# TrevorS/qwen3-tts-rs

Hardware: AMD Instinct MI355X
Metric: acoustic_frames_per_sec (higher is better)
Workload: dtype bf16

## Files before the change

include/q3tts.h:

```cpp
#ifndef Q3TTS_H
#define Q3TTS_H

#include <stddef.h>
#include <stdint.h>

#ifdef __cplusplus
extern "C" {
#endif

#define Q3_ABI_VERSION 1
#define Q3_MAX_BATCH 64

typedef enum q3_status {
    Q3_OK = 0,
    Q3_INVALID_ARG = 1,
    Q3_IO = 2,
    Q3_MISSING_WEIGHT = 3,
    Q3_KV_OVERFLOW = 4,
    Q3_HIP_ERROR = 5,
    Q3_RCCL_ERROR = 6,
    Q3_UNSUPPORTED = 7,
    Q3_OOM = 8
} q3_status;

// ... 141 lines not shown
q3_status q3_session_open_text(q3_session* s, int b);
q3_status q3_session_append_text(q3_session* s, int b, const uint32_t* ids, int n, int last);
q3_status q3_session_text_state(q3_session* s, int b, int* n_text, int* frames_committed, int* frames_runnable, int* closed,
                                int* frames_replayed);

enum {
    Q3_GET_PREFILL_EMBEDS = 0,
    Q3_GET_LAST_HIDDEN = 1,
    Q3_GET_LOGITS = 2,
    Q3_GET_TRAILING = 3,
    Q3_GET_PAD_EMBED = 4,
    Q3_GET_LOGITS_HIST = 5,
    Q3_GET_CP_LOGITS = 6,
    Q3_GET_TOKEN = 7,
    Q3_GET_CP_LOGITS_HIST = 8
};
q3_status q3_session_set_kv_dtype(q3_session* s, int dtype);
q3_status q3_session_set_debug(q3_session* s, int capture_logits);
q3_status q3_session_prefill_len(q3_session* s, int b, int* prefill_len, int* trailing_len);
q3_status q3_session_get(q3_session* s, int what, int b, void* out_host, size_t bytes);
q3_status q3_talker_step(q3_session* s, const float* embeds_host, float* hidden_host, float* logits_host);
q3_status q3_cp_generate(q3_session* s, const float* last_hidden_host, const float* sem_embed_host,
                         uint32_t* codes15_host, float* cp_logits_host );
q3_status q3_frame_embed(q3_model* m, uint32_t sem_token, const uint32_t* codes15, const float* text_add_host,
                         float* out_host);
q3_status q3_sample(int device, const float* logits_host, const uint8_t* seen_host, const float* u_host,
                    int rows, int vocab, const q3_options* opts, int token_count, uint32_t* tokens_host);
void      q3_rng_seed(uint64_t seed, uint64_t* state);
float     q3_rng_next(uint64_t* state);
q3_status q3_fused_residual_rmsnorm(int device, int dtype, const void* x_host, const void* res_host,
                                    const void* w_host, int rows, int cols, float eps,
                                    void* normed_host, void* sum_host);
q3_status q3_linear(int device, const float* x_host, const uint16_t* w_bf16_host, const float* bias_host,
                    int M, int N, int K, float* y_host);
typedef struct q3_linear_ex_args {
    int M, N, K, ldx, ldy, ldr, M_alloc;
    int epi, tiled, ksplit, use_ws, zero_n, zero_guard;
    float eps;
    const float* x; const uint16_t* w; const uint16_t* w2;
    const float* bias; const float* norm_w; const float* resid;
    float* y; float* zero_buf;
} q3_linear_ex_args;
q3_status q3_linear_ex(int device, const q3_linear_ex_args* args);
typedef struct q3_attn_step_args {
    int variant, B, nh, nkv, n_splits, max_seq;
    float eps; int reserved;
    const int* pos; const float* qkv; const float* q_norm_w; const float* k_norm_w;
    const float* rope_cos; const float* rope_sin;
    float* kcache; float* vcache; float* out;
} q3_attn_step_args;
q3_status q3_attn_step(int device, const q3_attn_step_args* args);
typedef struct q3_attn_step_ex_args {
    int variant, layout, B, nh, nkv, n_splits, max_seq, rows_per_seq;
    int n_layers, layer, n_slabs, kv_row_pages;
    int qkv_S, qkv_K, g_vocab, g_proj_dim, g_ldx, g_max_frames, g_code_slot, zero_n, zero_guard;
    float eps, qkv_eps; int reserved;
    const int* pos; const float* qkv; const float* q_norm_w; const float* k_norm_w;
    const float* rope_cos; const float* rope_sin;
    float* kcache; float* vcache; float* out;
    const int* page_slots; int* rot_used; long long* stray;
    const float* qkv_part; const float* qkv_ssq;
    const float* g_logits; const uint32_t* g_tok; const float* g_qkv_tab; const float* g_proj_tab;
    float* g_x; uint32_t* g_codes; const int* g_frame_idx;
    float* zero_buf;
} q3_attn_step_ex_args;
q3_status q3_attn_step_ex(int device, const q3_attn_step_ex_args* args);
q3_status q3_kv_pages_to_bf16_ex(int device, int n_layers, int nkv, int n_pages, const int* src_slots, const int* dst_slots,
                                 const float* src, uint16_t* dst, int* rot_used, long long* stray);
int         q3_conv_path(int cout, int cin, int L, int k, int dil, int phases, int packed, int has_resid, int planes, int aligned16);
int         q3_resunit_path(int C, int L, int dil, int packed, int ya_is_xa, int planes);
const char* q3_conv_path_name(int code);
typedef struct q3_conv_ex_args {
    int kind, cin, cout, L, k, dil, stride;
    int act, planes, packed, resid_in_place, snake_raw, y2_is_x;
    int y_front, y_elems;
    int* path;
    const float* x; const float* w; const float* b;
    const float* snake_a; const float* snake_b; const float* resid; const float* scale;
    const float* post_a; const float* post_ib;
    const float* w2; const float* b2; const float* mid_a; const float* mid_ib;
    float* y; float* y2;
} q3_conv_ex_args;
q3_status q3_conv_ex(int device, const q3_conv_ex_args* args);
int q3_gemm_path(int M, int N, int K, int epi, int norm, int w2, int planes, int* path);
typedef struct q3_gemm_ex_args {
    int M, N, K, ldx, ldy, ldr, M_alloc;
    int epi, geometry, k_split, sup_m, sup_n;
    float eps;
    int* path;
    const float* x; const uint16_t* w; const uint16_t* w2;
    const float* bias; const float* norm_w; const float* resid;
    float* y;
} q3_gemm_ex_args;
q3_status q3_gemm_ex(int device, const q3_gemm_ex_args* args);
int q3_attn_prefill_path(int nh, int nkv, int use_planes, int halves, int* path);
typedef struct q3_attn_prefill_ex_args {
    int n_seq, rps, base_pos, nh, nkv, max_seq, ld_qkv, ld_out;
    int kernel, halves, use_planes;
    float eps;
    int* path;
    const float* qkv; const float* q_norm_w; const float* k_norm_w;
    const float* rope_cos; const float* rope_sin;
    float* kcache; float* vcache; float* out;
    int layout, n_layers, layer, n_slabs;
    const int* page_slots; int* rot_used; long long* stray;
} q3_attn_prefill_ex_args;
q3_status q3_attn_prefill_ex(int device, const q3_attn_prefill_ex_args* args);
typedef struct q3_prompt_rows_ex_args {
    int mode, n, cols, n_table, n_rows, n_ref, cp_vocab, lds, ldd, reserved;
    const uint16_t* table; const uint32_t* ids; const float* src;
    const int* text_row; const int* codec_id; const float* xvec;
    const uint32_t* ref_codes; const uint16_t* cp_embs;
    const int* dst_row; const int* ent;
    float* out; int* trail_len; int* text_ready; int* limit;
} q3_prompt_rows_ex_args;
q3_status q3_prompt_rows_ex(int device, const q3_prompt_rows_ex_args* args);
int q3_attn_c_path(int hd, int kernel);
typedef struct q3_attn_c_ex_args {
    int mode, nh, hd, L, kernel, window;
    int N, n_rows, layers, layer, cap, n_blocks, n_tabs;
    float scale;
    const float* q; const float* k; const float* v;
    const int* rows; const float* caches;
    const int* tabs; const int* tab0; const int* tab_n;
    float* o;
} q3_attn_c_ex_args;
q3_status q3_attn_c_ex(int device, const q3_attn_c_ex_args* args);
q3_status q3_rope_c_ex(int device, float* q, float* k, const float* cs, const float* sn, const int* pos, int nh, int hd, int L, int n_pos);
q3_status q3_copy_cols_ex(int device, const float* src, size_t src_elems, float* dst, size_t dst_elems, int n, int C, const long long* s_off,
                          const long long* d_off, const int* sp, const int* dp, size_t src_off, size_t dst_off);
q3_status q3_copy_segs_ex(int device, const float* src, size_t src_elems, float* dst, size_t dst_elems, int n_segs, const unsigned long long* segs);
q3_status q3_gather_frames_ex(int device, const uint32_t* src, size_t src_elems, const long long* s_off, int n, uint32_t* dst, size_t dst_elems);
q3_status q3_rvq_embed_ex(int device, const uint32_t* frames, int n_frames, const float* first_cb, const float* rest_cbs, int cb_dim, int cb_size,
                          float* first_out, float* rest_out, int out_front, int out_elems);
q3_status q3_silu_mul_ex(int device, const float* g, const float* u, float* y, long long n, long long y_elems);
typedef struct q3_spk_op_ex_args {
    int op, C, T, pl, Tp, ld, off, reserved;
    long long a_elems, b_elems, out_front, out_elems;
    const float* a; const float* b; float* out;
} q3_spk_op_ex_args;
q3_status q3_spk_op_ex(int device, const q3_spk_op_ex_args* args);
typedef struct q3_mimi_op_ex_args {
    int op, C, L, r, Lf, elu, replicate, reserved;
    long long a_elems, b_elems, out_front, out_elems;
    const float* a; const float* b; float* out;
} q3_mimi_op_ex_args;
q3_status q3_mimi_op_ex(int device, const q3_mimi_op_ex_args* args);
q3_status q3_mimi_rvq_ex(int device, const float* proj, int T, const float* books, int n_layers, int CB, int CD, uint32_t* codes, int n_q,
                         int q0);
typedef struct q3_sample_rec {
    float inv_temp; int apply_temp, greedy;
    int top_k; float top_p; int use_top_p;
    float rep_pen, rep_inv; int use_rep;
    int eos_id, min_new_tokens, pad;
} q3_sample_rec;
q3_status q3_sample_row(const q3_options* opts, q3_sample_rec* out);
typedef struct q3_prompt_shape_rec {
    int32_t icl, n_ins, n_ref_text, n_icl, overlay;
    int32_t prefill_len, n_rows;
    int32_t trailing_len, n_trail;
    int32_t limit, open_need, prefix_pages;
    int32_t r_role, r_pad, r_bos, r_text, r_eos, trail_base;
} q3_prompt_shape_rec;
q3_status q3_prompt_shape(const q3_request* req, int n_text, q3_prompt_shape_rec* out, int* text_row, int* codec_id, int cap_positions);
typedef struct q3_sample_ex_args {
    int B, vocab, ld, u_stride, u_elems, advance, token_count_static, hist_stride_b, hist_cap, codec_eos, use_suppress, guard;
// ... 228 lines not shown
```

qwen3_tts_rs_amd/_lib.py:

```python
import ctypes
import os

from .config import CConfig

_HERE = os.path.dirname(os.path.abspath(__file__))
LIB_PATH = os.environ.get("Q3TTS_LIB") or os.path.join(_HERE, "libq3tts.so")

if not os.path.exists(LIB_PATH):
    raise ImportError(
        f"{LIB_PATH} not found: the gfx950 HIP library is not built. Run "
        "`python -c 'import __graft_entry__ as g; g.build()'` (or qwen3_tts_rs_amd/csrc/build.sh).")

lib = ctypes.CDLL(LIB_PATH)


class COptions(ctypes.Structure):
    _fields_ = [
        ("temperature", ctypes.c_double), ("top_p", ctypes.c_double), ("repetition_penalty", ctypes.c_double),
        ("seed", ctypes.c_uint64), ("max_length", ctypes.c_int32), ("top_k", ctypes.c_int32),
        ("eos_token_id", ctypes.c_int32), ("chunk_frames", ctypes.c_int32), ("min_new_tokens", ctypes.c_int32),
        ("has_seed", ctypes.c_int32),
    ]


# ... 199 lines not shown
    "q3_pcm_stage_tempo_lags": (c_int, [c_void_p, c_int, P(ctypes.c_int64), c_void_p, ctypes.c_size_t, P(ctypes.c_size_t)]),
    "q3_session_set_tempo": (c_int, [c_void_p, c_int, c_int]),
    "q3_batcher_ticket_tempo": (c_int, [c_void_p, ctypes.c_int64, c_int]),
    "q3_pcm_stage_set_pitch": (c_int, [c_void_p, c_int, c_int]),
    "q3_pcm_stage_pitch_plan": (c_int, [c_int, c_int, P(c_int), P(ctypes.c_double)]),
    "q3_pcm_stage_pitch_tables": (c_int, [c_void_p, ctypes.c_size_t, c_void_p, ctypes.c_size_t, P(c_int), P(c_int)]),
    "q3_pcm_stage_pitch_count": (c_int, [c_int, c_int, ctypes.c_size_t, c_int, P(ctypes.c_size_t)]),
    "q3_pcm_stage_bound_pitch": (c_int, [ctypes.c_uint32, c_int, c_int, c_int, ctypes.c_size_t, P(ctypes.c_size_t)]),
    "q3_session_set_pitch": (c_int, [c_void_p, c_int, c_int]),
    "q3_batcher_ticket_pitch": (c_int, [c_void_p, ctypes.c_int64, c_int]),
    "q3_pcm_stage_set_silence": (c_int, [c_void_p, c_int, c_int, c_int, c_int]),
    "q3_pcm_stage_silence": (c_int, [c_void_p, c_int] + [P(ctypes.c_int64)] * 5),
    "q3_pcm_stage_silence_hold": (c_int, [c_int, c_int, P(ctypes.c_size_t)]),
    "q3_pcm_stage_bound_silence": (c_int, [ctypes.c_uint32, c_int, c_int, c_int, c_int, c_int, ctypes.c_size_t, P(ctypes.c_size_t)]),
    "q3_silence_trim": (c_int, [c_void_p, ctypes.c_size_t, c_int, c_int, c_int, c_void_p, ctypes.c_size_t, P(ctypes.c_size_t), P(ctypes.c_int64)]),
    "q3_session_set_silence": (c_int, [c_void_p, c_int, c_int, c_int, c_int]),
    "q3_session_silence": (c_int, [c_void_p, c_int] + [P(ctypes.c_int64)] * 5),
    "q3_batcher_ticket_silence": (c_int, [c_void_p, ctypes.c_int64, c_int, c_int, c_int]),
    "q3_batcher_ticket_silence_read": (c_int, [c_void_p, ctypes.c_int64] + [P(ctypes.c_int64)] * 5),
    "q3_pcm_stage_set_level": (c_int, [c_void_p, c_int, c_int, c_int]),
    "q3_pcm_stage_level_coeffs": (c_int, [c_int, c_int, P(ctypes.c_float), P(ctypes.c_float)]),
    "q3_pcm_stage_level_count": (c_int, [ctypes.c_size_t, c_int, P(ctypes.c_size_t)]),
    "q3_pcm_stage_bound_level": (c_int, [ctypes.c_uint32, c_int, ctypes.c_size_t, P(ctypes.c_size_t)]),
    "q3_session_set_level": (c_int, [c_void_p, c_int, c_int, c_int]),
    "q3_batcher_ticket_level": (c_int, [c_void_p, ctypes.c_int64, c_int, c_int]),
    "q3_loudness_kweight": (c_int, [ctypes.c_uint32, P(ctypes.c_double), P(ctypes.c_double)]),
    "q3_pcm_stage_loudness_consts": (c_int, [c_int, c_int, P(ctypes.c_float), P(ctypes.c_float), P(ctypes.c_float), P(ctypes.c_float), P(ctypes.c_float)]),
    "q3_pcm_stage_set_loudness": (c_int, [c_void_p, c_int, c_int, c_int, c_int]),
    "q3_pcm_stage_loudness": (c_int, [c_void_p, c_int, P(ctypes.c_float), P(ctypes.c_float), P(c_int), P(c_int)]),
    "q3_pcm_stage_loudness_blocks": (c_int, [c_void_p, c_int, c_void_p, ctypes.c_size_t, P(ctypes.c_size_t)]),
    "q3_session_set_loudness": (c_int, [c_void_p, c_int, c_int, c_int, c_int]),
    "q3_session_loudness": (c_int, [c_void_p, c_int, P(ctypes.c_float), P(ctypes.c_float), P(c_int), P(c_int)]),
    "q3_batcher_ticket_loudness": (c_int, [c_void_p, ctypes.c_int64, c_int, c_int, c_int]),
    "q3_batcher_ticket_loudness_read": (c_int, [c_void_p, ctypes.c_int64, P(ctypes.c_float), P(ctypes.c_float), P(c_int), P(c_int)]),
    "q3_codec_stream_push_out": (c_int, [c_void_p, c_int, P(c_int), P(c_void_p), P(c_int), c_void_p, P(c_int), P(c_int), P(c_void_p),
                                         P(ctypes.c_size_t), P(ctypes.c_size_t)]),
    "q3_session_set_output": (c_int, [c_void_p, ctypes.c_uint32, c_int]),
    "q3_session_next_chunks_out": (c_int, [c_void_p, P(c_void_p), P(ctypes.c_size_t), P(ctypes.c_size_t), P(c_int)]),
    "q3_batcher_ticket_output": (c_int, [c_void_p, ctypes.c_int64, ctypes.c_uint32, c_int]),
    "q3_batcher_read_out": (c_int, [c_void_p, ctypes.c_int64, c_void_p, ctypes.c_size_t, P(ctypes.c_size_t), P(c_int)]),
    "q3_session_replace": (c_int, [c_void_p, c_int, c_void_p]),
    "q3_session_park_row": (c_int, [c_void_p, c_int, P(c_void_p)]),
    "q3_session_resume_row": (c_int, [c_void_p, c_int, c_void_p]),
    "q3_parked_free": (None, [c_void_p]),
    "q3_parked_info": (c_int, [c_void_p, P(c_int), P(c_int), P(c_int), P(c_int), P(ctypes.c_size_t)]),
    "q3_row_move": (c_int, [c_int, c_void_p, ctypes.c_size_t, c_void_p, ctypes.c_size_t, c_int, P(ctypes.c_size_t), P(ctypes.c_size_t),
                            P(ctypes.c_size_t), P(c_int)]),
    "q3_batcher_create": (c_int, [c_void_p, c_int, c_int, c_int, P(c_void_p)]),
    "q3_batcher_free": (None, [c_void_p]),
    "q3_batcher_submit": (c_int, [c_void_p, c_void_p, c_int, P(ctypes.c_int64)]),
    "q3_batcher_submit_streamed": (c_int, [c_void_p, c_void_p, P(ctypes.c_int64)]),
    "q3_batcher_read": (c_int, [c_void_p, ctypes.c_int64, c_void_p, ctypes.c_size_t, P(ctypes.c_size_t), P(c_int)]),
    "q3_batcher_stream_info": (c_int, [c_void_p, P(c_int), P(ctypes.c_size_t), P(c_int), P(c_int), P(c_int)]),
    "q3_batcher_submit_open": (c_int, [c_void_p, c_void_p, c_int, P(ctypes.c_int64)]),
    "q3_batcher_append_text": (c_int, [c_void_p, ctypes.c_int64, c_void_p, c_int, c_int]),
    "q3_batcher_text_state": (c_int, [c_void_p, ctypes.c_int64, P(c_int), P(c_int), P(c_int), P(c_int)]),
    "q3_batcher_cancel": (c_int, [c_void_p, ctypes.c_int64]),
    "q3_batcher_set_parking": (c_int, [c_void_p, c_int, c_int, c_int]),
    "q3_batcher_park": (c_int, [c_void_p, ctypes.c_int64]),
    "q3_batcher_unpark": (c_int, [c_void_p, ctypes.c_int64]),
    "q3_batcher_park_info": (c_int, [c_void_p, P(c_int), P(c_int), P(ctypes.c_longlong), P(ctypes.c_longlong), P(ctypes.c_longlong), P(c_int)]),
    "q3_batcher_step": (c_int, [c_void_p, c_int, c_int, P(c_int), P(c_int), P(c_int)]),
    "q3_batcher_poll": (c_int, [c_void_p, ctypes.c_int64, P(c_int), P(c_int), P(ctypes.c_size_t)]),
    "q3_batcher_fetch": (c_int, [c_void_p, ctypes.c_int64, c_void_p, c_int, c_void_p, ctypes.c_size_t]),
    "q3_session_set_debug": (c_int, [c_void_p, c_int]),
    "q3_session_prefill_len": (c_int, [c_void_p, c_int, P(c_int), P(c_int)]),
    "q3_session_get": (c_int, [c_void_p, c_int, c_int, c_void_p, ctypes.c_size_t]),
    "q3_talker_step": (c_int, [c_void_p, c_void_p, c_void_p, c_void_p]),
    "q3_cp_generate": (c_int, [c_void_p, c_void_p, c_void_p, c_void_p, c_void_p]),
    "q3_frame_embed": (c_int, [c_void_p, ctypes.c_uint32, c_void_p, c_void_p, c_void_p]),
    "q3_sample": (c_int, [c_int, c_void_p, c_void_p, c_void_p, c_int, c_int, P(COptions), c_int, c_void_p]),
    "q3_rng_seed": (None, [ctypes.c_uint64, P(ctypes.c_uint64)]),
    "q3_rng_next": (ctypes.c_float, [P(ctypes.c_uint64)]),
    "q3_fused_residual_rmsnorm": (c_int, [c_int, c_int, c_void_p, c_void_p, c_void_p, c_int, c_int, ctypes.c_float, c_void_p, c_void_p]),
    "q3_linear": (c_int, [c_int, c_void_p, c_void_p, c_void_p, c_int, c_int, c_int, c_void_p]),
    "q3_linear_ex": (c_int, [c_int, P(CLinearEx)]),
    "q3_attn_step": (c_int, [c_int, P(CAttnStep)]),
    "q3_attn_step_ex": (c_int, [c_int, P(CAttnStepEx)]),
    "q3_kv_pages_to_bf16_ex": (c_int, [c_int] * 4 + [c_void_p] * 6),
    "q3_conv_path": (c_int, [c_int] * 10),
    "q3_resunit_path": (c_int, [c_int] * 6),
    "q3_conv_path_name": (c_char_p, [c_int]),
    "q3_conv_ex": (c_int, [c_int, P(CConvEx)]),
    "q3_gemm_path": (c_int, [c_int] * 7 + [P(ctypes.c_int32)]),
    "q3_gemm_ex": (c_int, [c_int, P(CGemmEx)]),
    "q3_attn_prefill_path": (c_int, [c_int] * 4 + [P(ctypes.c_int32)]),
    "q3_attn_prefill_ex": (c_int, [c_int, P(CAttnPrefillEx)]),
    "q3_prompt_rows_ex": (c_int, [c_int, P(CPromptRowsEx)]),
    "q3_attn_c_path": (c_int, [c_int, c_int]),
    "q3_attn_c_ex": (c_int, [c_int, P(CAttnCEx)]),
    "q3_rope_c_ex": (c_int, [c_int, c_void_p, c_void_p, c_void_p, c_void_p, c_void_p, c_int, c_int, c_int, c_int]),
    "q3_copy_cols_ex": (c_int, [c_int, c_void_p, ctypes.c_size_t, c_void_p, ctypes.c_size_t, c_int, c_int, c_void_p, c_void_p, c_void_p, c_void_p,
                                ctypes.c_size_t, ctypes.c_size_t]),
    "q3_copy_segs_ex": (c_int, [c_int, c_void_p, ctypes.c_size_t, c_void_p, ctypes.c_size_t, c_int, c_void_p]),
    "q3_gather_frames_ex": (c_int, [c_int, c_void_p, ctypes.c_size_t, c_void_p, c_int, c_void_p, ctypes.c_size_t]),
    "q3_rvq_embed_ex": (c_int, [c_int, c_void_p, c_int, c_void_p, c_void_p, c_int, c_int, c_void_p, c_void_p, c_int, c_int]),
    "q3_silu_mul_ex": (c_int, [c_int, c_void_p, c_void_p, c_void_p, ctypes.c_longlong, ctypes.c_longlong]),
    "q3_spk_op_ex": (c_int, [c_int, P(CSpkOpEx)]),
    "q3_mimi_op_ex": (c_int, [c_int, P(CMimiOpEx)]),
    "q3_mimi_rvq_ex": (c_int, [c_int, c_void_p, c_int, c_void_p, c_int, c_int, c_int, c_void_p, c_int, c_int]),
    "q3_spk_tables": (c_int, [c_void_p, c_void_p, c_void_p]),
    "q3_sample_row": (c_int, [P(COptions), P(CSampleRow)]),
    "q3_prompt_shape": (c_int, [P(CRequest), c_int, P(CPromptShape), c_void_p, c_void_p, c_int]),
    "q3_sample_ex": (c_int, [c_int, P(CSampleEx)]),
    "q3_frame_embed_ex": (c_int, [c_int, P(CFrameEmbedEx)]),
    "q3_cp_gather_ex": (c_int, [c_int, P(CCpGatherEx)]),
    "q3_rmsnorm_ex": (c_int, [c_int, c_void_p, ctypes.c_longlong, ctypes.c_longlong, c_int, c_void_p, c_void_p, ctypes.c_longlong,
                              ctypes.c_longlong, c_int, c_int, c_int, ctypes.c_float, c_void_p, c_void_p]),
    "q3_norm_c": (c_int, [c_int, c_int, c_void_p, c_void_p, c_void_p, c_int, c_int, ctypes.c_float, c_void_p, c_int, c_int]),
    "q3_dwconv7": (c_int, [c_int, c_void_p, c_void_p, c_void_p, c_int, c_int, c_void_p, c_int, c_int]),
    "q3_decode_codes": (c_int, [c_void_p, c_void_p, c_int, c_void_p, P(c_void_p)]),
    "q3_codes_to_tensor": (None, [c_void_p, c_int, c_void_p]),
    "q3_session_set_profile": (c_int, [c_void_p, c_int]),
    "q3_session_profile_read": (c_int, [c_void_p, P(ctypes.c_double), P(ctypes.c_double), P(ctypes.c_long), c_int]),
    "q3_session_profile_shapes": (c_int, [c_void_p, P(c_int), c_int, P(c_int), c_int]),
    "q3_bench_linear": (c_int, [c_int] * 9 + [P(ctypes.c_double)]),
    "q3_session_stream": (c_int, [c_void_p, P(c_void_p)]),
    "q3_session_frame_bytes": (c_int, [c_void_p, c_int, P(ctypes.c_double), P(ctypes.c_double)]),
    "q3_session_submit_info": (c_int, [c_void_p, P(c_int), P(c_int)]),
    "q3_session_submit_fences": (c_int, [c_void_p, P(c_int), P(c_int)]),
    "q3_session_set_stream_mode": (c_int, [c_void_p, c_int]),
    "q3_session_open_text": (c_int, [c_void_p, c_int]),
    "q3_session_append_text": (c_int, [c_void_p, c_int, c_void_p, c_int, c_int]),
    "q3_session_text_state": (c_int, [c_void_p, c_int, P(c_int), P(c_int), P(c_int), P(c_int), P(c_int)]),
    "q3_model_config": (c_int, [c_void_p, P(CConfig)]),
    "q3_config_default": (c_int, [c_int, P(CConfig)]),
    "q3_config_from_json": (c_int, [c_char_p, P(CConfig), P(c_int)]),
    "q3_model_load": (c_int, [c_char_p, c_int, P(c_void_p), P(c_int)]),
    "q3_model_load_safetensors": (c_int, [c_void_p, c_char_p, P(c_int)]),
    "q3_safetensors_info": (c_int, [c_char_p, c_char_p, P(c_int), P(ctypes.c_int64), c_int, P(c_int)]),
    "q3_pcm16_from_f32": (c_int, [c_void_p, ctypes.c_int64, c_void_p]),
    "q3_wav_write_pcm16": (c_int, [c_char_p, c_void_p, ctypes.c_int64, ctypes.c_uint32]),
    "q3_g711_from_pcm16": (c_int, [c_void_p, ctypes.c_int64, c_int, c_void_p]),
    "q3_wav_write_g711": (c_int, [c_char_p, c_void_p, ctypes.c_int64, ctypes.c_uint32, c_int]),
    "q3_wav_read": (c_int, [c_char_p, c_void_p, ctypes.c_int64, P(ctypes.c_int64), P(ctypes.c_uint32)]),
    "q3_codes_write_bin": (c_int, [c_char_p, c_void_p, c_int, c_int]),
    "q3_codes_read_bin": (c_int, [c_char_p, c_void_p, c_int, c_int, P(c_int)]),
    "q3_audio_write_bin": (c_int, [c_char_p, c_void_p, ctypes.c_int64]),
    "q3_audio_read_bin": (c_int, [c_char_p, c_void_p, ctypes.c_int64, P(ctypes.c_int64)]),
    "q3_resample": (c_int, [c_void_p, ctypes.c_int64, ctypes.c_uint32, ctypes.c_uint32, c_void_p, ctypes.c_int64, P(ctypes.c_int64)]),
    "q3_dp_unique_id": (c_int, [c_void_p]),
    "q3_dp_init": (c_int, [c_int, c_int, c_void_p, c_int, P(c_void_p)]),
    "q3_dp_free": (None, [c_void_p]),
    "q3_dp_info": (c_int, [c_void_p, P(c_int), P(c_int)]),
    "q3_dp_broadcast_weights": (c_int, [c_void_p, c_void_p, c_int]),
    "q3_dp_allgather_f64": (c_int, [c_void_p, c_void_p, c_int, c_void_p]),
    "q3_spk_config_default": (c_int, [P(CSpkConfig)]),
    "q3_spk_config_from_json": (c_int, [c_char_p, P(CSpkConfig), P(c_int)]),
    "q3_spk_create": (c_int, [P(CSpkConfig), c_int, P(c_void_p)]),
    "q3_spk_free": (None, [c_void_p]),
    "q3_spk_get_config": (c_int, [c_void_p, P(CSpkConfig)]),
    "q3_spk_n_tensors": (c_int, [c_void_p]),
    "q3_spk_tensor_info": (c_int, [c_void_p, c_int, P(c_char_p), P(ctypes.c_int64)]),
    "q3_spk_set_tensor": (c_int, [c_void_p, c_char_p, c_void_p, c_int, ctypes.c_int64]),
    "q3_spk_finalize": (c_int, [c_void_p]),
    "q3_spk_load_safetensors": (c_int, [c_void_p, c_char_p]),
    "q3_spk_mel_frames": (c_int, [ctypes.c_int64]),
    "q3_spk_mel": (c_int, [c_void_p, c_void_p, ctypes.c_int64, c_void_p, ctypes.c_int64, P(c_int)]),
    "q3_spk_forward": (c_int, [c_void_p, c_void_p, c_int, c_void_p, P(c_void_p)]),
    "q3_spk_encode": (c_int, [c_void_p, c_void_p, ctypes.c_int64, ctypes.c_uint32, c_void_p]),
    "q3_mimi_config_default": (c_int, [P(CMimiConfig)]),
    "q3_mimi_create": (c_int, [P(CMimiConfig), c_int, P(c_void_p)]),
    "q3_mimi_free": (None, [c_void_p]),
    "q3_mimi_get_config": (c_int, [c_void_p, P(CMimiConfig)]),
    "q3_mimi_n_tensors": (c_int, [c_void_p]),
    "q3_mimi_tensor_info": (c_int, [c_void_p, c_int, P(c_char_p), P(ctypes.c_int64)]),
# ... 38 lines not shown
```

qwen3_tts_rs_amd/api.py:

```python
import ctypes
import enum
from dataclasses import dataclass
from typing import List, NamedTuple, Optional, Sequence, Tuple

import numpy as np

from . import _lib
from ._lib import lib, check, COptions, CRequest, CTiming
from .config import Q3Config
from . import synth

MAX_BATCH = 64
CODEC_EOS_TOKEN_ID = 2150
SAMPLES_PER_FRAME = 1920


class Language(enum.Enum):
    Chinese = 2055
    English = 2050
    Japanese = 2058
    Korean = 2064
    German = 2053
    French = 2061
    Russian = 2069
# ... 1997 lines not shown
def copy_segs_ex(src: np.ndarray, dst: np.ndarray, segs, device: int = 0) -> np.ndarray:
    src = np.ascontiguousarray(src, dtype=np.float32)
    assert dst.dtype == np.float32 and dst.flags.c_contiguous and dst.ndim == 1 and src.ndim == 1
    sg = np.ascontiguousarray(segs, dtype=np.uint64); assert sg.ndim == 2 and sg.shape[1] == 3
    check(lib.q3_copy_segs_ex(device, _vp(src), src.size, _vp(dst), dst.size, sg.shape[0], _vp(sg)))
    return dst


def gather_frames_ex(src: np.ndarray, s_off, dst: np.ndarray, device: int = 0) -> np.ndarray:
    src = np.ascontiguousarray(src, dtype=np.uint32)
    assert dst.dtype == np.uint32 and dst.flags.c_contiguous and dst.ndim == 1 and src.ndim == 1
    so = np.ascontiguousarray(s_off, dtype=np.int64); assert so.ndim == 1
    check(lib.q3_gather_frames_ex(device, _vp(src), src.size, _vp(so), so.size, _vp(dst), dst.size))
    return dst


def rvq_embed_ex(frames: np.ndarray, first_cb: np.ndarray, rest_cbs: np.ndarray, first_out: np.ndarray, rest_out: np.ndarray, out_front: int = 0,
                 device: int = 0):
    fr = np.ascontiguousarray(frames, dtype=np.uint32); assert fr.ndim == 2 and fr.shape[1] == 16
    fc = np.ascontiguousarray(first_cb, dtype=np.float32); rc = np.ascontiguousarray(rest_cbs, dtype=np.float32)
    assert fc.ndim == 2 and rc.shape == (15,) + fc.shape
    for buf in (first_out, rest_out):
        assert buf.dtype == np.float32 and buf.flags.c_contiguous and buf.ndim == 1 and buf.size == first_out.size
    check(lib.q3_rvq_embed_ex(device, _vp(fr), fr.shape[0], _vp(fc), _vp(rc), fc.shape[1], fc.shape[0], _vp(first_out), _vp(rest_out), out_front,
                              first_out.size))
    return first_out, rest_out


def silu_mul_ex(g: np.ndarray, u: np.ndarray, y: np.ndarray, device: int = 0) -> np.ndarray:
    g = np.ascontiguousarray(g, dtype=np.float32); u = np.ascontiguousarray(u, dtype=np.float32)
    assert g.ndim == 1 and u.shape == g.shape and y.dtype == np.float32 and y.flags.c_contiguous and y.ndim == 1
    check(lib.q3_silu_mul_ex(device, _vp(g), _vp(u), _vp(y), g.size, y.size))
    return y


SPK_PAD, SPK_COLS, SPK_MEAN, SPK_SE_APPLY, SPK_ASP_IN, SPK_ASP_POOL = range(6)
MIMI_ELU, MIMI_FOLD, MIMI_CODEBOOK = range(3)


def _clone_op(args, call, a, b, out, out_front, device):
    aa = np.ascontiguousarray(a, dtype=np.float32)
    bb = None if b is None else np.ascontiguousarray(b, dtype=np.float32)
    assert out.dtype == np.float32 and out.flags.c_contiguous and out.ndim == 1
    args.a_elems, args.b_elems, args.out_front, args.out_elems = aa.size, 0 if bb is None else bb.size, out_front, out.size
    args.a, args.b, args.out = _vp(aa), _vp(bb), _vp(out)
    check(call(device, ctypes.byref(args)))
    return out


def spk_op_ex(op: int, a: np.ndarray, out: np.ndarray, *, C: int, T: int, b: Optional[np.ndarray] = None, pl: int = 0, Tp: int = 0, ld: int = 0,
              off: int = 0, out_front: int = 0, device: int = 0) -> np.ndarray:
    args = _lib.CSpkOpEx()
    args.op, args.C, args.T, args.pl, args.Tp, args.ld, args.off = op, C, T, pl, Tp, ld, off
    return _clone_op(args, lib.q3_spk_op_ex, a, b, out, out_front, device)


def mimi_op_ex(op: int, a: np.ndarray, out: np.ndarray, *, L: int, C: int = 1, r: int = 1, Lf: int = 0, elu: bool = False, replicate: bool = False,
               b: Optional[np.ndarray] = None, out_front: int = 0, device: int = 0) -> np.ndarray:
    args = _lib.CMimiOpEx()
    args.op, args.C, args.L, args.r, args.Lf, args.elu, args.replicate = op, C, L, r, Lf, int(elu), int(replicate)
    return _clone_op(args, lib.q3_mimi_op_ex, a, b, out, out_front, device)


def mimi_rvq_ex(proj: np.ndarray, books: np.ndarray, codes: np.ndarray, q0: int = 0, device: int = 0) -> np.ndarray:
    pp = np.ascontiguousarray(proj, dtype=np.float32); bk = np.ascontiguousarray(books, dtype=np.float32)
    assert pp.ndim == 2 and bk.ndim == 3 and bk.shape[2] == pp.shape[0]
    assert codes.dtype == np.uint32 and codes.flags.c_contiguous and codes.ndim == 2 and codes.shape[0] == pp.shape[1]
    check(lib.q3_mimi_rvq_ex(device, _vp(pp), pp.shape[1], _vp(bk), bk.shape[0], bk.shape[1], bk.shape[2], _vp(codes), codes.shape[1], q0))
    return codes


def resunit_path(C: int, L: int, dil: int, packed: bool = True, ya_is_xa: bool = False, planes: int = 3) -> int:
    return lib.q3_resunit_path(C, L, dil, int(packed), int(ya_is_xa), planes)


def conv_path_name(code: int) -> str:
    return lib.q3_conv_path_name(code).decode()


def conv_ex(kind: int, x: np.ndarray, w: np.ndarray, *, dil: int = 1, stride: int = 1, b: Optional[np.ndarray] = None, snake=None,
            post=None, mid=None, resid: Optional[np.ndarray] = None, resid_in_place: bool = False, scale: Optional[np.ndarray] = None,
            act: int = 0, planes: int = 3, packed: bool = True, snake_raw: bool = False, w2: Optional[np.ndarray] = None,
            b2: Optional[np.ndarray] = None, y: Optional[np.ndarray] = None, y2: Optional[np.ndarray] = None, y_front: int = 0,
            y2_is_x: bool = False, device: int = 0):
    f = lambda a: np.ascontiguousarray(a, dtype=np.float32)
    x = f(x); w = f(w)
    assert x.ndim == 2 and w.ndim == 3
    cin, L = x.shape
    cout = w.shape[1] if kind == 1 else w.shape[0]
    assert (w.shape[0] if kind == 1 else w.shape[1]) == cin
    a = _lib.CConvEx()
    a.kind, a.cin, a.cout, a.L, a.k, a.dil, a.stride = kind, cin, cout, L, w.shape[2], dil, stride
    a.act, a.planes, a.packed, a.resid_in_place, a.snake_raw, a.y2_is_x = act, planes, int(packed), int(resid_in_place), int(snake_raw), int(y2_is_x)
    n_out = cout * L * (stride if kind == 1 else 1)
    if y is None:
        y = np.zeros(n_out, dtype=np.float32); y_front = 0
    for buf in (y, y2):
        assert buf is None or (buf.dtype == np.float32 and buf.flags.c_contiguous and buf.ndim == 1 and buf.size == y.size)
    a.y_front, a.y_elems = y_front, y.size
    path = ctypes.c_int32(0)
    a.path = ctypes.pointer(path)
    keep = [x, w]
    ptr = lambda arr: arr.ctypes.data_as(ctypes.c_void_p)
    a.x, a.w, a.y = ptr(x), ptr(w), ptr(y)
    if y2 is not None:
        a.y2 = ptr(y2)

    def opt(name, arr, n):
        if arr is not None:
            arr = f(arr); assert arr.size == n, (name, arr.size, n)
            keep.append(arr); setattr(a, name, ptr(arr))
    opt("b", b, cout); opt("b2", b2, cout); opt("scale", scale, cout); opt("resid", resid, n_out)
    if w2 is not None:
        opt("w2", w2, cout * cin)
    for (na, nb, pr, n) in (("snake_a", "snake_b", snake, cin), ("post_a", "post_ib", post, cout), ("mid_a", "mid_ib", mid, cout)):
        if pr is not None:
            opt(na, pr[0], n); opt(nb, pr[1], n)
    try:
        check(lib.q3_conv_ex(device, ctypes.byref(a)))
    except _lib.Q3Error as e:
        e.path = path.value
        raise
    return y, y2, path.value


def norm_c(x: np.ndarray, w: np.ndarray, b: Optional[np.ndarray] = None, eps: float = 1e-6, y: Optional[np.ndarray] = None,
           y_front: int = 0, device: int = 0) -> np.ndarray:
    x = np.ascontiguousarray(x, dtype=np.float32); C, L = x.shape
    w = np.ascontiguousarray(w, dtype=np.float32); assert w.shape == (C,)
    bb = None if b is None else np.ascontiguousarray(b, dtype=np.float32)
    if y is None:
        y = np.zeros(C * L, dtype=np.float32); y_front = 0
    assert y.dtype == np.float32 and y.flags.c_contiguous and y.ndim == 1
    ptr = lambda arr: arr.ctypes.data_as(ctypes.c_void_p)
    check(lib.q3_norm_c(device, 0 if bb is None else 1, ptr(x), ptr(w), None if bb is None else ptr(bb), C, L, eps, ptr(y), y_front, y.size))
    return y


def dwconv7(x: np.ndarray, w: np.ndarray, b: np.ndarray, y: Optional[np.ndarray] = None, y_front: int = 0, device: int = 0) -> np.ndarray:
    x = np.ascontiguousarray(x, dtype=np.float32); C, L = x.shape
    w = np.ascontiguousarray(w, dtype=np.float32); b = np.ascontiguousarray(b, dtype=np.float32)
    assert w.shape == (C, 7) and b.shape == (C,)
    if y is None:
        y = np.zeros(C * L, dtype=np.float32); y_front = 0
    assert y.dtype == np.float32 and y.flags.c_contiguous and y.ndim == 1
    ptr = lambda arr: arr.ctypes.data_as(ctypes.c_void_p)
    check(lib.q3_dwconv7(device, ptr(x), ptr(w), ptr(b), C, L, ptr(y), y_front, y.size))
    return y


def _io(arr, dtype, n, name):
    assert isinstance(arr, np.ndarray) and arr.dtype == dtype and arr.flags.c_contiguous and arr.ndim == 1 and arr.size == n, (name, n)
    return _vp(arr)


def prompt_shape(u: Utterance, options: SynthesisOptions, n_text: Optional[int] = None, tables: bool = False):
    r = CRequest(); keep = []; rec = _lib.CPromptShape()
    fill_request(r, u, options, keep)
    n = r.n_text if n_text is None else int(n_text)
    check(lib.q3_prompt_shape(ctypes.byref(r), n, ctypes.byref(rec), None, None, 0))
    if not tables:
        return rec
    tr = np.zeros(rec.prefill_len, np.int32); ci = np.zeros(rec.prefill_len, np.int32)
    check(lib.q3_prompt_shape(ctypes.byref(r), n, ctypes.byref(rec), tr.ctypes.data_as(ctypes.c_void_p), ci.ctypes.data_as(ctypes.c_void_p), rec.prefill_len))
    return rec, tr, ci


def sample_row(options: SynthesisOptions) -> "_lib.CSampleRow":
    r = _lib.CSampleRow(); o = options.to_c()
    check(lib.q3_sample_row(ctypes.byref(o), ctypes.byref(r)))
    return r


def sample_ex(logits: np.ndarray, u: np.ndarray, vocab: int, tok: np.ndarray, scalar, *, rows=None, seen: Optional[np.ndarray] = None,
              u_stride: int = 1, draw_idx=None, token_count: Optional[np.ndarray] = None, token_count_static: int = 0, advance: bool = False,
              frame_idx: Optional[np.ndarray] = None, pos: Optional[np.ndarray] = None, limit=None, text_ready=None,
              logits_hist: Optional[np.ndarray] = None, hist_stride_b: int = 0, hist_cap: int = 0, codec_eos: int = 2150,
              use_suppress: bool = True, guard: int = 0, device: int = 0) -> np.ndarray:
    lg = np.ascontiguousarray(logits, dtype=np.float32); assert lg.ndim == 2
    B, ld = lg.shape
    uu = np.ascontiguousarray(u, dtype=np.float32).reshape(-1)
    a = _lib.CSampleEx()
    a.B, a.vocab, a.ld, a.u_stride, a.u_elems, a.advance, a.token_count_static = B, vocab, ld, u_stride, uu.size, int(advance), token_count_static
    a.hist_stride_b, a.hist_cap, a.codec_eos, a.use_suppress, a.guard = hist_stride_b, hist_cap, codec_eos, int(use_suppress), guard
    a.scalar = scalar
    keep = [lg, uu]
    a.logits, a.u = _vp(lg), _vp(uu)
    a.tok = _io(tok, np.uint32, B + 2 * guard, "tok")
    if seen is not None:
        a.seen = _io(seen, np.uint8, B * vocab + 2 * guard, "seen")
    for name, arr in (("token_count", token_count), ("frame_idx", frame_idx), ("pos", pos)):
        if arr is not None:
            setattr(a, name, _io(arr, np.int32, B + 2 * guard, name))
    if logits_hist is not None:
        a.logits_hist = _io(logits_hist, np.float32, B * hist_stride_b + 2 * guard, "logits_hist")
    for name, arr in (("draw_idx", draw_idx), ("limit", limit), ("text_ready", text_ready)):
        if arr is not None:
            v = np.ascontiguousarray(arr, dtype=np.int32); assert v.shape == (B,), name
            keep.append(v); setattr(a, name, _vp(v))
    if rows is not None:
        assert len(rows) == B
        rr = (_lib.CSampleRow * B)(*rows); keep.append(rr)
        a.rows = ctypes.cast(rr, ctypes.c_void_p)
    check(lib.q3_sample_ex(device, ctypes.byref(a)))
    return tok

# ... 106 lines not shown
```

qwen3_tts_rs_amd/csrc/q3_codec_run.hip:

```cpp
#include "q3_engine.h"

namespace {
struct DevCache {
    std::mutex mu;
    std::unordered_multimap<uint64_t, void*> free_blocks;
    std::unordered_map<void*, uint64_t> live;
    size_t cached = 0, cap = 0;
    DevCache() { const char* e = getenv("Q3_DEV_CACHE_MB"); cap = (size_t)(e ? atol(e) : 32768) << 20; }
    static uint64_t key(int dev, size_t bytes) { return ((uint64_t)dev << 48) | (uint64_t)bytes; }
    static size_t size_class(size_t bytes) {
        if (bytes <= 4096) return (bytes + 255) & ~(size_t)255;
        size_t p2 = 1; while ((p2 << 1) <= bytes) p2 <<= 1;
        const size_t step = p2 >> 4;
        return (bytes + step - 1) / step * step;
    }
    hipError_t get(void** p, size_t bytes) {
        bytes = size_class(bytes);
        int dev = 0; (void)hipGetDevice(&dev);
        const uint64_t k = key(dev, bytes);
        {
            std::lock_guard<std::mutex> g(mu);
            auto it = free_blocks.find(k);
            if (it != free_blocks.end()) { *p = it->second; free_blocks.erase(it); cached -= bytes; live[*p] = k; return hipSuccess; }
        }
// ... 6 lines not shown
        std::lock_guard<std::mutex> g(mu);
        live[*p] = k;
        return hipSuccess;
    }
    void put(void* p) {
        if (!p) return;
        uint64_t k = 0; bool known = false;
        {
            std::lock_guard<std::mutex> g(mu);
            auto it = live.find(p);
            if (it != live.end()) { k = it->second; known = true; live.erase(it); }
            const size_t bytes = (size_t)(k & 0xffffffffffffull);
            if (known && cap && cached + bytes <= cap) { free_blocks.emplace(k, p); cached += bytes; return; }
        }
        (void)hipFree(p);
    }
    void trim(size_t keep) {
        std::vector<void*> drop;
        {
            std::lock_guard<std::mutex> g(mu);
            for (auto it = free_blocks.begin(); it != free_blocks.end() && cached > keep;) {
                cached -= (size_t)(it->first & 0xffffffffffffull); drop.push_back(it->second); it = free_blocks.erase(it);
            }
        }
        for (void* p : drop) (void)hipFree(p);
    }
};
DevCache& dev_cache() { static DevCache* c = new DevCache(); return *c; }
}
hipError_t dev_malloc(void** p, size_t bytes) { return dev_cache().get(p, bytes ? bytes : 4); }
void dev_free(void* p) { dev_cache().put(p); }

q3_status codec_reserve(const q3_model* m, CodecWS& ws, int T, int Tf) {
    if (Tf < T) Tf = T;
    if (T <= ws.cap_frames && Tf <= ws.cap_front) return Q3_OK;
    if (T < ws.cap_frames) T = ws.cap_frames;
    if (Tf < ws.cap_front) Tf = ws.cap_front;
    if (ws.bufA) HIPC(q3_hipDeviceSynchronize());
    ws.release();
    const q3_config& c = m->cfg;
    int up = 1; for (int i = 0; i < 2; ++i) up *= c.dec_up_ratios[i];
    size_t per = (size_t)4 * c.dec_latent * up;
    { size_t L = up; int C = c.dec_dim; per = per > (size_t)C * L ? per : (size_t)C * L;
      for (int b = 0; b < 4; ++b) { L *= c.dec_up_rates[b]; C /= 2; if ((size_t)C * L > per) per = (size_t)C * L; } }
    const int QDm = c.dec_heads * c.dec_head_dim;
    size_t per_front = (size_t)4 * QDm;
    if ((size_t)2 * c.dec_inter > per_front) per_front = (size_t)2 * c.dec_inter;
    if ((size_t)2 * c.dec_cb_dim > per_front) per_front = (size_t)2 * c.dec_cb_dim;
    if ((size_t)c.dec_latent > per_front) per_front = (size_t)c.dec_latent;
    if ((size_t)c.dec_q_dim > per_front) per_front = (size_t)c.dec_q_dim;
    size_t n = per * (size_t)T;
    if (per_front * (size_t)Tf > n) n = per_front * (size_t)Tf;
    HIPC(dev_malloc((void**)&ws.bufA, n * 4)); HIPC(dev_malloc((void**)&ws.bufB, n * 4)); HIPC(dev_malloc((void**)&ws.bufC, n * 4));
    HIPC(dev_malloc((void**)&ws.bufF, n * 4));
    const size_t small = (size_t)Tf * (size_t)(QDm > c.dec_latent ? QDm : c.dec_latent);
    HIPC(dev_malloc((void**)&ws.bufD, small * 4)); HIPC(dev_malloc((void**)&ws.bufE, small * 4));
    HIPC(dev_malloc((void**)&ws.cs, (size_t)Tf * 32 * 4)); HIPC(dev_malloc((void**)&ws.sn, (size_t)Tf * 32 * 4));
    HIPC(dev_malloc((void**)&ws.frames, (size_t)Tf * 16 * 4));
    size_t total_up = up; for (int b = 0; b < 4; ++b) total_up *= c.dec_up_rates[b];
    HIPC(dev_malloc((void**)&ws.pcm, (size_t)T * total_up * 4));
    Q3C(codec_rope_table(c, Tf, ws.cs, ws.sn));
    ws.cap_frames = T; ws.cap_front = Tf;
    return Q3_OK;
}
q3_status codec_rope_table(const q3_config& c, int n, float* cs_dev, float* sn_dev) {
    std::vector<float> cs((size_t)n * 32), sn((size_t)n * 32);
    for (int i = 0; i < 32; ++i) {
        const float inv = 1.0f / powf(c.dec_theta, (float)(2 * i) / (float)c.dec_head_dim);
        for (int t = 0; t < n; ++t) { const float f = (float)t * inv; cs[(size_t)t * 32 + i] = cosf(f); sn[(size_t)t * 32 + i] = sinf(f); }
    }
    HIPC(q3_hipMemcpy(cs_dev, cs.data(), cs.size() * 4, hipMemcpyHostToDevice));
    HIPC(q3_hipMemcpy(sn_dev, sn.data(), sn.size() * 4, hipMemcpyHostToDevice));
    return Q3_OK;
}

int samples_per_frame(const q3_config& c) {
    int u = 1; for (int i = 0; i < 2; ++i) u *= c.dec_up_ratios[i]; for (int i = 0; i < 4; ++i) u *= c.dec_up_rates[i];
    return u;
}

static thread_local const q3_model* tl_codec_model = nullptr;
static const void* packed_of(const float* w) { return tl_codec_model ? tl_codec_model->pk(w) : nullptr; }
static thread_local int tl_codec_planes = 3;
CodecScope::CodecScope(const q3_model* m) {
    static const int env_planes = [] { const char* e = getenv("Q3_CODEC_PLANES"); const int v = e ? atoi(e) : 0; return (v == 2 || v == 3) ? v : 0; }();
    planes = env_planes ? env_planes : m->codec_planes;
    tl_codec_model = m; tl_codec_planes = planes;
}
CodecScope::~CodecScope() { tl_codec_planes = 3; }
static hipError_t conv1(const float* x, const float* w, const float* b, float* y, int cin, int cout, int L, hipStream_t st,
                        const float* resid = nullptr, const float* scale = nullptr, int act = 0,
                        const float* sa = nullptr, const float* sib = nullptr) {
    ConvArgs a; a.x = x; a.w = w; a.b = b; a.y = y; a.cin = cin; a.cout = cout; a.L = L; a.k = 1; a.dil = 1;
    a.resid = resid; a.scale = scale; a.act = act; a.snake_a = sa; a.snake_b = sib; a.wpk = packed_of(w); a.planes = tl_codec_planes;
    return launch_conv1d(a, st);
}
static hipError_t convk(const float* x, const float* w, const float* b, float* y, int cin, int cout, int L, int k, int dil,
                        hipStream_t st, const float* sa = nullptr, const float* sib = nullptr, int act = 0) {
    ConvArgs a; a.x = x; a.w = w; a.b = b; a.y = y; a.cin = cin; a.cout = cout; a.L = L; a.k = k; a.dil = dil;
    a.snake_a = sa; a.snake_b = sib; a.act = act; a.wpk = packed_of(w); a.planes = tl_codec_planes;
    return launch_conv1d(a, st);
}

static q3_status tap_out(float** taps, int id, const float* dev, size_t n, hipStream_t st) {
    if (taps && taps[id]) { HIPC(hipStreamSynchronize(st)); HIPC(q3_hipMemcpy(taps[id], dev, n * 4, hipMemcpyDeviceToHost)); }
    return Q3_OK;
}
q3_status codec_front_quant(const q3_model* m, CodecWS& ws, int T, hipStream_t st) {
    const q3_config& c = m->cfg;
    const int CD = c.dec_cb_dim, Q = c.dec_q_dim;
    float *A = ws.bufA, *B = ws.bufB;
    float* e1 = A; float* e2 = A + (size_t)CD * T;
    HIPC(launch_rvq_embed(ws.frames, T, m->first_cb, m->rest_cbs_dev, e1, e2, CD, c.dec_cb_size, st));
    HIPC(conv1(e1, m->first_proj, nullptr, B, CD, Q, T, st));
    HIPC(conv1(e2, m->rest_proj, nullptr, B, CD, Q, T, st, B));
    return Q3_OK;
}
q3_status codec_front_preconv(const q3_model* m, const float* x, float* y, int L, hipStream_t st) {
    HIPC(convk(x, m->pre_w, m->pre_b, y, m->cfg.dec_q_dim, m->cfg.dec_latent, L, 3, 1, st));
    return Q3_OK;
}
q3_status codec_front_transformer(const q3_model* m, CodecWS& ws, int T, hipStream_t st, const CodecAttnFn& rope_attn) {
    const q3_config& c = m->cfg;
    const int LAT = c.dec_latent, DH = c.dec_hidden, QD = c.dec_heads * c.dec_head_dim, DI = c.dec_inter;
    float *A = ws.bufA, *B = ws.bufB, *C = ws.bufC, *D = ws.bufD, *E = ws.bufE;
    float* Hd = D;
    HIPC(conv1(C, m->inp_w, m->inp_b, Hd, LAT, DH, T, st));
    float* Nn = E;
    float* q = A; float* k = A + (size_t)QD * T; float* v = A + (size_t)2 * QD * T; float* ao = A + (size_t)3 * QD * T;
    float* g = B; float* u = B + (size_t)DI * T;
    for (int l = 0; l < c.dec_layers; ++l) {
        const DecLayerW& L = m->dl[l];
        HIPC(launch_rmsnorm_c(Hd, L.in_ln, Nn, DH, T, c.dec_eps, st));
        auto adjacent = [&](const float* w0, const float* w1, int cout, int cin) {
            const char* p0 = (const char*)m->pk(w0); const char* p1 = (const char*)m->pk(w1);
            return p0 && p1 && p1 == p0 + packed_conv_w_bytes(cout, cin, 1) && w1 == w0 + (size_t)cout * cin &&
                   cout % 32 == 0 && cin % 16 == 0;
        };
        static const bool no_fuse_qkv = getenv("Q3_CODEC_NO_QKV_FUSE") != nullptr || getenv("Q3_CONV_F32") != nullptr ||
                                        getenv("Q3_CONV_VALU") != nullptr;
        if (!no_fuse_qkv && adjacent(L.q, L.k, QD, DH) && adjacent(L.k, L.v, QD, DH)) {
            HIPC(conv1(Nn, L.q, nullptr, q, DH, 3 * QD, T, st));
        } else {
            HIPC(conv1(Nn, L.q, nullptr, q, DH, QD, T, st));
            HIPC(conv1(Nn, L.k, nullptr, k, DH, QD, T, st));
            HIPC(conv1(Nn, L.v, nullptr, v, DH, QD, T, st));
        }
        Q3C(rope_attn(l, q, k, v, ao));
        HIPC(conv1(ao, L.o, nullptr, Hd, QD, DH, T, st, Hd, L.attn_scale));
        HIPC(launch_rmsnorm_c(Hd, L.post_ln, Nn, DH, T, c.dec_eps, st));
        if (!no_fuse_qkv && adjacent(L.gate, L.up, DI, DH)) {
            HIPC(conv1(Nn, L.gate, nullptr, g, DH, 2 * DI, T, st));
        } else {
            HIPC(conv1(Nn, L.gate, nullptr, g, DH, DI, T, st));
            HIPC(conv1(Nn, L.up, nullptr, u, DH, DI, T, st));
        }
        HIPC(launch_silu_mul(g, u, g, (int64_t)DI * T, st));
        HIPC(conv1(g, L.down, nullptr, Hd, DI, DH, T, st, Hd, L.mlp_scale));
    }
    HIPC(launch_rmsnorm_c(Hd, m->dec_norm, Nn, DH, T, c.dec_eps, st));
    HIPC(conv1(Nn, m->outp_w, m->outp_b, C, DH, LAT, T, st));
    return Q3_OK;
}
q3_status codec_stack_dev(const q3_model* m, CodecWS& ws, float* cur, int L, hipStream_t st, float** taps, const CodecScope& scope) {
    const int NPL = scope.planes;
    const q3_config& c = m->cfg;
    const int LAT = c.dec_latent;
    auto TAP = [&](int id, const float* dev, size_t n) -> q3_status { return tap_out(taps, id, dev, n, st); };
    float *A = ws.bufA, *B = ws.bufB, *C = ws.bufC;
    for (int i = 0; i < 2; ++i) {
        const UpW& U = m->up[i];
        float* upo = (cur == C) ? A : C;
        HIPC(launch_transconv1d_taps(cur, U.tw, U.tb, upo, LAT, LAT, L, U.ratio, 1, nullptr, nullptr, st, nullptr, nullptr, nullptr, m->pk(U.tw), NPL));
        L *= U.ratio;
        float* dw = (upo == A) ? C : A;
        HIPC(launch_dwconv7(upo, U.dww, U.dwb, dw, LAT, L, st));
        float* ln = dw + (size_t)LAT * L;
        HIPC(launch_layernorm_c(dw, U.nw, U.nb, ln, LAT, L, 1e-6f, st));
        HIPC(conv1(ln, U.p1w, U.p1b, B, LAT, 4 * LAT, L, st, nullptr, nullptr, 1));
        HIPC(conv1(B, U.p2w, U.p2b, upo, 4 * LAT, LAT, L, st, upo, U.gamma));
        cur = upo;
        Q3C(TAP(Q3_DEC_UP0 + i, cur, (size_t)LAT * L));
    }
    int Cc = c.dec_dim;
    float* pool4[4] = {A, B, C, ws.bufF};
    auto other = [&](std::initializer_list<const float*> used) -> float* {
        for (float* p : pool4) { bool u = false; for (const float* q : used) if (q == p) u = true; if (!u) return p; }
        return nullptr;
    };
    float* xact = other({cur});
    {
        ConvArgs a; a.x = cur; a.w = m->init_w; a.wpk = m->pk(m->init_w); a.b = m->init_b; a.cin = LAT; a.cout = Cc; a.L = L; a.k = 7; a.dil = 1; a.planes = NPL;
        a.post_a = m->blk[0].a; a.post_ib = m->blk[0].ib;
        if (taps && taps[Q3_DEC_INIT]) { float* raw = other({cur, xact}); a.y = raw; a.y2 = xact; HIPC(launch_conv1d(a, st)); Q3C(TAP(Q3_DEC_INIT, raw, (size_t)Cc * L)); }
        else { a.y = xact; HIPC(launch_conv1d(a, st)); }
    }
    static const int dils[3] = {1, 3, 9};
    for (int b = 0; b < 4; ++b) {
        const DecBlockW& Bk = m->blk[b];
        float* Y = other({xact});
        float* YA = other({xact, Y});
        HIPC(launch_transconv1d_taps(xact, Bk.tw, Bk.tb, Y, Bk.cin, Bk.cout, L, Bk.rate, 2, nullptr, nullptr, st, Bk.res[0].a1, Bk.res[0].ib1, YA, m->pk(Bk.tw), NPL));
        L *= Bk.rate; Cc = Bk.cout;
        float* T2 = other({Y, YA});
        for (int uu = 0; uu < 3; ++uu) {
            const ResUnitW& R = Bk.res[uu];
            const float* nxt_a = uu < 2 ? Bk.res[uu + 1].a1 : (b < 3 ? m->blk[b + 1].a : m->fin_a);
            const float* nxt_ib = uu < 2 ? Bk.res[uu + 1].ib1 : (b < 3 ? m->blk[b + 1].ib : m->fin_ib);
            {
                ResUnitArgs r{};
                r.xa = YA; r.y = Y; r.ya = T2; r.w1pk = m->pk(R.c1w); r.w2pk = m->pk(R.c2w); r.b1 = R.c1b; r.b2 = R.c2b;
                r.mid_a = R.a2; r.mid_ib = R.ib2; r.post_a = nxt_a; r.post_ib = nxt_ib; r.C = Cc; r.L = L; r.dil = dils[uu]; r.planes = NPL;
                const hipError_t e = launch_resunit(r, st);
                if (e == hipSuccess) { float* t = YA; YA = T2; T2 = t; continue; }
                if (e != hipErrorNotSupported) HIPC(e);
            }
            {
                ConvArgs a; a.x = YA; a.w = R.c1w; a.wpk = m->pk(R.c1w); a.b = R.c1b; a.y = T2; a.cin = Cc; a.cout = Cc; a.L = L; a.k = 7; a.dil = dils[uu]; a.planes = NPL;
                a.post_a = R.a2; a.post_ib = R.ib2;
                HIPC(launch_conv1d(a, st));
            }
            {
                ConvArgs a; a.x = T2; a.w = R.c2w; a.wpk = m->pk(R.c2w); a.b = R.c2b; a.y = Y; a.y2 = YA; a.cin = Cc; a.cout = Cc; a.L = L; a.k = 1; a.dil = 1; a.resid = Y; a.planes = NPL;
                if (uu < 2) { a.post_a = Bk.res[uu + 1].a1; a.post_ib = Bk.res[uu + 1].ib1; }
                else if (b < 3) { a.post_a = m->blk[b + 1].a; a.post_ib = m->blk[b + 1].ib; }
                else { a.post_a = m->fin_a; a.post_ib = m->fin_ib; }
                HIPC(launch_conv1d(a, st));
            }
        }
        Q3C(TAP(Q3_DEC_BLK0 + b, Y, (size_t)Cc * L));
        xact = YA;
    }
    HIPC(convk(xact, m->fin_w, m->fin_b, ws.pcm, Cc, 1, L, 7, 1, st, nullptr, nullptr, 2));
    return Q3_OK;
}

q3_status codec_decode_dev(const q3_model* m, CodecWS& ws, int T, hipStream_t st, float** taps, int c0) {
    const q3_config& c = m->cfg;
    const CodecScope scope(m);
    const int Q = c.dec_q_dim, LAT = c.dec_latent;
    float *B = ws.bufB, *C = ws.bufC;
    Q3C(codec_front_quant(m, ws, T, st));
    Q3C(tap_out(taps, Q3_DEC_QUANT, B, (size_t)Q * T, st));
    Q3C(codec_front_preconv(m, B, C, T, st));
    Q3C(tap_out(taps, Q3_DEC_PRECONV, C, (size_t)LAT * T, st));
    const float scale = (float)pow((double)c.dec_head_dim, -0.5);
    Q3C(codec_front_transformer(m, ws, T, st, [&](int, float* q, float* k, float* v, float* ao) -> q3_status {
        HIPC(launch_rope_c(q, k, ws.cs, ws.sn, c.dec_heads, c.dec_head_dim, T, st));
        HIPC(launch_attn_c(q, k, v, ao, c.dec_heads, c.dec_head_dim, T, scale, st));
        return Q3_OK;
    }));
    Q3C(tap_out(taps, Q3_DEC_PRETRANS, C, (size_t)LAT * T, st));
    float* cur = C;
    int L = T;
    if (c0 > 0) {
        HIPC(launch_copy_rows(C + c0, T, ws.bufF, T - c0, LAT, T - c0, st));
        cur = ws.bufF; L = T - c0;
    }
    return codec_stack_dev(m, ws, cur, L, st, taps, scope);
}

extern "C" q3_status q3_decode_codes(q3_model* m, const uint32_t* frames_host, int n_frames, float* pcm_host, float** taps_host) {
    if (!m || !m->finalized) return set_err(Q3_INVALID_ARG, "model not finalized");
    if (n_frames < 0 || (n_frames > 0 && (!frames_host || !pcm_host))) return set_err(Q3_INVALID_ARG, "q3_decode_codes: bad argument");
    if (n_frames == 0) return Q3_OK;
    for (int f = 0; f < n_frames; ++f)
        for (int g = 1; g < 16; ++g)
            if (frames_host[(size_t)f * 16 + g] >= (uint32_t)m->cfg.dec_cb_size)
                return set_err(Q3_INVALID_ARG, "code %u out of range for codebook %d (frame %d)", frames_host[(size_t)f * 16 + g], g, f);
    HIPC(hipSetDevice(m->device));
    CodecWS ws;
    q3_status st = codec_reserve(m, ws, n_frames);
    if (st == Q3_OK) {
        hipError_t e = q3_hipMemcpy(ws.frames, frames_host, (size_t)n_frames * 16 * 4, hipMemcpyHostToDevice);
        if (e != hipSuccess) st = set_err(Q3_HIP_ERROR, "hipMemcpy frames: %s", hipGetErrorString(e));
    }
    if (st == Q3_OK) st = codec_decode_dev(m, ws, n_frames, 0, taps_host);
    if (st == Q3_OK) {
        hipError_t e = q3_hipDeviceSynchronize();
        if (e == hipSuccess) e = q3_hipMemcpy(pcm_host, ws.pcm, (size_t)n_frames * samples_per_frame(m->cfg) * 4, hipMemcpyDeviceToHost);
        if (e != hipSuccess) st = set_err(Q3_HIP_ERROR, "decode: %s", hipGetErrorString(e));
    }
    ws.release();
    return st;
}
```

qwen3_tts_rs_amd/csrc/q3_engine.h:

```cpp
#pragma once
#include "../../include/q3tts.h"
#include "q3_kernels.h"

#include <math.h>
#include <stdarg.h>
#include <stdio.h>
#include <string.h>

#include <algorithm>
#include <atomic>
#include <chrono>
#include <functional>
#include <memory>
#include <string>
#include <thread>
#include <mutex>
#include <unordered_map>
#include <vector>

#include "q3_internal.h"
#include "q3_aql.h"

using namespace q3;
#define Q3_HIDDEN __attribute__((visibility("hidden")))
// ... 285 lines not shown
    int gain_mB = 0, ceil_mB = 0;
    int loud = Q3_LOUD_OFF, target_mB = -1900, prior_mB = 0;
    int sil_mB = 0, edge_ms = 0, pause_ms = 20;
    bool plain() const {
        return rate == 24000 && fmt == Q3_PCM_F32 && tempo == 1000 && cents == 0 && gain_mB == 0 && ceil_mB == 0 && loud == Q3_LOUD_OFF && sil_mB == 0;
    }
    size_t sample_bytes() const { return fmt == Q3_PCM_F32 ? 4 : fmt == Q3_PCM_S16 ? 2 : 1; }
};

struct q3_session {
    q3_model* m = nullptr; int B = 0;
    hipStream_t stream = nullptr; bool owns_stream = true;
    DevPool pool;
    std::vector<SeqInfo> seq;
    q3_options opts{};
    int max_frames = 0, max_seq = 0, prefill_len = 0, n_splits = 1;
    int* limit = nullptr;
    SampleRow* sample_rows = nullptr;
    int row_cap = 0, repl_base = 0;
    LmBuf tb{}, cb{};
    float *LASTH = nullptr, *LOGITS = nullptr, *CP_IN = nullptr, *CP_LOGITS = nullptr;
    float* wide_ws = nullptr; size_t wide_ws_bytes = 0;
    float *kcache = nullptr, *vcache = nullptr, *ckcache = nullptr, *cvcache = nullptr;
    size_t kv_layer_stride = 0, ckv_layer_stride = 0;
    bool paged = false; unsigned long long* kv_table = nullptr; std::vector<std::vector<float*>> kv_rows;
    std::vector<BatReq> ragged;
    bool regrouped = false;
    bool prefix_common = false;
    int kv_overflow_row = -1;
    bool kv_bf16 = false, kv_in_bf16 = false; unsigned long long* kv_conv = nullptr;
    float *rows = nullptr, *embeds = nullptr, *xvec = nullptr; int n_rows_total = 0;
    uint32_t* ids_dev = nullptr; int *tr_dev = nullptr, *ci_dev = nullptr; float *proj_e = nullptr, *proj_h = nullptr;
    uint32_t* ref_codes_dev = nullptr;
    int *trail_base = nullptr, *trail_len = nullptr, *pad_row = nullptr;
    int* text_ready = nullptr;
    uint32_t* app_ids = nullptr; float *app_e = nullptr, *app_h = nullptr, *app_out = nullptr;
    int* flush_buf = nullptr; size_t flush_cap = 0;
    uint32_t* tok = nullptr; uint8_t* seen = nullptr; int *frame_idx = nullptr, *pos = nullptr, *token_count = nullptr;
    float* U = nullptr; uint32_t* codes = nullptr;
    float* logits_hist = nullptr; float* cp_logits_hist = nullptr; bool debug = false;
    bool prefilled = false; int frames_run = 0;
    uint64_t uid = 0; char* park_desc = nullptr; std::shared_ptr<ParkShelf> shelf;
    hipGraphExec_t graph_exec = nullptr; hipGraph_t graph = nullptr;
    q3::AqlProgram* aql = nullptr; int aql_mode = 0; bool aql_tried = false, aql_failed = false;
    bool precapture = false;
    CodecWS cws;
    q3_codec_stream* cstream = nullptr;
    q3_pcm_stage* ostage = nullptr; bool out_started = false;
    std::vector<OutSettings> out;
    hipStream_t dec_stream = nullptr; hipEvent_t dec_ev = nullptr;
    std::vector<CodecWS> par_ws; std::vector<hipStream_t> par_streams;
    CodecWS seg_ws;
    std::vector<uint32_t> codes_host; bool codes_host_valid = false;
    int stream_pos = 0;
    int stream_mode = 0;
    bool profile = false; ProfAcc prof_linear;
    bool legacy_attn = getenv("Q3_LEGACY_ATTN") != nullptr;
    bool proj_tables = getenv("Q3_NO_PROJ_TABLES") == nullptr;
    bool qkv_tables = getenv("Q3_NO_QKV_TABLES") == nullptr;
    bool ksplit = getenv("Q3_NO_KSPLIT") == nullptr;
    bool cp_attn = getenv("Q3_NO_CP_ATTN") == nullptr;
    bool no_chunk = getenv("Q3_NO_CHUNK") != nullptr;
    std::vector<std::pair<hipEvent_t, hipEvent_t>> prof_events; std::vector<double> prof_event_bytes;
    std::vector<hipEvent_t> prof_pool; size_t prof_pool_next = 0;
    std::vector<ProfShape> prof_shapes;
#ifdef Q3_TRACE
    unsigned long long* trace_buf = nullptr; int trace_node = 0, trace_cap = 0;
    struct TraceMeta { int kind, a, b, c, d, e, f; };
    std::vector<TraceMeta> trace_meta;
    unsigned long long* trace_next(int kind, int a, int b, int c, int d = 0, int e = 0, int f = 0) {
        if (!trace_buf || trace_node >= trace_cap) return nullptr;
        trace_meta.push_back({kind, a, b, c, d, e, f});
        return trace_buf + (size_t)(trace_node++) * TRACE_NODE;
    }
#endif
    ~q3_session();
};


Q3_HIDDEN void model_destroy(q3_model* m);
Q3_HIDDEN void retile_bf16(const uint16_t* src, int N, int K, uint16_t* dst, int mode);
Q3_HIDDEN q3_status codec_reserve(const q3_model* m, CodecWS& ws, int T, int Tf = 0);
Q3_HIDDEN int samples_per_frame(const q3_config& c);
Q3_HIDDEN q3_status codec_decode_dev(const q3_model* m, CodecWS& ws, int T, hipStream_t st, float** taps, int c0 = 0);
struct Q3_HIDDEN CodecScope { int planes; explicit CodecScope(const q3_model* m); ~CodecScope(); CodecScope(const CodecScope&) = delete; };
using CodecAttnFn = std::function<q3_status(int layer, float* q, float* k, float* v, float* ao)>;
Q3_HIDDEN q3_status codec_rope_table(const q3_config& c, int n, float* cs_dev, float* sn_dev);
Q3_HIDDEN q3_status codec_front_quant(const q3_model* m, CodecWS& ws, int T, hipStream_t st);
Q3_HIDDEN q3_status codec_front_preconv(const q3_model* m, const float* x, float* y, int L, hipStream_t st);
Q3_HIDDEN q3_status codec_front_transformer(const q3_model* m, CodecWS& ws, int T, hipStream_t st, const CodecAttnFn& rope_attn);
Q3_HIDDEN q3_status codec_stack_dev(const q3_model* m, CodecWS& ws, float* cur, int L, hipStream_t st, float** taps, const CodecScope& scope);
struct CsPush {
    int row; int n; int skip; const uint32_t* host; const uint32_t* dev; float* pcm_host;
    q3_pcm_stage* ps = nullptr; int ps_row = -1; int last = 0; void* out_host = nullptr; size_t* n_out = nullptr;
};
Q3_HIDDEN q3_status codec_stream_create(q3_model* m, int rows, int max_frames, hipStream_t st, q3_codec_stream** out, int block_frames = 0,
                                        int max_blocks = 0);
Q3_HIDDEN q3_status codec_stream_push(q3_codec_stream* cs, const std::vector<CsPush>& pushes);
Q3_HIDDEN int codec_stream_pos(const q3_codec_stream* cs, int row);
Q3_HIDDEN void codec_stream_blocks(const q3_codec_stream* cs, int row, int upto, int* held, int* need);
Q3_HIDDEN void codec_stream_reset(q3_codec_stream* cs, int row);
struct PsSeg { int row; const float* dev; size_t n; int last; };
struct PsDesc {
    const float* src; const float* tail_in; float* tail_out; const float* taps; void* out;
    long long base, i0;
    int n_new, n_out, L, M, fmt, pad;
};
struct PsPlan { std::vector<PsDesc> desc; std::vector<size_t> off, count; size_t bytes = 0; bool late = false; };
Q3_HIDDEN void resampler_taps(int L, int M, std::vector<float>& out);
Q3_HIDDEN int pcm_stage_rows(const q3_pcm_stage* ps);
Q3_HIDDEN void pcm_stage_reset(q3_pcm_stage* ps, int row);
Q3_HIDDEN q3_status pcm_stage_check_rows(const q3_pcm_stage* ps, const char* who, int n_rows, const int* rows);
Q3_HIDDEN size_t pcm_stage_count(const q3_pcm_stage* ps, int row, size_t n, int last);
Q3_HIDDEN q3_status out_set_output(const char* who, OutSettings& o, uint32_t sample_rate, int format);
Q3_HIDDEN q3_status out_set_tempo(const char* who, OutSettings& o, int tempo_permille);
Q3_HIDDEN q3_status out_set_pitch(const char* who, OutSettings& o, int cents);
Q3_HIDDEN q3_status out_set_level(const char* who, OutSettings& o, int gain_mB, int ceiling_mB);
Q3_HIDDEN q3_status out_set_loudness(const char* who, OutSettings& o, int mode, int target_mB, int prior_mB);
Q3_HIDDEN q3_status out_set_silence(const char* who, OutSettings& o, int threshold_mB, int edge_ms, int pause_ms);
Q3_HIDDEN q3_status pcm_stage_apply(q3_pcm_stage* ps, int row, const char* who, const OutSettings& o);
Q3_HIDDEN const OutSettings& pcm_stage_settings(const q3_pcm_stage* ps, int row);
Q3_HIDDEN void out_loudness_at_rest(const OutSettings& o, float* mean_square, float* gain, int* blocks, int* gated);
Q3_HIDDEN void out_silence_at_rest(int64_t* n_in, int64_t* n_out, int64_t* lead_cut, int64_t* pause_cut, int64_t* trail_cut);
Q3_HIDDEN q3_status pcm_stage_begin(q3_pcm_stage* ps, const std::vector<PsSeg>& segs, PsPlan& plan);
Q3_HIDDEN q3_status pcm_stage_run(q3_pcm_stage* ps, const std::vector<PsSeg>& segs, PsPlan& plan, const PsDesc* desc_dev, hipStream_t st);
Q3_HIDDEN void pcm_stage_finish(q3_pcm_stage* ps, const std::vector<PsSeg>& segs, const PsPlan& plan, void* const* out_host, size_t* n_samples);
Q3_HIDDEN q3_status pcm_stage_push_dev(q3_pcm_stage* ps, const std::vector<PsSeg>& segs, hipStream_t st, void* const* out_host, size_t* n_samples);
Q3_HIDDEN hipError_t sync_frames(q3_session* s);
Q3_HIDDEN q3_status kv_reserve_row(q3_session* s, int b, int n_pos);
Q3_HIDDEN q3_status kv_reserve_frames(q3_session* s, int frames);
Q3_HIDDEN void kv_release_row(q3_session* s, int b);
Q3_HIDDEN LmDims talker_dims(const q3_config& c);
Q3_HIDDEN LmDims cp_dims(const q3_config& c);
Q3_HIDDEN q3_status talker_step(q3_session* s, const int* pos_dev, int pos_static, bool with_head, int rows_per_seq = 1,
                                const int* text_ready = nullptr);
Q3_HIDDEN SampleRow sample_row(const q3_options& o);
using PromptShape = q3_prompt_shape_rec;
Q3_HIDDEN int icl_frame_cap(int n_text);
Q3_HIDDEN PromptShape prompt_shape(const q3_request& r, int n_text);
static inline PromptShape prompt_shape(const q3_request& r) { return prompt_shape(r, r.n_text); }
Q3_HIDDEN void prompt_positions(const PromptShape& sh, const q3_request& r, int row_base, int* text_row, int* codec_id);
Q3_HIDDEN long row_worst_units(int prefill_len, int limit, bool bf16);
Q3_HIDDEN q3_request idle_request(int chunk_frames);
Q3_HIDDEN q3_status session_create(q3_model* m, const q3_request* reqs, int batch, int frame_budget, int prompt_budget, q3_session** out,
                                   hipStream_t borrow = nullptr);
Q3_HIDDEN q3_status lm_layer(q3_session* s, const LmDims& d, const LayerW& w, LmBuf& b, float* kc, float* vc, int max_seq,
                             const int* pos_dev, int pos_static, int n_splits, int rows_per_seq = 1, bool skip_qkv = false,
                             const CpGatherArgs* fold = nullptr, int paged_layer = -1);
struct TextPiece { int b; const uint32_t* ids; int n; bool last; };
Q3_HIDDEN q3_status session_text_enable(q3_session* s);
Q3_HIDDEN q3_status session_append_many(q3_session* s, const std::vector<TextPiece>& pieces);
Q3_HIDDEN int session_row_remaining(const q3_session* s, int b);
Q3_HIDDEN int session_row_committed(const q3_session* s, int b);
Q3_HIDDEN q3_status session_refresh_codes(q3_session* s);
enum { ROW_MOVE_COPY = 0, ROW_MOVE_EXCHANGE = 1 };
struct RowSeg { void* src; void* dst; unsigned long long bytes; int mode; int pad; };
Q3_HIDDEN hipError_t launch_row_move(const RowSeg* segs_dev, int n_segs, size_t max_bytes, hipStream_t st);
Q3_HIDDEN int parked_frames(const q3_parked* p, const uint32_t** codes);
Q3_HIDDEN int parked_committed(const q3_parked* p);
Q3_HIDDEN int parked_pages(const q3_parked* p);
Q3_HIDDEN bool parked_done(const q3_parked* p);
Q3_HIDDEN const SeqInfo& parked_seq(const q3_parked* p);
Q3_HIDDEN q3_status transplant_row(q3_session* s, int b, q3_session* side, int j, int limit);
Q3_HIDDEN q3_status side_prefill(q3_session* host, const q3_request* reqs, const int* limit_req, int n, bool open_text, bool closed,
                                 bool prefix_common, hipStream_t borrow, std::unique_ptr<q3_session>* side_out, int* limit_out,
                                 const std::function<void()>& created = nullptr);
```

qwen3_tts_rs_amd/csrc/q3_kernels.h:

```cpp
#pragma once
#include <hip/hip_runtime.h>
#include <stdint.h>

namespace q3 {

constexpr int HEAD_DIM = 128;
constexpr int MAX_SPLITS = 64;
constexpr int PART_STRIDE = HEAD_DIM + 2;
constexpr int KV_PAGE_POS = 128, KV_PAGE_SHIFT = 7, KV_MAX_PAGES = 64;

#ifdef Q3_TRACE
constexpr int TRACE_SLOTS = 8, TRACE_WGS = 512, TRACE_DWGS = 16, TRACE_WAVES = 16;
constexpr int TRACE_NODE = TRACE_SLOTS * (TRACE_WGS + TRACE_DWGS * TRACE_WAVES);
#define Q3_TRACE_FIELD unsigned long long* trace = nullptr;
#if defined(__HIPCC__)
#define Q3T_DECL unsigned long long q3t_[q3::TRACE_SLOTS] = {0, 0, 0, 0, 0, 0, 0, 0};
#define Q3T(i) do { q3t_[i] = (unsigned long long)wall_clock64(); } while (0)
#define Q3T_W(i) do { asm volatile("s_waitcnt vmcnt(0)" ::: "memory"); q3t_[i] = (unsigned long long)wall_clock64(); } while (0)
#define Q3T_K(i, val) do { asm volatile("s_waitcnt lgkmcnt(0)" :: "s"(val) : "memory"); q3t_[i] = (unsigned long long)wall_clock64(); } while (0)
#define Q3T_FLUSH(a, wg) do { if ((a).trace && threadIdx.x == 0 && (int)(wg) < q3::TRACE_WGS) { \
        _Pragma("unroll") for (int q3i_ = 0; q3i_ < q3::TRACE_SLOTS; ++q3i_) (a).trace[(size_t)(wg) * q3::TRACE_SLOTS + q3i_] = q3t_[q3i_]; } \
    if ((a).trace && (threadIdx.x & 63) == 0 && (int)(wg) < q3::TRACE_DWGS && (int)(threadIdx.x >> 6) < q3::TRACE_WAVES) { \
        _Pragma("unroll") for (int q3i_ = 0; q3i_ < q3::TRACE_SLOTS; ++q3i_) \
            (a).trace[(size_t)q3::TRACE_SLOTS * (q3::TRACE_WGS + (wg) * q3::TRACE_WAVES + (threadIdx.x >> 6)) + q3i_] = q3t_[q3i_]; } } while (0)
// ... 134 lines not shown
int attn_prefill_rows_wg(int kernel, int nrep);
hipError_t launch_attn_prefill(const AttnArgs& a, hipStream_t st);
hipError_t launch_attn_prefill(const AttnArgs& a, const AttnPrefillPick& p, hipStream_t st);
hipError_t launch_attn_fused(const AttnArgs& a, hipStream_t st);
bool attn_cp_ok(const AttnArgs& a);
hipError_t launch_attn_cp(const AttnArgs& a, hipStream_t st);

hipError_t launch_gather_rows_bf16(const uint16_t* table, const uint32_t* ids, float* out, int n_rows, int dim,
                                   hipStream_t st);
hipError_t launch_assemble_rows(const float* rows, const int* text_row, const uint16_t* codec_emb, const int* codec_id,
                                const float* xvec, float* out, int n, int H, hipStream_t st,
                                const uint32_t* ref_codes = nullptr, const uint16_t* const* cp_embs = nullptr);
hipError_t launch_copy_rows(const float* src, int lds, float* dst, int ldd, int rows, int cols, hipStream_t st);
hipError_t launch_scatter_rows(const float* src, const int* dst_row, float* rows, int n_src, int cols, hipStream_t st);
hipError_t launch_publish_text(const int* ent, int n, int* trail_len, int* text_ready, int* limit, hipStream_t st);

struct CpGatherArgs {
    int pass;
    const float* last_hidden; int H;
    const uint16_t* codec_emb;
    const uint32_t* tok;
    const uint16_t* cp_emb;
    const float* cp_logits;
    int cp_vocab;
    uint32_t* codes;
    const int* frame_idx;
    int max_frames;
    float* out; int ld_out;
    const float* proj_tab = nullptr; int proj_dim = 0;
    const float* qkv_tab = nullptr; int qkv_dim = 0; float* qkv_out = nullptr; int ld_qkv_out = 0;
    int B;
};
hipError_t launch_cp_gather(const CpGatherArgs& a, hipStream_t st);

struct FrameEmbedArgs {
    const uint16_t* codec_emb; const uint16_t* cp_embs[15];
    const uint32_t* tok; const float* cp_logits_last; int cp_vocab;
    uint32_t* codes; const int* frame_idx; int max_frames;
    const float* text_rows; const int* trail_base; const int* trail_len; const int* pad_row;
    float* out; int H; int B; int n_acoustic;
    const int* text_ready = nullptr;
};
hipError_t launch_frame_embed(const FrameEmbedArgs& a, hipStream_t st);

struct SampleRow {
    float inv_temp; int apply_temp; int greedy;
    int top_k; float top_p; int use_top_p;
    float rep_pen, rep_inv; int use_rep;
    int eos_id; int min_new_tokens; int pad;
};
struct SampleArgs {
    const float* logits; int ld;
    uint8_t* seen;
    const float* u; int u_stride;
    const int* draw_idx;
    uint32_t* tok;
    int* token_count;
    int token_count_static;
    int* frame_idx; int* pos;
    int advance;
    const SampleRow* rows;
    const int* limit;
    float* logits_hist; int hist_stride_b; int hist_cap;
    int vocab, B;
    float inv_temp; int apply_temp; int greedy;
    int top_k; float top_p; int use_top_p;
    float rep_pen, rep_inv; int use_rep;
    int eos_id; int min_new_tokens; int codec_eos; int use_suppress;
    const int* text_ready;
};
hipError_t launch_sample(const SampleArgs& a, hipStream_t st);

struct ConvArgs {
    const float* x; const float* w; const float* b; float* y;
    int cin, cout, L, k, dil;
    const float* snake_a = nullptr; const float* snake_b = nullptr;
    const float* resid = nullptr;
    const float* scale = nullptr;
    int act = 0;
    const float* post_a = nullptr; const float* post_ib = nullptr;
    float* y2 = nullptr;
    const void* wpk = nullptr;
    int planes = 3;
};
hipError_t launch_pack_conv_w(const float* w, void* out, int cout, int cin, int K, hipStream_t st);
size_t packed_conv_w_bytes(int cout, int cin, int K);
enum ConvKernel {
    CK_NONE = 0,
    CK_OUT1 = 1, CK_OUT1_V4 = 2,
    CK_LIN_SMALL_4W = 3, CK_LIN_SMALL_8W = 4,
    CK_BF16X3_96x128_TM4 = 5,
    CK_BF16X3_4Wx32x128 = 6,
    CK_BF16X3_4Wx32x256 = 7,
    CK_BF16X3_64x128 = 8,
    CK_BF16X3_64x64 = 9,
    CK_BF16X3_128x128 = 10,
    CK_BF16X3_96x128_6W = 11,
    CK_MFMA_F32_64 = 12, CK_MFMA_F32_32 = 13,
    CK_VALU = 14,
    CK_RESUNIT_3W = 15, CK_RESUNIT_6W = 16,
    CK_COUNT = 17
};
enum { CP_KERNEL_MASK = 31, CP_PRE = 32, CP_SEG = 64, CP_CIS128 = 128, CP_NP2 = 256 };
struct ConvPath {
    int kernel = CK_NONE;
    int co_m = 0, t_m = 0, wco = 0, wt = 0;
    bool pre = false, seg = false;
    int cis = 0, np = 0;
    hipError_t refusal = hipSuccess;
};
ConvPath conv_pick(int cout, int cin, int L, int k, int dil, int phases, bool packed, bool has_resid, int planes, bool aligned16,
                   bool transposed = false);
ConvPath resunit_pick(int C, int L, int dil, bool complete, bool ya_is_xa, int planes);
int conv_path_code(const ConvPath& p);
const char* conv_path_name(int code);
hipError_t launch_conv1d(const ConvArgs& a, hipStream_t st, int* path = nullptr);
struct ResUnitArgs {
    const float* xa; float* y; float* ya;
    const void* w1pk; const void* w2pk; const float* b1; const float* b2;
    const float* mid_a; const float* mid_ib; const float* post_a; const float* post_ib;
    int C, L, dil;
    int planes = 3;
};
hipError_t launch_resunit(const ResUnitArgs& r, hipStream_t st, int* path = nullptr);
hipError_t launch_transconv1d_taps(const float* x, const float* wp, const float* b, float* y, int cin, int cout, int L,
                                   int stride, int taps, const float* snake_a, const float* snake_ib, hipStream_t st,
                                   const float* post_a = nullptr, const float* post_ib = nullptr, float* y2 = nullptr,
                                   const void* wpk = nullptr,
                                   int planes = 3, int* path = nullptr);
void transconv_phase_weights(const float* w, int cin, int cout, int k, int stride, float* out);
hipError_t launch_snake_tables(const float* alpha, const float* beta, float* a, float* ib, int C, hipStream_t st);
hipError_t launch_dwconv7(const float* x, const float* w, const float* b, float* y, int C, int L, hipStream_t st);
hipError_t launch_layernorm_c(const float* x, const float* w, const float* b, float* y, int C, int L, float eps,
                              hipStream_t st);
hipError_t launch_rmsnorm_c(const float* x, const float* w, float* y, int C, int L, float eps, hipStream_t st);
hipError_t launch_rope_c(float* q, float* k, const float* cs, const float* sn, int nh, int hd, int L, hipStream_t st);
enum { ATTN_C_VALU = 0, ATTN_C_MFMA = 1 };
int attn_c_pick();
hipError_t launch_attn_c(const float* q, const float* k, const float* v, float* o, int nh, int hd, int L, float scale,
                         hipStream_t st);
hipError_t launch_attn_c(const float* q, const float* k, const float* v, float* o, int nh, int hd, int L, float scale, int kernel,
                         hipStream_t st);
hipError_t launch_mimi_attn(const float* q, const float* k, const float* v, float* o, int nh, int hd, int T, int window, float scale,
                            hipStream_t st);
hipError_t launch_mimi_elu(const float* x, float* y, size_t n, hipStream_t st);
hipError_t launch_mimi_fold(const float* x, float* y, int C, int L, int r, int Lf, int elu, int replicate, hipStream_t st);
hipError_t launch_mimi_codebook(const float* esum, const float* usage, float* out, int CB, int dim, hipStream_t st);
hipError_t launch_mimi_rvq(const float* proj, int T, const float* books, int n_layers, int CB, int CD, uint32_t* codes, int n_q, int q0,
                           hipStream_t st);
hipError_t launch_spk_stft_mel(const float* x, long n, int T, const float* win, const double* cs, const double* sn, const float* fb, float* mel,
                               int n_mels, hipStream_t st);
hipError_t launch_spk_pad(const float* a, const float* b, float* out, int C, int T, int pl, int Tp, hipStream_t st);
hipError_t launch_spk_cols(const float* src, int ld, int off, float* dst, int C, int T, hipStream_t st);
hipError_t launch_spk_mean(const float* x, float* mean, int C, int T, hipStream_t st);
hipError_t launch_spk_se_apply(const float* o, const float* g, float* h, int C, int T, hipStream_t st);
hipError_t launch_spk_asp_in(const float* m, float* ain, int C, int T, hipStream_t st);
hipError_t launch_spk_asp_pool(const float* aw, const float* m, float* pooled, int C, int T, hipStream_t st);
struct AttnCsRow { const float* kv; int a0, e, qcol; };
struct AttnCbRow { int tab0, a0, e, qcol; };
struct ColCopy { const float* src; float* dst; int sp, dp; };
struct SegCopy { unsigned long long src, dst, n; };
hipError_t launch_rope_c_pos(float* q, float* k, const float* cs, const float* sn, const int* pos, int nh, int hd, int L, hipStream_t st);
hipError_t launch_attn_cs(const float* q, float* o, const AttnCsRow* rows, int n_rows, int max_tiles, size_t layer_off, int nh, int hd,
                          int N, int cap, float scale, hipStream_t st);
hipError_t launch_attn_cb(const float* q, float* o, const AttnCbRow* rows, const float* const* tabs, int n_rows, int max_tiles, size_t layer_off,
                          int nh, int hd, int N, int bf, float scale, hipStream_t st);
hipError_t launch_copy_cols(const ColCopy* d, int n, int C, size_t src_off, size_t dst_off, hipStream_t st);
hipError_t launch_copy_segs(const float* src, float* dst, const SegCopy* segs, int n_segs, size_t max_n, hipStream_t st);
hipError_t launch_gather_frames(const uint32_t* const* src, uint32_t* dst, int n, hipStream_t st);
hipError_t launch_silu_mul(const float* g, const float* u, float* y, int64_t n, hipStream_t st);
hipError_t launch_rvq_embed(const uint32_t* frames, int n_frames, const float* first_cb, const float* const* rest_cbs,
                            float* first_out, float* rest_out, int cb_dim, int cb_size, hipStream_t st);
hipError_t launch_norm_codebook(const float* esum, const float* usage, float* out, int rows, int dim, hipStream_t st);

#if defined(__HIPCC__)
__device__ __forceinline__ float mul_rn(float a, float b) {
#pragma clang fp contract(off)
    return a * b;
}
__device__ __forceinline__ float add_rn(float a, float b) {
#pragma clang fp contract(off)
    return a + b;
}
__device__ __forceinline__ float sub_rn(float a, float b) {
#pragma clang fp contract(off)
    return a - b;
}
typedef __attribute__((ext_vector_type(4))) float act_f4_t;
typedef __attribute__((ext_vector_type(2))) float act_f2_t;
constexpr int ACT_SC1 = 16;
__device__ __forceinline__ __amdgpu_buffer_rsrc_t act_rsrc(const void* p) {
    return __builtin_amdgcn_make_buffer_rsrc(const_cast<void*>(p), 0, 0x7fffffff, 0x00020000);
}
__device__ __forceinline__ float4 act_ld4(__amdgpu_buffer_rsrc_t r, int byte_off) {
    const act_f4_t v = __builtin_bit_cast(act_f4_t, __builtin_amdgcn_raw_buffer_load_b128(r, byte_off, 0, ACT_SC1));
    return float4{v[0], v[1], v[2], v[3]};
}
__device__ __forceinline__ float2 act_ld2(__amdgpu_buffer_rsrc_t r, int byte_off) {
    const act_f2_t v = __builtin_bit_cast(act_f2_t, __builtin_amdgcn_raw_buffer_load_b64(r, byte_off, 0, ACT_SC1));
    return float2{v[0], v[1]};
}
__device__ __forceinline__ float act_ld1(__amdgpu_buffer_rsrc_t r, int byte_off) {
    return __builtin_bit_cast(float, __builtin_amdgcn_raw_buffer_load_b32(r, byte_off, 0, ACT_SC1));
}
__device__ __forceinline__ void act_st4(__amdgpu_buffer_rsrc_t r, int byte_off, const float4& v) {
    typedef __attribute__((ext_vector_type(4))) unsigned int u4;
    const act_f4_t f = {v.x, v.y, v.z, v.w};
    __builtin_amdgcn_raw_buffer_store_b128(__builtin_bit_cast(u4, f), r, byte_off, 0, ACT_SC1);
}
__device__ __forceinline__ void act_st2(__amdgpu_buffer_rsrc_t r, int byte_off, const float2& v) {
    typedef __attribute__((ext_vector_type(2))) unsigned int u2;
    const act_f2_t f = {v.x, v.y};
// ... 52 lines not shown
```

qwen3_tts_rs_amd/csrc/q3_kernels_codec.hip:

```cpp
#include "q3_kernels.h"

#include <math.h>
#include <stdio.h>
#include <stdlib.h>

namespace q3 {

__device__ __forceinline__ float sin_sq(float x) {
    if (fabsf(x) >= 8192.0f) { const float s = sinf(x); return s * s; }
    const float k = rintf(x * 0.31830988618379067154f);
    float r = fmaf(-k, 3.140625f, x);
    r = fmaf(-k, 9.67502593994140625e-4f, r);
    r = fmaf(-k, 1.509957990978376432e-7f, r);
    const float z = r * r;
    float p = fmaf(z, -2.50521083854417188e-8f, 2.75573192239858907e-6f);
    p = fmaf(z, p, -1.98412698412698413e-4f);
    p = fmaf(z, p, 8.33333333333333333e-3f);
    p = fmaf(z, p, -1.66666666666666667e-1f);
    const float s = fmaf(r * z, p, r);
    return s * s;
}
__device__ __forceinline__ float snake_f(float x, float a, float ib) { return add_rn(x, mul_rn(sin_sq(x * a), ib)); }

constexpr int CV_CO = 32, CV_T = 128, CV_CI = 16, CV_MAXK = 7, CV_MAXHALO = 54;

__device__ __forceinline__ float conv_act(float v, int act) {
    if (act == 1) return 0.5f * v * (1.0f + erff(v * 0.70710678118654752440f));
    if (act == 3) return fmaxf(v, 0.0f);
    if (act == 4) return tanhf(fmaxf(v, 0.0f));
    if (act == 5) return 1.0f / (expf(-v) + 1.0f);
    if (act == 6) return v > 0.0f ? v : expf(v) - 1.0f;
    return v;
}

struct ConvDev {
    const float* x; const float* w; const float* b; float* y;
    int cin, cout, L, k, dil;
    const float* snake_a; const float* snake_ib;
    const float* resid; const float* scale;
    int act;
    int ostride, ooff, oL;
    size_t w_phase_stride;
    int ooff_phase;
    const float* post_a; const float* post_ib;
    float* y2;
    const void* wpk;
    size_t wpk_phase_stride;
    int phases;
    int planes;
};

__global__ __launch_bounds__(256) void k_conv1d(ConvDev a) {
    __shared__ float xs[CV_CI][CV_T + CV_MAXHALO + 2];
    __shared__ __attribute__((aligned(16))) float ws[CV_CI][CV_MAXK][CV_CO];
    const int tid = threadIdx.x, tx = tid & 31, ty = tid >> 5;
    const int t0 = blockIdx.x * CV_T, co0 = blockIdx.y * CV_CO;
    const float* w = a.w + (size_t)blockIdx.z * a.w_phase_stride;
    const int ooff = a.ooff + (int)blockIdx.z * a.ooff_phase;
    const int halo = (a.k - 1) * a.dil;
    const int W = CV_T + halo;
    float acc[4][4];
#pragma unroll
    for (int i = 0; i < 4; ++i)
#pragma unroll
        for (int j = 0; j < 4; ++j) acc[i][j] = 0.0f;

    for (int ci0 = 0; ci0 < a.cin; ci0 += CV_CI) {
        __syncthreads();
        for (int e = tid; e < CV_CI * W; e += 256) {
            const int ci = e / W, tt = e - ci * W;
            const int c = ci0 + ci, t = t0 - halo + tt;
            float v = 0.0f;
            if (c < a.cin && t >= 0 && t < a.L) {
                v = a.x[(size_t)c * a.L + t];
                if (a.snake_a) v = snake_f(v, a.snake_a[c], a.snake_ib[c]);
            }
            xs[ci][tt] = v;
        }
        for (int e = tid; e < CV_CI * a.k * CV_CO; e += 256) {
            const int co = e % CV_CO, r = e / CV_CO, kk = r % a.k, ci = r / a.k;
            const int c = ci0 + ci, o = co0 + co;
            ws[ci][kk][co] = (c < a.cin && o < a.cout) ? w[((size_t)o * a.cin + c) * a.k + kk] : 0.0f;
        }
        __syncthreads();
// ... 532 lines not shown
        for (int st = 0; st < n_steps; st += 2) {
            fetch(A[1], st + 1); do_step(A[0], st);
            fetch(A[0], st + 2); do_step(A[1], st + 1);
        }
    }
    auto load_A2 = [&](cu32x4_t (&A)[NP], int s) {
        const int tile = wave * nc16 + s;
#pragma unroll
        for (int pl = 0; pl < NP; ++pl)
            A[pl] = __builtin_bit_cast(cu32x4_t, __builtin_amdgcn_raw_buffer_load_b128(w2rs, lane * 16, (tile * 3 + pl) * 1024, 0));
    };
    constexpr unsigned plane2 = 32u * XP2;
    const unsigned bfrag2 = (unsigned)(li * XP2 + lk * 16);
#pragma unroll
    for (int tq = 0; tq < T_M; ++tq) {
        cu32x4_t A2[3][NP];
        load_A2(A2[0], 0); load_A2(A2[1], 1);
        float rs[16];
#pragma unroll
        for (int reg = 0; reg < 16; ++reg) {
            const int o = wave * 32 + (reg & 3) + 8 * (reg >> 2) + 4 * lk;
            const int t = t0 + tq * 32 + li;
            rs[reg] = t < a.L ? a.y[(size_t)o * a.L + t] : 0.0f;
        }
        __syncthreads();
        {
            const f32x16_t& ac = acc[tq];
            unsigned char* row = smem + (unsigned)li * XP2 + wave * 64 + lk * 8;
#pragma unroll
            for (int g = 0; g < 4; ++g) {
                float v[4];
#pragma unroll
                for (int j = 0; j < 4; ++j) {
                    const int pi = wave * 32 + 8 * g + 4 * lk + j;
                    v[j] = snake_f(ac[4 * g + j] + s_prm[0][pi], s_prm[1][pi], s_prm[2][pi]);
                }
                uint32_t h0, m0, l0, h1, m1, l1;
                split3_pair(v[0], v[1], h0, m0, l0); split3_pair(v[2], v[3], h1, m1, l1);
                *reinterpret_cast<uint2*>(row + g * 16) = make_uint2(h0, h1);
                *reinterpret_cast<uint2*>(row + g * 16 + plane2) = make_uint2(m0, m1);
                if constexpr (NP == 3) *reinterpret_cast<uint2*>(row + g * 16 + 2 * plane2) = make_uint2(l0, l1);
            }
        }
        __syncthreads();
        f32x16_t acc2;
#pragma unroll
        for (int r = 0; r < 16; ++r) acc2[r] = 0.0f;
        auto step2 = [&](const cu32x4_t (&Af)[NP], int s) {
            cu32x4_t B[NP];
            const unsigned char* bp = smem + (bfrag2 + (unsigned)s * 32);
            B[0] = *reinterpret_cast<const cu32x4_t*>(bp);
            B[1] = *reinterpret_cast<const cu32x4_t*>(bp + plane2);
            if constexpr (NP == 3) B[2] = *reinterpret_cast<const cu32x4_t*>(bp + 2 * plane2);
            acc2 = mfmaP<NP>(Af, B, acc2);
        };
        auto fetch2 = [&](cu32x4_t (&Ad)[NP], int sp) {
            sp = sp < nc16 - 1 ? sp : nc16 - 1;
            __builtin_amdgcn_sched_barrier(0); load_A2(Ad, sp); __builtin_amdgcn_sched_barrier(0);
        };
        static_assert(nc16 % 3 == 0, "ring of three");
        for (int s = 0; s < nc16; s += 3) {
            fetch2(A2[2], s + 2); step2(A2[0], s);
            fetch2(A2[0], s + 3); step2(A2[1], s + 1);
            fetch2(A2[1], s + 4); step2(A2[2], s + 2);
        }
#pragma unroll
        for (int reg = 0; reg < 16; ++reg) {
            const int pi = wave * 32 + (reg & 3) + 8 * (reg >> 2) + 4 * lk;
            const float bias = s_prm[3][pi], pa = s_prm[4][pi], pib = s_prm[5][pi];
            const int t = t0 + tq * 32 + li;
            if (t < a.L) {
                float v = acc2[reg] + bias;
                v = rs[reg] + v;
                const size_t oi = (size_t)pi * a.L + t;
                a.y[oi] = v;
                if (a.ya) a.ya[oi] = a.post_a ? snake_f(v, pa, pib) : v;
            }
        }
    }
}

static int conv_planes(int asked) { return asked == 2 ? 2 : 3; }

ConvPath resunit_pick(int C, int L, int dil, bool complete, bool ya_is_xa, int planes) {
    static const bool off = getenv("Q3_CONV_F32") != nullptr || getenv("Q3_CODEC_NO_UNIT_FUSE") != nullptr;
    static const bool fuse192 = getenv("Q3_CODEC_UNIT_FUSE_192") != nullptr;
    ConvPath p;
    p.refusal = hipErrorNotSupported;
    if (off || !complete || (C != 96 && !(C == 192 && fuse192)) || L < 4096 || (dil != 1 && dil != 3 && dil != 9) || ya_is_xa) return p;
    p.kernel = C == 96 ? CK_RESUNIT_3W : CK_RESUNIT_6W;
    p.co_m = 1; p.t_m = 4; p.wco = C / 32; p.wt = 1; p.cis = 32; p.np = conv_planes(planes);
    p.refusal = hipSuccess;
    return p;
}

hipError_t launch_resunit(const ResUnitArgs& r, hipStream_t st, int* path) {
    const ConvPath p = resunit_pick(r.C, r.L, r.dil, r.w1pk && r.w2pk && r.mid_a && r.xa && r.y, r.ya == r.xa, r.planes);
    if (path) *path = conv_path_code(p);
    if (p.kernel == CK_NONE) return p.refusal;
    ResUnitDev a{};
    a.xa = r.xa; a.y = r.y; a.ya = r.ya; a.w1pk = r.w1pk; a.w2pk = r.w2pk; a.b1 = r.b1; a.b2 = r.b2;
    a.mid_a = r.mid_a; a.mid_ib = r.mid_ib; a.post_a = r.post_a; a.post_ib = r.post_ib; a.C = r.C; a.L = r.L; a.dil = r.dil;
    const int W = 128 + 6 * r.dil;
    const int np = conv_planes(r.planes);
    const size_t lds_x = (size_t)np * W * 80, lds_mid = (size_t)np * 32 * (r.C * 2 + 16);
    const size_t lds = lds_x > lds_mid ? lds_x : lds_mid;
    const dim3 grid((r.L + 127) / 128);
    if (np == 2) {
        if (r.C == 96) hipLaunchKernelGGL((k_resunit_bf16x3<3, 2>), grid, dim3(192), lds, st, a);
        else hipLaunchKernelGGL((k_resunit_bf16x3<6, 2>), grid, dim3(384), lds, st, a);
    } else {
        if (r.C == 96) hipLaunchKernelGGL((k_resunit_bf16x3<3, 3>), grid, dim3(192), lds, st, a);
        else hipLaunchKernelGGL((k_resunit_bf16x3<6, 3>), grid, dim3(384), lds, st, a);
    }
    return hipGetLastError();
}

template <int W, int NP = 3>
__global__ __launch_bounds__(64 * W) void k_lin_small_bf16x3(ConvDev a) {
    __shared__ float part[W][16][64];
    constexpr int NR = 16 / W;
    const int tid = threadIdx.x, wave = tid >> 6, lane = tid & 63, li = lane & 31, lk = lane >> 5;
    const int co32 = blockIdx.x, co0 = co32 * 32;
    const int tc = (int)blockIdx.y * 32 + li;
    const cu32x4_t* __restrict__ wpk = reinterpret_cast<const cu32x4_t*>(a.wpk);
    const float* __restrict__ x = a.x;
    const int nc16 = a.cin >> 4, nseg = a.cin >> 7;
    const bool tok = tc < a.L;
    float tot[NR];
#pragma unroll
    for (int j = 0; j < NR; ++j) tot[j] = 0.0f;
    for (int s0 = 0; s0 < nseg; s0 += W) {
        const int seg = s0 + wave;
        if (seg < nseg) {
            cu32x4_t A[8][NP];
            float xv[8][8];
#pragma unroll
            for (int i = 0; i < 8; ++i) {
                const size_t tile = (size_t)co32 * nc16 + seg * 8 + i;
#pragma unroll
                for (int pl = 0; pl < NP; ++pl) A[i][pl] = wpk[(tile * 3 + pl) * 64 + lane];
            }
#pragma unroll
            for (int i = 0; i < 8; ++i)
#pragma unroll
                for (int e = 0; e < 8; ++e) {
                    const int ci = seg * 128 + i * 16 + lk * 8 + e;
                    xv[i][e] = tok ? x[(size_t)ci * a.L + tc] : 0.0f;
                }
            if (a.snake_a) {
#pragma unroll
                for (int i = 0; i < 8; ++i)
#pragma unroll
                    for (int e = 0; e < 8; ++e) {
                        const int ci = seg * 128 + i * 16 + lk * 8 + e;
                        if (tok) xv[i][e] = snake_f(xv[i][e], a.snake_a[ci], a.snake_ib[ci]);
                    }
            }
            f32x16_t acc;
#pragma unroll
            for (int r = 0; r < 16; ++r) acc[r] = 0.0f;
#pragma unroll
            for (int i = 0; i < 8; ++i) {
                cu32x4_t B[NP];
#pragma unroll
                for (int e = 0; e < 4; ++e) { uint32_t h, m, l; split3_pair(xv[i][2 * e], xv[i][2 * e + 1], h, m, l); B[0][e] = h; B[1][e] = m; if constexpr (NP == 3) B[2][e] = l; }
                acc = mfmaP<NP>(A[i], B, acc);
            }
#pragma unroll
            for (int r = 0; r < 16; ++r) part[wave][r][lane] = acc[r];
        }
        __syncthreads();
        const int n = (nseg - s0) < W ? (nseg - s0) : W;
#pragma unroll
        for (int j = 0; j < NR; ++j)
            for (int q = 0; q < n; ++q) tot[j] = tot[j] + part[q][wave + j * W][lane];
        __syncthreads();
    }
#pragma unroll
    for (int j = 0; j < NR; ++j) {
        const int reg = wave + j * W;
        const int o = co0 + (reg & 3) + 8 * (reg >> 2) + 4 * lk;
        if (o < a.cout && tok) {
            float v = tot[j] + (a.b ? a.b[o] : 0.0f);
            v = conv_act(v, a.act);
            if (a.scale) v = v * a.scale[o];
            const size_t oi = (size_t)o * a.oL + (size_t)tc * a.ostride + a.ooff;
            if (a.resid) v = a.resid[oi] + v;
            if (a.act == 2) v = fminf(fmaxf(v, -1.0f), 1.0f);
            if (a.post_a) {
                const float va = snake_f(v, a.post_a[o], a.post_ib[o]);
                if (a.y2) { a.y[oi] = v; a.y2[oi] = va; } else a.y[oi] = va;
            } else {
                a.y[oi] = v;
            }
        }
    }
}

template <int K, int CO_M, int T_M, int WCO, int WT, int NP>
static hipError_t launch_bf16x3_vp(const ConvPath& p, const ConvDev& a, int phases, hipStream_t st) {
    constexpr int CO_WG = 32 * CO_M * WCO, T_WG = 32 * T_M * WT;
    constexpr bool K1 = K == 1;
    constexpr int CIS1 = T_WG <= 64 ? 128 : 32;
    if ((p.cis != 32 && !(K1 && p.cis == CIS1)) || (!K1 && (p.pre || p.seg)) || (p.pre && CO_M != 1)) return hipErrorInvalidValue;
    const bool wide = p.cis > 32;
    const size_t lds = (size_t)NP * (T_WG + (K - 1) * a.dil) * (p.cis * 2 + 16);
    dim3 grid(((a.L + T_WG - 1) / T_WG) * (a.cout / CO_WG) * phases);
    ConvDev ap = a; ap.phases = phases;
    const bool segm = p.seg;
    const dim3 blk(64 * WCO * WT);
    if constexpr (K1) {
        const bool pre = p.pre;
#define Q3_CV(P, S, C) hipLaunchKernelGGL((k_conv_bf16x3<K, CO_M, T_M, WCO, WT, P, S, C, NP>), grid, blk, lds, st, ap)
        if (wide) {
            if (segm) { if (pre) Q3_CV(CO_M == 1, true, CIS1); else Q3_CV(false, true, CIS1); }
            else { if (pre) Q3_CV(CO_M == 1, false, CIS1); else Q3_CV(false, false, CIS1); }
        } else {
            if (segm) { if (pre) Q3_CV(CO_M == 1, true, 32); else Q3_CV(false, true, 32); }
            else { if (pre) Q3_CV(CO_M == 1, false, 32); else Q3_CV(false, false, 32); }
        }
#undef Q3_CV
    } else {
        hipLaunchKernelGGL((k_conv_bf16x3<K, CO_M, T_M, WCO, WT, false, false, 32, NP>), grid, blk, lds, st, ap);
    }
    return hipGetLastError();
}
static bool conv_two_plane_taps(int k) { return k == 1 || k == 2 || k == 7; }
template <int K, int CO_M, int T_M, int WCO, int WT>
static hipError_t launch_bf16x3_v(const ConvPath& p, const ConvDev& a, int phases, hipStream_t st) {
    if constexpr (K == 1 || K == 2 || K == 7)
        if (p.np == 2) return launch_bf16x3_vp<K, CO_M, T_M, WCO, WT, 2>(p, a, phases, st);
    if (p.np != 3) return hipErrorInvalidValue;
    return launch_bf16x3_vp<K, CO_M, T_M, WCO, WT, 3>(p, a, phases, st);
}
template <int K>
static hipError_t launch_bf16x3_k(const ConvPath& p, const ConvDev& a, int phases, hipStream_t st) {
    switch (p.kernel) {
        case CK_BF16X3_96x128_TM4: return launch_bf16x3_v<K, 1, 4, 3, 1>(p, a, phases, st);
        case CK_BF16X3_4Wx32x128: return launch_bf16x3_v<K, 1, 4, 4, 1>(p, a, phases, st);
        case CK_BF16X3_4Wx32x256: return launch_bf16x3_v<K, 1, 8, 4, 1>(p, a, phases, st);
        case CK_BF16X3_64x128: return launch_bf16x3_v<K, 1, 2, 2, 2>(p, a, phases, st);
        case CK_BF16X3_64x64: return launch_bf16x3_v<K, 1, 1, 2, 2>(p, a, phases, st);
        case CK_BF16X3_128x128: return launch_bf16x3_v<K, 2, 2, 2, 2>(p, a, phases, st);
        case CK_BF16X3_96x128_6W: return launch_bf16x3_v<K, 1, 2, 3, 2>(p, a, phases, st);
        default: return hipErrorInvalidValue;
    }
}
static int conv_pick_geometry(int K, int cout, int L, int phases, bool has_resid) {
    const long big_tiles = (long)((L + 127) / 128) * (cout / 128) * phases;
    static const int geo = [] { const char* e = getenv("Q3_CONV_TM4"); return e ? atoi(e) : 2; }();
    if (geo && K >= 2 && L >= 4096 && (cout == 192 || cout == 96)) return CK_BF16X3_96x128_TM4;
    if (geo >= 2 && K >= 2 && L >= 4096 && cout % 128 == 0 && big_tiles >= 192) {
        if (geo == 2) return CK_BF16X3_4Wx32x128;
        if (geo == 3) return CK_BF16X3_4Wx32x256;
    }
    if (K == 1 && has_resid && cout % 64 == 0 && cout != 96 && big_tiles >= 192) return CK_BF16X3_64x128;
    {
        static const int pw = [] { const char* e = getenv("Q3_CONV_PW1_GEO"); return e ? atoi(e) : 2; }();
        if (pw && K == 1 && !has_resid && cout % 128 == 0 && big_tiles >= 192 && big_tiles < 1024) {
            if (pw == 1) return CK_BF16X3_64x128;
            return CK_BF16X3_64x64;
        }
    }
    if (cout % 128 == 0 && big_tiles >= 192) return CK_BF16X3_128x128;
    if (cout == 192) return CK_BF16X3_96x128_6W;
    if (cout == 96) return CK_BF16X3_96x128_6W;
    if (cout % 64 == 0) return CK_BF16X3_64x64;
    return CK_NONE;
}
static bool conv_pick_bf16x3(ConvPath& p, int cout, int cin, int L, int k, int phases, bool packed, bool has_resid, int np) {
    static const bool off = getenv("Q3_CONV_F32") != nullptr;
    if (off || !packed || cin % 16 || cout % 32) return false;
    static const bool no_small = getenv("Q3_CONV_NO_SMALL") != nullptr;
    static const bool no_small_tiles = getenv("Q3_CONV_NO_SMALL_TILES") != nullptr;
    const long small_wgs = (long)(cout / 32) * ((L + 31) / 32);
    const bool small_tiles = L > 32 && cin >= 1024 && small_wgs <= 512 && !no_small_tiles;
    if (conv_segmented(k, cin) && (L <= 32 || small_tiles) && phases == 1 && cout % 64 == 0 && !no_small) {
        p.kernel = cin >= 1024 ? CK_LIN_SMALL_8W : CK_LIN_SMALL_4W;
        p.co_m = 1; p.t_m = 1; p.wco = 1; p.wt = 1; p.seg = true; p.np = np;
        return true;
    }
    if (k != 1 && k != 2 && k != 3 && k != 5 && k != 7) return false;
    const int g = conv_pick_geometry(k, cout, L, phases, has_resid);
    if (g == CK_NONE) return false;
    static const int GEO[7][4] = {{1, 4, 3, 1}, {1, 4, 4, 1}, {1, 8, 4, 1}, {1, 2, 2, 2}, {1, 1, 2, 2}, {2, 2, 2, 2}, {1, 2, 3, 2}};
    const int* q = GEO[g - CK_BF16X3_96x128_TM4];
    p.kernel = g; p.co_m = q[0]; p.t_m = q[1]; p.wco = q[2]; p.wt = q[3];
    p.np = conv_two_plane_taps(k) ? np : 3;
    p.cis = 32;
    if (k == 1) {
        static const bool cis32 = getenv("Q3_CONV_CIS32") != nullptr;
        const int cis1 = 32 * p.t_m * p.wt <= 64 ? 128 : 32;
        if (cis1 > 32 && !cis32 && cin >= 2 * cis1) p.cis = cis1;
        p.seg = conv_segmented(k, cin);
        p.pre = p.co_m == 1 && has_resid;
    }
    return true;
}

ConvPath conv_pick(int cout, int cin, int L, int k, int dil, int phases, bool packed, bool has_resid, int planes, bool aligned16, bool transposed) {
    ConvPath p;
    if (k < 1 || k > CV_MAXK || (k - 1) * dil > CV_MAXHALO || L <= 0 || cout < 1 || cin < 1 || phases < 1) { p.refusal = hipErrorInvalidValue; return p; }
    if (cout == 1 && !transposed) {
        p.kernel = (k == 7 && dil == 1 && L % 4 == 0 && aligned16) ? CK_OUT1_V4 : CK_OUT1;
        return p;
    }
    if (conv_pick_bf16x3(p, cout, cin, L, k, phases, packed, has_resid, conv_planes(planes))) return p;
    if (conv_pick_mfma(p, cout, k)) return p;
    p.kernel = CK_VALU;
    return p;
}

int conv_path_code(const ConvPath& p) {
    return p.kernel | (p.pre ? CP_PRE : 0) | (p.seg ? CP_SEG : 0) | (p.cis == 128 ? CP_CIS128 : 0) | (p.np == 2 ? CP_NP2 : 0);
}
const char* conv_path_name(int code) {
    static const char* const KN[CK_COUNT] = {
        "none", "k_conv_out1", "k_conv_out1_v4", "k_lin_small_bf16x3<4>", "k_lin_small_bf16x3<8>",
        "k_conv_bf16x3<96co x 128t, 3 waves, T_M=4>", "k_conv_bf16x3<4 waves x 32co x 128t>", "k_conv_bf16x3<4 waves x 32co x 256t>",
        "k_conv_bf16x3<64co x 128t>", "k_conv_bf16x3<64co x 64t>", "k_conv_bf16x3<128co x 128t>", "k_conv_bf16x3<96co x 128t, 6 waves>",
        "k_conv1d_mfma<CO_W=2>", "k_conv1d_mfma<CO_W=1>", "k_conv1d", "k_resunit_bf16x3<3>", "k_resunit_bf16x3<6>"};
    static thread_local char buf[96];
    const int k = code & CP_KERNEL_MASK;
    if (code < 0 || k >= CK_COUNT || (code & ~(CP_KERNEL_MASK | CP_PRE | CP_SEG | CP_CIS128 | CP_NP2))) return "invalid";
    snprintf(buf, sizeof buf, "%s%s%s%s%s", KN[k], (code & CP_PRE) ? " PRE" : "", (code & CP_SEG) ? " SEG" : "", (code & CP_CIS128) ? " CIS=128" : "",
             (code & CP_NP2) ? " NP=2" : "");
    return buf;
}

__global__ __launch_bounds__(256) void k_conv_out1(ConvDev a) {
    const int t = blockIdx.x * 256 + threadIdx.x;
    if (t >= a.L) return;
    float acc = 0.0f;
    for (int c = 0; c < a.cin; ++c) {
        const float sa = a.snake_a ? a.snake_a[c] : 0.0f, sib = a.snake_a ? a.snake_ib[c] : 0.0f;
        for (int kk = 0; kk < a.k; ++kk) {
            const int ts = t - (a.k - 1 - kk) * a.dil;
            if (ts < 0) continue;
            float v = a.x[(size_t)c * a.L + ts];
            if (a.snake_a) v = snake_f(v, sa, sib);
            acc = fmaf(a.w[(size_t)c * a.k + kk], v, acc);
        }
    }
    float v = acc + (a.b ? a.b[0] : 0.0f);
    if (a.act == 2) v = fminf(fmaxf(v, -1.0f), 1.0f);
    a.y[t] = v;
}

__global__ __launch_bounds__(256) void k_conv_out1_v4(ConvDev a) {
    const int t = (blockIdx.x * 256 + threadIdx.x) * 4;
    if (t >= a.L) return;
    float acc[4] = {0.0f, 0.0f, 0.0f, 0.0f};
    for (int c = 0; c < a.cin; ++c) {
        const float* xr = a.x + (size_t)c * a.L + t;
        const float4 z = make_float4(0.f, 0.f, 0.f, 0.f);
        const float4 p0 = t >= 8 ? *reinterpret_cast<const float4*>(xr - 8) : z;
        const float4 p1 = t >= 4 ? *reinterpret_cast<const float4*>(xr - 4) : z;
        const float4 p2 = *reinterpret_cast<const float4*>(xr);
        float v[12] = {p0.x, p0.y, p0.z, p0.w, p1.x, p1.y, p1.z, p1.w, p2.x, p2.y, p2.z, p2.w};
        if (a.snake_a) {
            const float sa = a.snake_a[c], sib = a.snake_ib[c];
#pragma unroll
            for (int i = 2; i < 12; ++i) v[i] = snake_f(v[i], sa, sib);
        }
        float w[7];
#pragma unroll
        for (int kk = 0; kk < 7; ++kk) w[kk] = a.w[(size_t)c * 7 + kk];
#pragma unroll
        for (int j = 0; j < 4; ++j)
#pragma unroll
            for (int kk = 0; kk < 7; ++kk) acc[j] = fmaf(w[kk], v[j + kk + 2], acc[j]);
    }
    float o[4];
#pragma unroll
    for (int j = 0; j < 4; ++j) {
        float v = acc[j] + (a.b ? a.b[0] : 0.0f);
        if (a.act == 2) v = fminf(fmaxf(v, -1.0f), 1.0f);
        o[j] = v;
    }
    *reinterpret_cast<float4*>(a.y + t) = make_float4(o[0], o[1], o[2], o[3]);
}

static hipError_t launch_conv_path(const ConvPath& p, const ConvDev& a, int phases, hipStream_t st) {
    switch (p.kernel) {
        case CK_NONE: return p.refusal != hipSuccess ? p.refusal : hipErrorInvalidValue;
        case CK_OUT1_V4: hipLaunchKernelGGL(k_conv_out1_v4, dim3((a.L / 4 + 255) / 256), dim3(256), 0, st, a); break;
        case CK_OUT1: hipLaunchKernelGGL(k_conv_out1, dim3((a.L + 255) / 256), dim3(256), 0, st, a); break;
        case CK_LIN_SMALL_4W:
        case CK_LIN_SMALL_8W: {
            const dim3 grid(a.cout / 32, (a.L + 31) / 32);
            if (p.np == 2) {
                if (p.kernel == CK_LIN_SMALL_8W) hipLaunchKernelGGL((k_lin_small_bf16x3<8, 2>), grid, dim3(512), 0, st, a);
                else hipLaunchKernelGGL((k_lin_small_bf16x3<4, 2>), grid, dim3(256), 0, st, a);
            } else {
                if (p.kernel == CK_LIN_SMALL_8W) hipLaunchKernelGGL((k_lin_small_bf16x3<8, 3>), grid, dim3(512), 0, st, a);
                else hipLaunchKernelGGL((k_lin_small_bf16x3<4, 3>), grid, dim3(256), 0, st, a);
            }
            break;
        }
        case CK_MFMA_F32_64:
        case CK_MFMA_F32_32: return launch_conv_mfma(p, a, phases, st);
        case CK_VALU: {
            dim3 grid((a.L + CV_T - 1) / CV_T, (a.cout + CV_CO - 1) / CV_CO, phases);
            hipLaunchKernelGGL(k_conv1d, grid, dim3(256), 0, st, a);
            break;
        }
        default:
            switch (a.k) {
                case 1: return launch_bf16x3_k<1>(p, a, phases, st);
                case 2: return launch_bf16x3_k<2>(p, a, phases, st);
                case 3: return launch_bf16x3_k<3>(p, a, phases, st);
                case 5: return launch_bf16x3_k<5>(p, a, phases, st);
                case 7: return launch_bf16x3_k<7>(p, a, phases, st);
                default: return hipErrorInvalidValue;
            }
    }
    return hipGetLastError();
}

hipError_t launch_conv1d(const ConvArgs& c, hipStream_t st, int* path) {
    const ConvPath p = conv_pick(c.cout, c.cin, c.L, c.k, c.dil, 1, c.wpk != nullptr, c.resid != nullptr, c.planes,
                                 (((uintptr_t)c.x | (uintptr_t)c.y) & 15) == 0, false);
    if (path) *path = conv_path_code(p);
    if (p.kernel == CK_NONE) return p.refusal;
    ConvDev a{};
    a.x = c.x; a.w = c.w; a.b = c.b; a.y = c.y; a.cin = c.cin; a.cout = c.cout; a.L = c.L; a.k = c.k; a.dil = c.dil;
    a.snake_a = c.snake_a; a.snake_ib = c.snake_b; a.resid = c.resid; a.scale = c.scale; a.act = c.act;
    a.ostride = 1; a.ooff = 0; a.oL = c.L; a.w_phase_stride = 0; a.ooff_phase = 0;
    a.post_a = c.post_a; a.post_ib = c.post_ib; a.y2 = c.y2;
    a.wpk = c.wpk; a.wpk_phase_stride = 0; a.planes = conv_planes(c.planes);
    return launch_conv_path(p, a, 1, st);
}

hipError_t launch_transconv1d_taps(const float* x, const float* wp, const float* b, float* y, int cin, int cout, int L,
                                   int stride, int taps, const float* snake_a, const float* snake_ib, hipStream_t st,
                                   const float* post_a, const float* post_ib, float* y2, const void* wpk, int planes, int* path) {
    const ConvPath p = conv_pick(cout, cin, L, taps, 1, stride, wpk != nullptr, false, planes, false, true);
    if (path) *path = conv_path_code(p);
    if (p.kernel == CK_NONE) return p.refusal;
    ConvDev a{};
    a.planes = conv_planes(planes);
    a.wpk = wpk; a.wpk_phase_stride = packed_conv_w_bytes(cout, cin, taps) / 16;
    a.post_a = post_a; a.post_ib = post_ib; a.y2 = y2;
    a.x = x; a.w = wp; a.b = b; a.y = y; a.cin = cin; a.cout = cout; a.L = L; a.k = taps; a.dil = 1;
    a.snake_a = snake_a; a.snake_ib = snake_ib; a.resid = nullptr; a.scale = nullptr; a.act = 0;
    a.ostride = stride; a.ooff = 0; a.oL = L * stride;
    a.w_phase_stride = (size_t)cout * cin * taps; a.ooff_phase = 1;
    return launch_conv_path(p, a, stride, st);
}

void transconv_phase_weights(const float* w, int cin, int cout, int k, int stride, float* out) {
    const int taps = k / stride;
    for (int ph = 0; ph < stride; ++ph)
        for (int co = 0; co < cout; ++co)
            for (int ci = 0; ci < cin; ++ci)
                for (int tp = 0; tp < taps; ++tp) {
                    const int kk = ph + (taps - 1 - tp) * stride;
                    out[(((size_t)ph * cout + co) * cin + ci) * taps + tp] = w[((size_t)ci * cout + co) * k + kk];
                }
}

__global__ __launch_bounds__(256) void k_dwconv7(const float* x, const float* w, const float* b, float* y, int L) {
    const int c = blockIdx.y, t = blockIdx.x * 256 + threadIdx.x;
    if (t >= L) return;
    const float* xr = x + (size_t)c * L;
    float acc = 0.0f;
#pragma unroll
    for (int kk = 0; kk < 7; ++kk) {
        const int ts = t - 6 + kk;
        if (ts >= 0) acc = fmaf(w[c * 7 + kk], xr[ts], acc);
    }
    y[(size_t)c * L + t] = acc + b[c];
}
hipError_t launch_dwconv7(const float* x, const float* w, const float* b, float* y, int C, int L, hipStream_t st) {
    hipLaunchKernelGGL(k_dwconv7, dim3((L + 255) / 256, C), dim3(256), 0, st, x, w, b, y, L);
    return hipGetLastError();
}

template <bool LAYERNORM>
__global__ __launch_bounds__(256) void k_norm_c(const float* __restrict__ x, const float* __restrict__ w, const float* __restrict__ b,
                                                float* __restrict__ y, int C, int L, float eps) {
    __shared__ float s1[8][32], s2[8][32];
    const int tx = threadIdx.x & 31, cg = threadIdx.x >> 5;
    const int t = blockIdx.x * 32 + tx;
    float a = 0.0f, q = 0.0f;
    if (t < L) {
        int c = cg;
        for (; c + 56 < C; c += 64) {
            float v[8];
#pragma unroll
            for (int u = 0; u < 8; ++u) v[u] = x[(size_t)(c + 8 * u) * L + t];
#pragma unroll
            for (int u = 0; u < 8; ++u) { a += v[u]; q += v[u] * v[u]; }
        }
        for (; c < C; c += 8) { const float v = x[(size_t)c * L + t]; a += v; q += v * v; }
    }
    s1[cg][tx] = a; s2[cg][tx] = q;
    __syncthreads();
    float sum = 0.0f, sq = 0.0f;
#pragma unroll
    for (int g = 0; g < 8; ++g) { sum += s1[g][tx]; sq += s2[g][tx]; }
    if (t >= L) return;
    if (LAYERNORM) {
        const float mean = sum / (float)C, var = sq / (float)C - mean * mean;
        const float inv = 1.0f / sqrtf(var + eps);
#pragma unroll 8
        for (int c = cg; c < C; c += 8) y[(size_t)c * L + t] = (x[(size_t)c * L + t] - mean) * inv * w[c] + b[c];
    } else {
        const float den = sqrtf(sq / (float)C + eps);
#pragma unroll 8
        for (int c = cg; c < C; c += 8) y[(size_t)c * L + t] = x[(size_t)c * L + t] / den * w[c];
    }
}
template <bool LAYERNORM, int CPT>
__global__ __launch_bounds__(256) void k_norm_c2(const float* __restrict__ x, const float* __restrict__ w, const float* __restrict__ b,
                                                 float* __restrict__ y, int C, int L, float eps) {
    __shared__ float s1[16][16], s2[16][16];
    const int tx = threadIdx.x & 15, cg = threadIdx.x >> 4;
    const int t = blockIdx.x * 16 + tx;
    const bool in = t < L;
    float v[CPT];
#pragma unroll
    for (int u = 0; u < CPT; ++u) v[u] = in ? x[(size_t)(cg + 16 * u) * L + t] : 0.0f;
    float wv[CPT], bv[LAYERNORM ? CPT : 1];
#pragma unroll
    for (int u = 0; u < CPT; ++u) { wv[u] = w[cg + 16 * u]; if (LAYERNORM) bv[u] = b[cg + 16 * u]; }
    float a = 0.0f, q = 0.0f;
#pragma unroll
    for (int u = 0; u < CPT; ++u) { a += v[u]; q += v[u] * v[u]; }
    s1[cg][tx] = a; s2[cg][tx] = q;
    __syncthreads();
// ... 331 lines not shown
```

qwen3_tts_rs_amd/csrc/q3_session.hip:

```cpp
#include "q3_engine.h"
#include "q3_prefix_cache.h"

hipError_t sync_frames(q3_session* s) {
    if (s->aql) {
        std::string why;
        if (!q3::aql_wait(s->aql, &why)) { s->aql_failed = true; set_err(Q3_HIP_ERROR, "AQL frame submission: %s", why.c_str()); return hipErrorUnknown; }
    }
    return hipStreamSynchronize(s->stream);
}

static hipError_t run_linear(q3_session* s, const LinArgs& a_in) {
    LinArgs a = a_in;
    a.ws = s->wide_ws; a.ws_bytes = s->wide_ws_bytes;
#ifdef Q3_TRACE
    a.trace = s->trace_next(0, a.M, a.N, a.K, a.epi, a.norm_w ? 1 : 0, a.tiled);
#endif
    if (!s->profile) return launch_linear(a, s->stream);
    hipEvent_t e0, e1;
    if (s->prof_pool_next + 2 <= s->prof_pool.size()) { e0 = s->prof_pool[s->prof_pool_next++]; e1 = s->prof_pool[s->prof_pool_next++]; }
    else {
        hipError_t e = hipEventCreate(&e0); if (e != hipSuccess) return e;
        e = hipEventCreate(&e1); if (e != hipSuccess) return e;
        s->prof_pool.push_back(e0); s->prof_pool.push_back(e1); s->prof_pool_next = s->prof_pool.size();
    }
// ... 1624 lines not shown
        }
        if (a <= 0) continue;
        if (s->stream_mode == 1 && !q.icl) {
            if (!s->cstream) Q3C(codec_stream_create(s->m, s->B, s->max_frames, s->stream, &s->cstream));
            if (codec_stream_pos(s->cstream, b) > q.stream_pos) codec_stream_reset(s->cstream, b);
            const int sp = codec_stream_pos(s->cstream, b);
            pushes.push_back({b, q.stream_pos + a - sp, q.stream_pos - sp, nullptr, s->codes + ((size_t)b * s->max_frames + sp) * 16,
                              pcm_host ? pcm_host[b] : nullptr});
        } else {
            Q3C(chunk_decode_row(s, b, a, pcm_host ? pcm_host[b] : nullptr, cap ? cap[b] : 0, nullptr));
        }
    }
    if (!pushes.empty()) Q3C(codec_stream_push(s->cstream, pushes));
    for (int b = 0; b < s->B; ++b) {
        SeqInfo& q = s->seq[b];
        q.stream_pos += avail[(size_t)b];
        done[b] = held[(size_t)b] ? 0 : (avail[(size_t)b] <= 0 || (q.done && q.stream_pos >= q.n_frames)) ? 1 : 0;
    }
    return Q3_OK;
}

extern "C" q3_status q3_session_frames(q3_session* s, int b, int* n_frames, int* done) {
    if (!s || b < 0 || b >= s->B) return set_err(Q3_INVALID_ARG, "bad sequence index");
    HIPC(hipSetDevice(s->m->device));
    Q3C(refresh_codes(s));
    if (n_frames) *n_frames = s->seq[b].n_frames;
    if (done) *done = s->seq[b].done ? 1 : 0;
    return Q3_OK;
}

extern "C" q3_status q3_session_codes(q3_session* s, int b, uint32_t* codes_host, int cap_frames, int* n_frames) {
    if (!s || b < 0 || b >= s->B) return set_err(Q3_INVALID_ARG, "bad sequence index");
    HIPC(hipSetDevice(s->m->device));
    Q3C(refresh_codes(s));
    const int n = s->seq[b].n_frames;
    if (n_frames) *n_frames = n;
    if (codes_host) {
        if (cap_frames < n) return set_err(Q3_INVALID_ARG, "codes buffer too small (%d < %d frames)", cap_frames, n);
        memcpy(codes_host, &s->codes_host[(size_t)b * s->max_frames * 16], (size_t)n * 16 * 4);
    }
    return Q3_OK;
}

static q3_status decode_range_on(q3_session* s, int b, int f0, int f1, hipStream_t st, float* pcm_host, size_t cap, size_t* n_samples) {
    const int T = f1 - f0, spf = samples_per_frame(s->m->cfg);
    if (n_samples) *n_samples = (size_t)T * spf;
    if (T == 0) return Q3_OK;
    Q3C(codec_reserve(s->m, s->cws, T));
    HIPC(hipMemcpyAsync(s->cws.frames, s->codes + ((size_t)b * s->max_frames + f0) * 16, (size_t)T * 16 * 4, hipMemcpyDeviceToDevice, st));
    Q3C(codec_decode_dev(s->m, s->cws, T, st, nullptr));
    HIPC(hipStreamSynchronize(st));
    if (pcm_host) {
        if (cap < (size_t)T * spf) return set_err(Q3_INVALID_ARG, "pcm buffer too small");
        HIPC(q3_hipMemcpy(pcm_host, s->cws.pcm, (size_t)T * spf * 4, hipMemcpyDeviceToHost));
    }
    return Q3_OK;
}

extern "C" q3_status q3_session_decode(q3_session* s, int b, int f0, int f1, float* pcm_host, size_t cap, size_t* n_samples) {
    if (!s || b < 0 || b >= s->B) return set_err(Q3_INVALID_ARG, "bad sequence index");
    HIPC(hipSetDevice(s->m->device));
    Q3C(refresh_codes(s));
    if (f0 < 0 || f1 < f0 || f1 > s->seq[b].n_frames) return set_err(Q3_INVALID_ARG, "bad frame range [%d,%d) of %d", f0, f1, s->seq[b].n_frames);
    const int T = f1 - f0, spf = samples_per_frame(s->m->cfg);
    const SeqInfo& q = s->seq[b];
    if (!q.ref_codes.empty() && s->prefilled && f0 == 0 && f1 == q.n_frames) {
        const int n_ref = (int)(q.ref_codes.size() / 16), total = n_ref + T;
        const size_t all = (size_t)total * spf, cut = (size_t)n_ref * all / (size_t)(total > 0 ? total : 1);
        if (n_samples) *n_samples = all - cut;
        Q3C(codec_reserve(s->m, s->cws, total));
        HIPC(hipMemcpyAsync(s->cws.frames, q.ref_codes.data(), (size_t)n_ref * 16 * 4, hipMemcpyHostToDevice, s->stream));
        if (T > 0) HIPC(hipMemcpyAsync(s->cws.frames + (size_t)n_ref * 16, s->codes + (size_t)b * s->max_frames * 16, (size_t)T * 16 * 4, hipMemcpyDeviceToDevice, s->stream));
        Q3C(codec_decode_dev(s->m, s->cws, total, s->stream, nullptr));
        HIPC(sync_frames(s));
        if (pcm_host) {
            if (cap < all - cut) return set_err(Q3_INVALID_ARG, "pcm buffer too small");
            HIPC(q3_hipMemcpy(pcm_host, s->cws.pcm + cut, (all - cut) * 4, hipMemcpyDeviceToHost));
        }
        return Q3_OK;
    }
    return decode_range_on(s, b, f0, f1, s->stream, pcm_host, cap, n_samples);
}

extern "C" q3_status q3_session_run(q3_session* s, int use_graph, float** pcm_host, const size_t* cap, size_t* n_samples, q3_timing* timing) {
    if (!s) return set_err(Q3_INVALID_ARG, "null session");
    if (any_open_text(s)) return set_err(Q3_UNSUPPORTED, "q3_session_run: a row's text is still open (q3_session_append_text with last != 0 closes it; or drive the session with q3_session_generate)");
    using clk = std::chrono::steady_clock;
    auto ms = [](clk::time_point a, clk::time_point b) { return std::chrono::duration<double, std::milli>(b - a).count(); };
    const auto t0 = clk::now();
    s->precapture = use_graph != 0;
    Q3C(q3_session_prefill(s));
    const auto t1 = clk::now();
    const int overlap_env = [] { const char* e = getenv("Q3_DECODE_OVERLAP"); return e ? atoi(e) : 0; }();
    static const int seg_env = [] { const char* e = getenv("Q3_DECODE_SEG"); const int v = e ? atoi(e) : 128; return v < 16 ? 16 : v; }();
    bool overlap = overlap_env != 0 && !s->debug && !s->profile && s->max_frames > seg_env;
    for (auto& q : s->seq) if (!q.ref_codes.empty()) overlap = false;
    const int spf = samples_per_frame(s->m->cfg);
    if (!overlap) {
        Q3C(q3_session_generate(s, s->max_frames, use_graph));
        Q3C(refresh_codes(s));
        const auto t2 = clk::now();
        int total = 0;
        static const int conc = [] { const char* e = getenv("Q3_DECODE_PAIRS"); const int v = e ? atoi(e) : 2; return v < 1 ? 1 : (v > 8 ? 8 : v); }();
        bool any_icl = false;
        for (auto& q : s->seq) any_icl = any_icl || !q.ref_codes.empty();
        if (conc > 1 && s->B > 1 && !any_icl) {
            while ((int)s->par_ws.size() < conc - 1) {
                s->par_ws.emplace_back();
                hipStream_t st = nullptr;
                HIPC(hipStreamCreateWithFlags(&st, hipStreamNonBlocking));
                s->par_streams.push_back(st);
            }
            auto ws_of = [&](int k) -> CodecWS& { return k == 0 ? s->cws : s->par_ws[(size_t)k - 1]; };
            auto st_of = [&](int k) { return k == 0 ? s->stream : s->par_streams[(size_t)k - 1]; };
            if (pcm_host)
                for (int b = 0; b < s->B; ++b)
                    if (pcm_host[b] && s->seq[b].n_frames && (!cap || cap[b] < (size_t)s->seq[b].n_frames * spf)) return set_err(Q3_INVALID_ARG, "pcm buffer too small");
            for (int b0 = 0; b0 < s->B; b0 += conc) {
                const int nb = (s->B - b0) < conc ? (s->B - b0) : conc;
                for (int k = 0; k < nb; ++k) {
                    const int b = b0 + k, T = s->seq[b].n_frames;
                    if (n_samples) n_samples[b] = (size_t)T * spf;
                    total += T;
                    if (T == 0) continue;
                    Q3C(codec_reserve(s->m, ws_of(k), T));
                    HIPC(hipMemcpyAsync(ws_of(k).frames, s->codes + (size_t)b * s->max_frames * 16, (size_t)T * 16 * 4, hipMemcpyDeviceToDevice, st_of(k)));
                    Q3C(codec_decode_dev(s->m, ws_of(k), T, st_of(k), nullptr));
                    if (pcm_host && pcm_host[b])
                        HIPC(hipMemcpyAsync(pcm_host[b], ws_of(k).pcm, (size_t)T * spf * 4, hipMemcpyDeviceToHost, st_of(k)));
                }
                for (int k = 0; k < nb; ++k) HIPC(hipStreamSynchronize(st_of(k)));
            }
        } else
        for (int b = 0; b < s->B; ++b) {
            size_t n = 0;
            Q3C(q3_session_decode(s, b, 0, s->seq[b].n_frames, pcm_host ? pcm_host[b] : nullptr, cap ? cap[b] : 0, &n));
            if (n_samples) n_samples[b] = n;
            total += s->seq[b].n_frames;
        }
        const auto t3 = clk::now();
        if (timing) { timing->prefill_ms = ms(t0, t1); timing->generation_ms = ms(t1, t2); timing->decode_ms = ms(t2, t3); timing->generation_frames = total; }
        return Q3_OK;
    }
    HIPC(hipSetDevice(s->m->device));
    static const int cus = [] { const char* e = getenv("Q3_DECODE_CUS"); const int v = e ? atoi(e) : 0; return v <= 0 ? 0 : (v < 8 ? 8 : (v > 248 ? 248 : v & ~7)); }();
    if (!s->dec_stream) {
        if (cus) {
            uint32_t mask[8] = {0, 0, 0, 0, 0, 0, 0, 0};
            for (int i = 256 - cus; i < 256; ++i) mask[i >> 5] |= 1u << (i & 31);
            HIPC(hipExtStreamCreateWithCUMask(&s->dec_stream, 8, mask));
        } else {
            int least = 0, greatest = 0;
            HIPC(hipDeviceGetStreamPriorityRange(&least, &greatest));
            HIPC(hipStreamCreateWithPriority(&s->dec_stream, hipStreamNonBlocking, least));
        }
    }
    Q3C(codec_reserve(s->m, s->seg_ws, seg_env + CODEC_CTX_FRAMES, s->max_frames));
    struct Split {
        q3::AqlProgram* p = nullptr;
        void release() { if (p) { std::string why; q3::aql_restrict_cus(p, 0, &why); p = nullptr; } }
        ~Split() { release(); }
    } split;
    if (cus && s->aql && !s->aql_failed) { std::string why; if (q3::aql_restrict_cus(s->aql, 256 - cus, &why)) split.p = s->aql; }
    std::vector<int> dec_pos((size_t)s->B, 0);
    std::thread worker; q3_status wst = Q3_OK; std::string werr;
    auto join = [&]() -> q3_status {
        if (worker.joinable()) worker.join();
        if (wst != Q3_OK) return set_err(wst, "%s", werr.c_str());
        return Q3_OK;
    };
    struct Job { int b, a, e; };
    auto seg_enqueue = [s, spf, pcm_host, cap](const Job& j, CodecWS& ws, hipStream_t st) -> q3_status {
        const int c0 = j.a > CODEC_CTX_FRAMES ? j.a - CODEC_CTX_FRAMES : 0;
        if (pcm_host && pcm_host[j.b] && (!cap || cap[j.b] < (size_t)j.e * spf)) return set_err(Q3_INVALID_ARG, "pcm buffer too small");
        HIPC(hipMemcpyAsync(ws.frames, s->codes + (size_t)j.b * s->max_frames * 16, (size_t)j.e * 16 * 4, hipMemcpyDeviceToDevice, st));
        Q3C(codec_decode_dev(s->m, ws, j.e, st, nullptr, c0));
        if (pcm_host && pcm_host[j.b])
            HIPC(hipMemcpyAsync(pcm_host[j.b] + (size_t)j.a * spf, ws.pcm + (size_t)(j.a - c0) * spf, (size_t)(j.e - j.a) * spf * 4, hipMemcpyDeviceToHost, st));
        return Q3_OK;
    };
    auto collect = [&](bool final_pass) {
        std::vector<Job> jobs;
        for (int b = 0; b < s->B; ++b) {
            const SeqInfo& q = s->seq[b];
            const int e = (q.done || final_pass) ? q.n_frames : (q.n_frames < s->frames_run ? q.n_frames : s->frames_run);
            if (e > dec_pos[(size_t)b] && (final_pass || q.done || e - dec_pos[(size_t)b] >= 16)) {
                for (int a = dec_pos[(size_t)b]; a < e; a += seg_env) jobs.push_back({b, a, a + seg_env < e ? a + seg_env : e});
                dec_pos[(size_t)b] = e;
            }
        }
        return jobs;
    };
    auto dispatch = [&]() -> q3_status {
        std::vector<Job> jobs = collect(false);
        if (jobs.empty()) return Q3_OK;
        Q3C(join());
        worker = std::thread([s, jobs, seg_enqueue, &wst, &werr]() {
            if (hipSetDevice(s->m->device) != hipSuccess) { wst = Q3_HIP_ERROR; werr = "hipSetDevice failed in the decode thread"; return; }
            for (const Job& j : jobs) {
                const q3_status st = seg_enqueue(j, s->seg_ws, s->dec_stream);
                if (st != Q3_OK) { wst = st; werr = q3_last_error(); return; }
            }
        });
        return Q3_OK;
    };
    static const int tail_env = [] { const char* e = getenv("Q3_DECODE_TAIL"); const int v = e ? atoi(e) : 32; return v < 16 ? 16 : v; }();
    q3_status st = Q3_OK;
    while (st == Q3_OK && session_remaining(s) > 0 && !all_done(s)) {
        int n = seg_env;
        const int left = session_remaining(s);
        if (left > tail_env && left - n < tail_env) n = left - tail_env;
        st = q3_session_generate(s, n, use_graph);
        if (st == Q3_OK) st = refresh_codes(s);
        if (st == Q3_OK && session_remaining(s) > 0 && !all_done(s)) st = dispatch();
    }
    const auto t2 = clk::now();
    split.release();
    { const q3_status js = join(); if (st == Q3_OK) st = js; }
    if (st != Q3_OK) { hipStreamSynchronize(s->dec_stream); return st; }
    {
        const int conc = 2;
        auto ws_of = [&](int k) -> CodecWS& { return k == 0 ? s->cws : s->par_ws[(size_t)k - 1]; };
        auto st_of = [&](int k) { return k == 0 ? s->stream : s->par_streams[(size_t)k - 1]; };
        auto tail = [&]() -> q3_status {
            std::vector<Job> jobs = collect(true);
            while ((int)s->par_ws.size() < conc - 1) {
                hipStream_t pst = nullptr;
                HIPC(hipStreamCreateWithFlags(&pst, hipStreamNonBlocking));
                s->par_ws.emplace_back(); s->par_streams.push_back(pst);
            }
            for (int k = 0; k < conc; ++k) Q3C(codec_reserve(s->m, ws_of(k), seg_env + CODEC_CTX_FRAMES, s->max_frames));
            for (size_t i = 0; i < jobs.size(); ++i) Q3C(seg_enqueue(jobs[i], ws_of((int)(i % conc)), st_of((int)(i % conc))));
            return Q3_OK;
        };
        st = tail();
        hipError_t he = hipStreamSynchronize(s->dec_stream);
        for (int k = 0; k < conc && k <= (int)s->par_streams.size(); ++k) { const hipError_t e2 = hipStreamSynchronize(st_of(k)); if (he == hipSuccess) he = e2; }
        if (st != Q3_OK) return st;
        HIPC(he);
    }
    int total = 0;
    for (int b = 0; b < s->B; ++b) {
        if (n_samples) n_samples[b] = (size_t)s->seq[b].n_frames * spf;
        total += s->seq[b].n_frames;
    }
    const auto t3 = clk::now();
    if (timing) { timing->prefill_ms = ms(t0, t1); timing->generation_ms = ms(t1, t2); timing->decode_ms = ms(t2, t3); timing->generation_frames = total; }
    return Q3_OK;
}

extern "C" q3_status q3_session_set_stream_mode(q3_session* s, int mode) {
    if (!s || (mode != 0 && mode != 1)) return set_err(Q3_INVALID_ARG, "q3_session_set_stream_mode: mode must be 0 (context-free) or 1 (continuous)");
    s->stream_mode = mode;
    return Q3_OK;
}

extern "C" q3_status q3_session_next_chunk(q3_session* s, float* pcm_host, size_t cap, size_t* n_samples, int* done) {
    if (!s) return set_err(Q3_INVALID_ARG, "null session");
    if (s->B != 1) return set_err(Q3_UNSUPPORTED, "streaming sessions are batch 1 (StreamingSession, lib.rs:1484)");
    if (!s->prefilled) { s->precapture = true; Q3C(q3_session_prefill(s)); }
    Q3C(refresh_codes(s));
    SeqInfo& q = s->seq[0];
    const int chunk = s->opts.chunk_frames > 0 ? s->opts.chunk_frames : 10;
    while (!q.done && q.n_frames - s->stream_pos < chunk && session_remaining(s) > 0) {
        int need = chunk - (q.n_frames - s->stream_pos);
        Q3C(q3_session_generate(s, need, 1));
        Q3C(refresh_codes(s));
    }
    int avail = q.n_frames - s->stream_pos;
    if (avail > chunk) avail = chunk;
    if (q.opened && !q.done && avail < chunk) { if (n_samples) *n_samples = 0; if (done) *done = 0; return Q3_OK; }
    if (avail <= 0) { if (n_samples) *n_samples = 0; if (done) *done = 1; return Q3_OK; }
    const bool chunk_done = q.done && s->stream_pos + avail >= q.n_frames;
    static const bool no_ahead = getenv("Q3_STREAM_NO_AHEAD") != nullptr;
    int ahead = 0;
    if (!no_ahead && !q.done && (s->aql || s->graph_exec) && !s->aql_failed && !s->debug && !s->profile) {
        ahead = chunk - (q.n_frames - (s->stream_pos + avail));
        if (ahead > session_remaining(s)) ahead = session_remaining(s);
        if (ahead < 0) ahead = 0;
    }
    const bool first = s->stream_pos == 0;
    auto launch_ahead = [&]() -> q3_status {
        Q3C(kv_reserve_frames(s, ahead));
        if (s->aql) HIPC(hipStreamSynchronize(s->stream));
        return frames_enqueue(s, ahead);
    };
    hipStream_t dst = s->stream;
    if (ahead > 0 && !first) {
        if (!s->dec_stream) HIPC(hipStreamCreateWithFlags(&s->dec_stream, hipStreamNonBlocking));
        Q3C(launch_ahead());
        dst = s->dec_stream;
    }
    const int spf = samples_per_frame(s->m->cfg);
    const float* src = nullptr;
    if (s->stream_mode == 1 && !q.icl) {
        const int a0 = s->stream_pos, e = s->stream_pos + avail;
        const int c0 = a0 > CODEC_CTX_FRAMES ? a0 - CODEC_CTX_FRAMES : 0;
        Q3C(codec_reserve(s->m, s->cws, chunk + CODEC_CTX_FRAMES, s->max_frames));
        HIPC(hipMemcpyAsync(s->cws.frames, s->codes, (size_t)e * 16 * 4, hipMemcpyDeviceToDevice, dst));
        Q3C(codec_decode_dev(s->m, s->cws, e, dst, nullptr, c0));
        src = s->cws.pcm + (size_t)(a0 - c0) * spf;
    } else {
        Q3C(codec_reserve(s->m, s->cws, avail));
        HIPC(hipMemcpyAsync(s->cws.frames, s->codes + (size_t)s->stream_pos * 16, (size_t)avail * 16 * 4, hipMemcpyDeviceToDevice, dst));
        Q3C(codec_decode_dev(s->m, s->cws, avail, dst, nullptr));
        src = s->cws.pcm;
    }
    if (ahead > 0 && first) {
        if (!s->dec_ev) HIPC(hipEventCreateWithFlags(&s->dec_ev, hipEventDisableTiming));
        HIPC(hipEventRecord(s->dec_ev, s->stream));
        Q3C(launch_ahead());
        HIPC(hipEventSynchronize(s->dec_ev));
    } else {
        HIPC(hipStreamSynchronize(dst));
    }
    if (n_samples) *n_samples = (size_t)avail * spf;
    if (pcm_host) {
        if (cap < (size_t)avail * spf) return set_err(Q3_INVALID_ARG, "pcm buffer too small");
        HIPC(q3_hipMemcpy(pcm_host, src, (size_t)avail * spf * 4, hipMemcpyDeviceToHost));
    }
    s->stream_pos += avail;
    if (done) *done = chunk_done ? 1 : 0;
    return Q3_OK;
}

extern "C" q3_status q3_session_get(q3_session* s, int what, int b, void* out, size_t bytes) {
    if (!s || !out || b < 0 || b >= s->B) return set_err(Q3_INVALID_ARG, "bad argument");
    const q3_config& c = s->m->cfg;
    HIPC(hipSetDevice(s->m->device));
    HIPC(sync_frames(s));
// ... 36 lines not shown
```

qwen3_tts_rs_amd/csrc/q3_testapi.hip:

```cpp
#include "q3_engine.h"

extern "C" q3_status q3_talker_step(q3_session* s, const float* embeds_host, float* hidden_host, float* logits_host) {
    if (!s || !embeds_host) return set_err(Q3_INVALID_ARG, "null argument");
    if (!s->prefilled) return set_err(Q3_INVALID_ARG, "session not prefilled");
    const q3_config& c = s->m->cfg;
    HIPC(hipSetDevice(s->m->device));
    std::vector<int> posv(s->B);
    HIPC(sync_frames(s));
    HIPC(q3_hipMemcpy(posv.data(), s->pos, s->B * 4, hipMemcpyDeviceToHost));
    for (int p : posv) if (p >= s->max_seq) return set_err(Q3_KV_OVERFLOW, "KV cache full (%d)", s->max_seq);
    for (int b = 0; b < s->B; ++b) Q3C(kv_reserve_row(s, b, posv[(size_t)b] + 1));
    HIPC(hipMemcpyAsync(s->tb.X, embeds_host, (size_t)s->B * c.hidden * 4, hipMemcpyHostToDevice, s->stream));
    Q3C(talker_step(s, s->pos, 0, true));
    HIPC(sync_frames(s));
    for (int& p : posv) p += 1;
    HIPC(q3_hipMemcpy(s->pos, posv.data(), s->B * 4, hipMemcpyHostToDevice));
    if (hidden_host) HIPC(q3_hipMemcpy(hidden_host, s->LASTH, (size_t)s->B * c.hidden * 4, hipMemcpyDeviceToHost));
    if (logits_host) HIPC(q3_hipMemcpy(logits_host, s->LOGITS, (size_t)s->B * c.codec_vocab * 4, hipMemcpyDeviceToHost));
    return Q3_OK;
}

extern "C" q3_status q3_cp_generate(q3_session* s, const float* last_hidden_host, const float* sem_embed_host,
                                    uint32_t* codes15_host, float* cp_logits_host) {
    if (!s || !last_hidden_host || !codes15_host) return set_err(Q3_INVALID_ARG, "null argument");
// ... 483 lines not shown
        if (e == hipSuccess && p->n_splits > 1) e = launch_attn_merge(t, 0);
    } else if (variant == 1) {
        e = launch_qknorm_rope_kv(t, 0);
        if (e == hipSuccess) e = launch_attn_decode(t, 0);
        if (e == hipSuccess) e = launch_attn_merge(t, 0);
    } else if (variant == 2) e = launch_attn_cp(t, 0);
    else e = launch_attn_first2(t, 0);
    if (e == hipErrorInvalidValue || e == hipErrorNotSupported) {
        (void)hipGetLastError();
        (void)q3_hipDeviceSynchronize();
        return set_err(Q3_UNSUPPORTED, "q3_attn_step_ex: the launcher refused variant=%d layout=%d nh=%d nkv=%d splits=%d rows_per_seq=%d (%s)", variant, layout, nh, nkv,
                       p->n_splits, rps, hipGetErrorString(e));
    }
    HIPC(e);
    HIPC(q3_hipDeviceSynchronize());
    HIPC(q3_hipMemcpy(p->out, out, (size_t)B * QD * 4, hipMemcpyDeviceToHost));
    if (layout != 0) {
        std::vector<std::vector<uint32_t>> got;
        HIPC(slabs.download(got));
        each_row([&](int slot, size_t elem, float* row) { slabs.get_row(got, slot, elem, row); slabs.copy_row(slabs.img, got, slot, elem); });
        slabs.strays(got, p->stray);
    } else {
        HIPC(q3_hipMemcpy(p->kcache, kv, cn * 4, hipMemcpyDeviceToHost)); HIPC(q3_hipMemcpy(p->vcache, kv + cn, cn * 4, hipMemcpyDeviceToHost));
        if (p->stray) { p->stray[0] = 0; p->stray[1] = -1; }
    }
    if (t.g_x) HIPC(q3_hipMemcpy(p->g_x, t.g_x, gx_rows * p->g_ldx * 4, hipMemcpyDeviceToHost));
    if (t.g_codes) HIPC(q3_hipMemcpy(p->g_codes, t.g_codes, (size_t)B * p->g_max_frames * 16 * 4, hipMemcpyDeviceToHost));
    if (t.zero) HIPC(q3_hipMemcpy(p->zero_buf, t.zero, zn * 4, hipMemcpyDeviceToHost));
    return Q3_OK;
}

extern "C" q3_status q3_kv_pages_to_bf16_ex(int device, int n_layers, int nkv, int n_pages, const int* src_slots, const int* dst_slots,
                                            const float* src, uint16_t* dst, int* rot_used, long long* stray) {
    if (!src_slots || !dst_slots || !src || !dst || !stray) return set_err(Q3_INVALID_ARG, "q3_kv_pages_to_bf16_ex: null argument");
    if (n_layers < 1 || n_layers > 4 || nkv < 1 || nkv > 8 || n_pages < 1 || n_pages > KvPool::SLAB_SLOTS)
        return set_err(Q3_INVALID_ARG, "q3_kv_pages_to_bf16_ex: bad shape (n_layers 1..4, nkv 1..8, n_pages 1..%d)", KvPool::SLAB_SLOTS);
    if (!slots_ok(src_slots, n_pages, KvPool::SLAB_SLOTS) || !slots_ok(dst_slots, n_pages, KvPool::SLAB_SLOTS))
        return set_err(Q3_INVALID_ARG, "q3_kv_pages_to_bf16_ex: the slots of a list must be distinct slots of 0 .. %d", KvPool::SLAB_SLOTS - 1);
    HIPC(hipSetDevice(device));
    DevPool pool;
    TestSlabs a, b;
    a.shape(n_layers, nkv, 4); b.shape(n_layers, nkv, 2);
    HIPC(a.add_slab(pool)); HIPC(b.add_slab(pool));
    a.fill_pattern(); b.fill_pattern();
    auto each_row = [&](auto&& f) {
        for (int pg = 0; pg < n_pages; ++pg) for (int l = 0; l < n_layers; ++l) for (int v = 0; v < 2; ++v) for (int g = 0; g < nkv; ++g) for (int pp = 0; pp < KV_PAGE_POS; ++pp)
            f(pg, l, v, g, pp, (((((size_t)pg * n_layers + l) * 2 + v) * nkv + g) * KV_PAGE_POS + pp) * HEAD_DIM);
    };
    each_row([&](int pg, int l, int v, int g, int pp, size_t at) { a.put_row(a.img, src_slots[pg], a.row_elem(src_slots[pg], l, v, g, pp), src + at); });
    HIPC(a.upload()); HIPC(b.upload());
    std::vector<unsigned long long> lists((size_t)2 * n_pages);
    for (int pg = 0; pg < n_pages; ++pg) { lists[(size_t)pg] = a.page(src_slots[pg]); lists[(size_t)n_pages + pg] = b.page(dst_slots[pg]); }
    if (rot_used)
        for (int pg = 0; pg < n_pages; ++pg) for (int g = 0; g < nkv; ++g) {
            rot_used[(size_t)pg * nkv + g] = kv_rot(lists[(size_t)pg], g);
            rot_used[((size_t)n_pages + pg) * nkv + g] = kv_rot(lists[(size_t)n_pages + pg], g);
        }
    unsigned long long* dl; HIPC(pool.alloc(&dl, lists.size()));
    HIPC(q3_hipMemcpy(dl, lists.data(), lists.size() * 8, hipMemcpyHostToDevice));
    HIPC(q3_hipDeviceSynchronize());
    HIPC(launch_kv_pages_to_bf16(dl, dl + n_pages, n_pages, n_layers, nkv, a.geo.layer_stride(), a.geo.v_delta(), 0));
    HIPC(q3_hipDeviceSynchronize());
    std::vector<std::vector<uint32_t>> got;
    HIPC(b.download(got));
    std::vector<float> row((size_t)HEAD_DIM);
    each_row([&](int pg, int l, int v, int g, int pp, size_t at) {
        const size_t elem = b.row_elem(dst_slots[pg], l, v, g, pp);
        b.get_row(got, dst_slots[pg], elem, row.data());
        for (int dd = 0; dd < HEAD_DIM; ++dd) { uint32_t u; memcpy(&u, &row[(size_t)dd], 4); dst[at + dd] = (uint16_t)(u >> 16); }
        b.copy_row(b.img, got, dst_slots[pg], elem);
    });
    b.strays(got, stray);
    return Q3_OK;
}

extern "C" int q3_conv_path(int cout, int cin, int L, int k, int dil, int phases, int packed, int has_resid, int planes, int aligned16) {
    return conv_path_code(conv_pick(cout, cin, L, k, dil, phases, packed != 0, has_resid != 0, planes, aligned16 != 0, phases > 1));
}
extern "C" int q3_resunit_path(int C, int L, int dil, int packed, int ya_is_xa, int planes) {
    return conv_path_code(resunit_pick(C, L, dil, packed != 0, ya_is_xa != 0, planes));
}
extern "C" const char* q3_conv_path_name(int code) { return conv_path_name(code); }

extern "C" q3_status q3_conv_ex(int device, const q3_conv_ex_args* p) {
    if (!p || !p->x || !p->w || !p->y) return set_err(Q3_INVALID_ARG, "q3_conv_ex: null argument");
    if (p->path) *p->path = 0;
    const int kind = p->kind, cin = p->cin, cout = p->cout, L = p->L, k = p->k, dil = p->dil;
    if (kind < 0 || kind > 2) return set_err(Q3_INVALID_ARG, "q3_conv_ex: kind 0..2");
    if (cin < 1 || cin > 8192 || cout < 1 || cout > 8192 || L < 1 || L > (1 << 22) || k < 1 || k > 64 || dil < 1 || dil > 64 || p->act < 0 || p->act > 6)
        return set_err(Q3_INVALID_ARG, "q3_conv_ex: bad shape (channels 1..8192, L 1..2^22, k 1..64, dil 1..64, act 0..6)");
    const int stride = kind == 1 ? p->stride : 1;
    if (kind == 1 && (stride < 1 || stride > 16 || k % stride)) return set_err(Q3_INVALID_ARG, "q3_conv_ex: transposed conv needs 1 <= stride <= 16 and k %% stride == 0");
    const int taps = k / stride;
    if (kind == 2 && (cin != cout || k != 7 || !p->w2 || !p->mid_a || !p->mid_ib)) return set_err(Q3_INVALID_ARG, "q3_conv_ex: residual unit needs cin == cout, k == 7, w2 and the middle snake pair");
    if (!p->snake_a != !p->snake_b || !p->post_a != !p->post_ib || !p->mid_a != !p->mid_ib) return set_err(Q3_INVALID_ARG, "q3_conv_ex: half a snake pair");
    if (kind != 0 && (p->resid || p->resid_in_place || p->scale || p->act)) return set_err(Q3_INVALID_ARG, "q3_conv_ex: resid / scale / act belong to kind 0");
    if (kind != 0 && kind != 2 && p->y2_is_x) return set_err(Q3_INVALID_ARG, "q3_conv_ex: y2_is_x belongs to kind 2");
    if ((p->resid && p->resid_in_place) || (p->y2 && p->y2_is_x)) return set_err(Q3_INVALID_ARG, "q3_conv_ex: two residuals / two y2");
    const size_t out_n = (size_t)cout * L * stride, xn = (size_t)cin * L, wn = (size_t)cout * cin * k;
    if (p->y_front < 0 || p->y_front % 4 || p->y_elems < 0 || (size_t)p->y_elems < (size_t)p->y_front + out_n)
        return set_err(Q3_INVALID_ARG, "q3_conv_ex: y must hold y_front (a multiple of 4) + cout * L * stride floats");
    HIPC(hipSetDevice(device));
    DevPool pool;
    float *x, *w, *w2 = nullptr, *b = nullptr, *b2 = nullptr, *res = nullptr, *scale = nullptr, *y, *y2 = nullptr;
    void *wpk = nullptr, *w2pk = nullptr;
    HIPC(pool.alloc(&x, xn)); HIPC(q3_hipMemcpy(x, p->x, xn * 4, hipMemcpyHostToDevice));
    HIPC(pool.alloc(&w, wn));
    if (kind == 1) {
        std::vector<float> wp(wn);
        transconv_phase_weights(p->w, cin, cout, k, stride, wp.data());
        HIPC(q3_hipMemcpy(w, wp.data(), wn * 4, hipMemcpyHostToDevice));
    } else HIPC(q3_hipMemcpy(w, p->w, wn * 4, hipMemcpyHostToDevice));
    if (kind == 2) { HIPC(pool.alloc(&w2, (size_t)cout * cin)); HIPC(q3_hipMemcpy(w2, p->w2, (size_t)cout * cin * 4, hipMemcpyHostToDevice)); }
    auto vec = [&](const float* h, int n, float** d) -> q3_status {
        *d = nullptr;
        if (!h) return Q3_OK;
        HIPC(pool.alloc(d, (size_t)n)); HIPC(q3_hipMemcpy(*d, h, (size_t)n * 4, hipMemcpyHostToDevice));
        return Q3_OK;
    };
    auto pair = [&](const float* ha, const float* hb, int n, float** da, float** db) -> q3_status {
        Q3C(vec(ha, n, da)); Q3C(vec(hb, n, db));
        if (ha && p->snake_raw) {
            float *ta, *tb;
            HIPC(pool.alloc(&ta, (size_t)n)); HIPC(pool.alloc(&tb, (size_t)n));
            HIPC(launch_snake_tables(*da, *db, ta, tb, n, 0));
            *da = ta; *db = tb;
        }
        return Q3_OK;
    };
    float *sa, *sb, *pa, *pb, *ma, *mb;
    Q3C(vec(p->b, cout, &b)); Q3C(vec(p->b2, cout, &b2)); Q3C(vec(p->scale, cout, &scale)); Q3C(vec(p->resid, (int)out_n, &res));
    Q3C(pair(p->snake_a, p->snake_b, cin, &sa, &sb)); Q3C(pair(p->post_a, p->post_ib, cout, &pa, &pb)); Q3C(pair(p->mid_a, p->mid_ib, cout, &ma, &mb));
    const size_t yn = (size_t)p->y_elems;
    HIPC(pool.alloc(&y, yn)); HIPC(q3_hipMemcpy(y, p->y, yn * 4, hipMemcpyHostToDevice));
    if (p->y2) { HIPC(pool.alloc(&y2, yn)); HIPC(q3_hipMemcpy(y2, p->y2, yn * 4, hipMemcpyHostToDevice)); }
    float* yr = y + p->y_front; float* y2r = y2 ? y2 + p->y_front : nullptr;
    if (p->packed) {
        const int pk = kind == 1 ? taps : k;
        if (cout % 32 || cin % 16 || pk < 1) return set_err(Q3_UNSUPPORTED, "q3_conv_ex: cout %d / cin %d cannot be packed (cout %% 32, cin %% 16)", cout, cin);
        const size_t per = packed_conv_w_bytes(cout, cin, pk);
        char* d; HIPC(pool.alloc(&d, per * (size_t)stride)); wpk = d;
        for (int ph = 0; ph < stride; ++ph) HIPC(launch_pack_conv_w(w + (size_t)ph * cout * cin * pk, d + (size_t)ph * per, cout, cin, pk, 0));
        if (kind == 2) {
            char* d2; HIPC(pool.alloc(&d2, packed_conv_w_bytes(cout, cin, 1))); w2pk = d2;
            HIPC(launch_pack_conv_w(w2, d2, cout, cin, 1, 0));
        }
    }
    HIPC(q3_hipDeviceSynchronize());
    hipError_t e;
    int path = 0;
    if (kind == 0) {
        ConvArgs a;
        a.x = x; a.w = w; a.b = b; a.y = yr; a.cin = cin; a.cout = cout; a.L = L; a.k = k; a.dil = dil;
        a.snake_a = sa; a.snake_b = sb; a.resid = p->resid_in_place ? yr : res; a.scale = scale; a.act = p->act;
        a.post_a = pa; a.post_ib = pb; a.y2 = y2r; a.wpk = wpk; a.planes = p->planes;
        e = launch_conv1d(a, 0, &path);
    } else if (kind == 1) {
        e = launch_transconv1d_taps(x, w, b, yr, cin, cout, L, stride, taps, sa, sb, 0, pa, pb, y2r, wpk, p->planes, &path);
    } else {
        ResUnitArgs r{};
        r.xa = x; r.y = yr; r.ya = p->y2_is_x ? x : y2r; r.w1pk = wpk; r.w2pk = w2pk; r.b1 = b; r.b2 = b2;
        r.mid_a = ma; r.mid_ib = mb; r.post_a = pa; r.post_ib = pb; r.C = cout; r.L = L; r.dil = dil; r.planes = p->planes;
        e = launch_resunit(r, 0, &path);
    }
    if (p->path) *p->path = path;
    if (e == hipErrorInvalidValue || e == hipErrorNotSupported) {
        (void)hipGetLastError();
        return set_err(Q3_UNSUPPORTED, "q3_conv_ex: the launcher refused kind=%d cin=%d cout=%d L=%d k=%d dil=%d stride=%d packed=%d planes=%d (%s)", kind, cin, cout,
                       L, k, dil, stride, p->packed, p->planes, hipGetErrorString(e));
    }
    HIPC(e);
    HIPC(q3_hipDeviceSynchronize());
    HIPC(q3_hipMemcpy(p->y, y, yn * 4, hipMemcpyDeviceToHost));
    if (y2) HIPC(q3_hipMemcpy(p->y2, y2, yn * 4, hipMemcpyDeviceToHost));
    return Q3_OK;
}

static q3_status check_cl_out(const char* who, const void* x, const void* w, const void* y, int C, int L, int y_front, int y_elems) {
    if (!x || !w || !y) return set_err(Q3_INVALID_ARG, "%s: null argument", who);
    if (C < 1 || C > 8192 || L < 1 || L > (1 << 22)) return set_err(Q3_INVALID_ARG, "%s: bad shape (C 1..8192, L 1..2^22)", who);
    if (y_front < 0 || y_elems < 0 || (size_t)y_elems < (size_t)y_front + (size_t)C * L) return set_err(Q3_INVALID_ARG, "%s: y must hold y_front + C * L floats", who);
    return Q3_OK;
}

extern "C" q3_status q3_norm_c(int device, int layernorm, const float* x_host, const float* w_host, const float* b_host, int C, int L, float eps,
                               float* y_host, int y_front, int y_elems) {
    Q3C(check_cl_out("q3_norm_c", x_host, w_host, y_host, C, L, y_front, y_elems));
    if (layernorm && !b_host) return set_err(Q3_INVALID_ARG, "q3_norm_c: LayerNorm needs a bias");
    HIPC(hipSetDevice(device));
    DevPool pool;
    float *x, *w, *b = nullptr, *y;
    const size_t n = (size_t)C * L;
    HIPC(pool.alloc(&x, n)); HIPC(pool.alloc(&w, (size_t)C)); HIPC(pool.alloc(&y, (size_t)y_elems));
    HIPC(q3_hipMemcpy(x, x_host, n * 4, hipMemcpyHostToDevice)); HIPC(q3_hipMemcpy(w, w_host, (size_t)C * 4, hipMemcpyHostToDevice));
    HIPC(q3_hipMemcpy(y, y_host, (size_t)y_elems * 4, hipMemcpyHostToDevice));
    if (layernorm) { HIPC(pool.alloc(&b, (size_t)C)); HIPC(q3_hipMemcpy(b, b_host, (size_t)C * 4, hipMemcpyHostToDevice)); }
    HIPC(q3_hipDeviceSynchronize());
    if (layernorm) HIPC(launch_layernorm_c(x, w, b, y + y_front, C, L, eps, 0));
    else HIPC(launch_rmsnorm_c(x, w, y + y_front, C, L, eps, 0));
    HIPC(q3_hipDeviceSynchronize());
    HIPC(q3_hipMemcpy(y_host, y, (size_t)y_elems * 4, hipMemcpyDeviceToHost));
    return Q3_OK;
}

extern "C" q3_status q3_dwconv7(int device, const float* x_host, const float* w_host, const float* b_host, int C, int L, float* y_host, int y_front,
                                int y_elems) {
    Q3C(check_cl_out("q3_dwconv7", x_host, w_host, y_host, C, L, y_front, y_elems));
    if (!b_host) return set_err(Q3_INVALID_ARG, "q3_dwconv7: null argument");
    HIPC(hipSetDevice(device));
    DevPool pool;
    float *x, *w, *b, *y;
    const size_t n = (size_t)C * L;
    HIPC(pool.alloc(&x, n)); HIPC(pool.alloc(&w, (size_t)C * 7)); HIPC(pool.alloc(&b, (size_t)C)); HIPC(pool.alloc(&y, (size_t)y_elems));
    HIPC(q3_hipMemcpy(x, x_host, n * 4, hipMemcpyHostToDevice)); HIPC(q3_hipMemcpy(w, w_host, (size_t)C * 7 * 4, hipMemcpyHostToDevice));
    HIPC(q3_hipMemcpy(b, b_host, (size_t)C * 4, hipMemcpyHostToDevice)); HIPC(q3_hipMemcpy(y, y_host, (size_t)y_elems * 4, hipMemcpyHostToDevice));
    HIPC(q3_hipDeviceSynchronize());
    HIPC(launch_dwconv7(x, w, b, y + y_front, C, L, 0));
    HIPC(q3_hipDeviceSynchronize());
    HIPC(q3_hipMemcpy(y_host, y, (size_t)y_elems * 4, hipMemcpyDeviceToHost));
    return Q3_OK;
}

static hipError_t fill_ff(void* dev, size_t bytes) {
    std::vector<unsigned char> h(bytes, 0xFF);
    return q3_hipMemcpy(dev, h.data(), bytes, hipMemcpyHostToDevice);
}
static void gemm_path_out(const GemmPick& p, int* path) {
    if (!path) return;
    path[0] = p.geometry; path[1] = p.geometry == GEMM_G3 ? p.k_ranges : 1; path[2] = p.geometry == GEMM_G3 ? p.k_split : 1;
    path[3] = p.geometry == GEMM_G2 ? p.n_split : 1;
}
static size_t gemm_ex_ws_bytes(int M, int N, int Kpad, int epi) {
    if (Kpad % 128 || (Kpad >> 6) % 16) return 0;
    return (size_t)8 * (epi == EPI_SWIGLU ? 2 : 1) * M * N * sizeof(float);
}

extern "C" int q3_gemm_path(int M, int N, int K, int epi, int norm, int w2, int planes, int* path) {
    if (path) path[0] = path[1] = path[2] = path[3] = 0;
    if (M < 1 || N < 1 || K < 4) return -1;
    static float dummy[4];
    GemmArgs g;
    g.W = reinterpret_cast<const uint16_t*>(dummy); g.W2 = w2 ? g.W : nullptr; g.x = dummy; g.ldx = up32(K); g.y = dummy; g.ldy = N;
    g.norm_w = norm ? dummy : nullptr; g.den = norm ? dummy : nullptr;
    g.M = M; g.N = N; g.K = K; g.Kpad = up32(K); g.epi = epi;
    if (planes) { g.xp = g.W; g.xp_plane = (size_t)up128(M) * g.Kpad; g.splitk_ws_bytes = gemm_ex_ws_bytes(M, N, g.Kpad, epi); g.splitk_ws = g.splitk_ws_bytes ? dummy : nullptr; }
    if (g.K % 4 || g.N % 64 || (planes && K % 8)) return -1;
    const bool rms = norm != 0;
    if (epi < EPI_NONE || epi > EPI_SWIGLU || ((epi == EPI_RESID || epi == EPI_SILU) && rms) || (epi == EPI_SWIGLU && (!rms || !w2))) return -1;
    const GemmPick p = lm_gemm_pick(g);
    gemm_path_out(p, path);
    return p.geometry;
}

extern "C" q3_status q3_gemm_ex(int device, const q3_gemm_ex_args* p) {
    if (!p || !p->x || !p->w || !p->y) return set_err(Q3_INVALID_ARG, "q3_gemm_ex: null argument");
    if (p->path) p->path[0] = p->path[1] = p->path[2] = p->path[3] = 0;
    const int M = p->M, N = p->N, K = p->K;
    if (M < 1 || M > 8192 || N < 1 || N > 16384 || K < 4 || K > 16384) return set_err(Q3_INVALID_ARG, "q3_gemm_ex: bad shape (M 1..8192, N 1..16384, K 4..16384)");
// ... 1034 lines not shown
```

Baseline: 2842.

## Cap codec conv occupancy by padding dynamic LDS during overlapped decode

Adds a 'resident' setting that pads the dynamic LDS of the bf16x3 conv and resunit kernels, raising the max-dynamic-shared attribute where needed, so only a bounded number of workgroups fit on each CU. The overlapped decode thread uses this by default (Q3_DECODE_RESIDENT=1), so codec decode takes fewer CU resources while talker frame generation runs at the same time. It also adds env-tunable segment and tail sizes, join-wait timing, optional logging and a test entry point. The risk is that the decode kernels themselves run slower because of lower occupancy.

```diff
diff --git a/include/q3tts.h b/include/q3tts.h
--- a/include/q3tts.h
+++ b/include/q3tts.h
@@ -247,6 +247,7 @@
     float* y; float* y2;
 } q3_conv_ex_args;
 q3_status q3_conv_ex(int device, const q3_conv_ex_args* args);
+q3_status q3_test_conv_resident(int device, const q3_conv_ex_args* args, int resident, int* lds_bytes);
 int q3_gemm_path(int M, int N, int K, int epi, int norm, int w2, int planes, int* path);
 typedef struct q3_gemm_ex_args {
     int M, N, K, ldx, ldy, ldr, M_alloc;
diff --git a/qwen3_tts_rs_amd/_lib.py b/qwen3_tts_rs_amd/_lib.py
--- a/qwen3_tts_rs_amd/_lib.py
+++ b/qwen3_tts_rs_amd/_lib.py
@@ -305,6 +305,7 @@
     "q3_resunit_path": (c_int, [c_int] * 6),
     "q3_conv_path_name": (c_char_p, [c_int]),
     "q3_conv_ex": (c_int, [c_int, P(CConvEx)]),
+    "q3_test_conv_resident": (c_int, [c_int, P(CConvEx), c_int, P(ctypes.c_int32)]),
     "q3_gemm_path": (c_int, [c_int] * 7 + [P(ctypes.c_int32)]),
     "q3_gemm_ex": (c_int, [c_int, P(CGemmEx)]),
     "q3_attn_prefill_path": (c_int, [c_int] * 4 + [P(ctypes.c_int32)]),
diff --git a/qwen3_tts_rs_amd/api.py b/qwen3_tts_rs_amd/api.py
--- a/qwen3_tts_rs_amd/api.py
+++ b/qwen3_tts_rs_amd/api.py
@@ -2103,7 +2103,7 @@
             post=None, mid=None, resid: Optional[np.ndarray] = None, resid_in_place: bool = False, scale: Optional[np.ndarray] = None,
             act: int = 0, planes: int = 3, packed: bool = True, snake_raw: bool = False, w2: Optional[np.ndarray] = None,
             b2: Optional[np.ndarray] = None, y: Optional[np.ndarray] = None, y2: Optional[np.ndarray] = None, y_front: int = 0,
-            y2_is_x: bool = False, device: int = 0):
+            y2_is_x: bool = False, device: int = 0, resident: Optional[int] = None):
     f = lambda a: np.ascontiguousarray(a, dtype=np.float32)
     x = f(x); w = f(w)
     assert x.ndim == 2 and w.ndim == 3
@@ -2137,12 +2137,16 @@
     for (na, nb, pr, n) in (("snake_a", "snake_b", snake, cin), ("post_a", "post_ib", post, cout), ("mid_a", "mid_ib", mid, cout)):
         if pr is not None:
             opt(na, pr[0], n); opt(nb, pr[1], n)
+    lds = ctypes.c_int32(0)
     try:
-        check(lib.q3_conv_ex(device, ctypes.byref(a)))
+        if resident is None:
+            check(lib.q3_conv_ex(device, ctypes.byref(a)))
+        else:
+            check(lib.q3_test_conv_resident(device, ctypes.byref(a), int(resident), ctypes.byref(lds)))
     except _lib.Q3Error as e:
         e.path = path.value
         raise
-    return y, y2, path.value
+    return (y, y2, path.value) if resident is None else (y, y2, path.value, lds.value)
 
 
 def norm_c(x: np.ndarray, w: np.ndarray, b: Optional[np.ndarray] = None, eps: float = 1e-6, y: Optional[np.ndarray] = None,
diff --git a/qwen3_tts_rs_amd/csrc/q3_codec_run.hip b/qwen3_tts_rs_amd/csrc/q3_codec_run.hip
--- a/qwen3_tts_rs_amd/csrc/q3_codec_run.hip
+++ b/qwen3_tts_rs_amd/csrc/q3_codec_run.hip
@@ -112,23 +112,25 @@
 static thread_local const q3_model* tl_codec_model = nullptr;
 static const void* packed_of(const float* w) { return tl_codec_model ? tl_codec_model->pk(w) : nullptr; }
 static thread_local int tl_codec_planes = 3;
-CodecScope::CodecScope(const q3_model* m) {
+static thread_local int tl_codec_resident = 0;
+CodecScope::CodecScope(const q3_model* m, int resident_) {
     static const int env_planes = [] { const char* e = getenv("Q3_CODEC_PLANES"); const int v = e ? atoi(e) : 0; return (v == 2 || v == 3) ? v : 0; }();
     planes = env_planes ? env_planes : m->codec_planes;
-    tl_codec_model = m; tl_codec_planes = planes;
-}
-CodecScope::~CodecScope() { tl_codec_planes = 3; }
+    resident = resident_ < 0 ? 0 : resident_;
+    tl_codec_model = m; tl_codec_planes = planes; tl_codec_resident = resident;
+}
+CodecScope::~CodecScope() { tl_codec_planes = 3; tl_codec_resident = 0; }
 static hipError_t conv1(const float* x, const float* w, const float* b, float* y, int cin, int cout, int L, hipStream_t st,
                         const float* resid = nullptr, const float* scale = nullptr, int act = 0,
                         const float* sa = nullptr, const float* sib = nullptr) {
     ConvArgs a; a.x = x; a.w = w; a.b = b; a.y = y; a.cin = cin; a.cout = cout; a.L = L; a.k = 1; a.dil = 1;
-    a.resid = resid; a.scale = scale; a.act = act; a.snake_a = sa; a.snake_b = sib; a.wpk = packed_of(w); a.planes = tl_codec_planes;
+    a.resid = resid; a.scale = scale; a.act = act; a.snake_a = sa; a.snake_b = sib; a.wpk = packed_of(w); a.planes = tl_codec_planes; a.resident = tl_codec_resident;
     return launch_conv1d(a, st);
 }
 static hipError_t convk(const float* x, const float* w, const float* b, float* y, int cin, int cout, int L, int k, int dil,
                         hipStream_t st, const float* sa = nullptr, const float* sib = nullptr, int act = 0) {
     ConvArgs a; a.x = x; a.w = w; a.b = b; a.y = y; a.cin = cin; a.cout = cout; a.L = L; a.k = k; a.dil = dil;
-    a.snake_a = sa; a.snake_b = sib; a.act = act; a.wpk = packed_of(w); a.planes = tl_codec_planes;
+    a.snake_a = sa; a.snake_b = sib; a.act = act; a.wpk = packed_of(w); a.planes = tl_codec_planes; a.resident = tl_codec_resident;
     return launch_conv1d(a, st);
 }
 
@@ -193,7 +195,7 @@
     return Q3_OK;
 }
 q3_status codec_stack_dev(const q3_model* m, CodecWS& ws, float* cur, int L, hipStream_t st, float** taps, const CodecScope& scope) {
-    const int NPL = scope.planes;
+    const int NPL = scope.planes, RES = scope.resident;
     const q3_config& c = m->cfg;
     const int LAT = c.dec_latent;
     auto TAP = [&](int id, const float* dev, size_t n) -> q3_status { return tap_out(taps, id, dev, n, st); };
@@ -201,7 +203,7 @@
     for (int i = 0; i < 2; ++i) {
         const UpW& U = m->up[i];
         float* upo = (cur == C) ? A : C;
-        HIPC(launch_transconv1d_taps(cur, U.tw, U.tb, upo, LAT, LAT, L, U.ratio, 1, nullptr, nullptr, st, nullptr, nullptr, nullptr, m->pk(U.tw), NPL));
+        HIPC(launch_transconv1d_taps(cur, U.tw, U.tb, upo, LAT, LAT, L, U.ratio, 1, nullptr, nullptr, st, nullptr, nullptr, nullptr, m->pk(U.tw), NPL, nullptr, RES));
         L *= U.ratio;
         float* dw = (upo == A) ? C : A;
         HIPC(launch_dwconv7(upo, U.dww, U.dwb, dw, LAT, L, st));
@@ -220,7 +222,7 @@
     };
     float* xact = other({cur});
     {
-        ConvArgs a; a.x = cur; a.w = m->init_w; a.wpk = m->pk(m->init_w); a.b = m->init_b; a.cin = LAT; a.cout = Cc; a.L = L; a.k = 7; a.dil = 1; a.planes = NPL;
+        ConvArgs a; a.x = cur; a.w = m->init_w; a.wpk = m->pk(m->init_w); a.b = m->init_b; a.cin = LAT; a.cout = Cc; a.L = L; a.k = 7; a.dil = 1; a.planes = NPL; a.resident = RES;
         a.post_a = m->blk[0].a; a.post_ib = m->blk[0].ib;
         if (taps && taps[Q3_DEC_INIT]) { float* raw = other({cur, xact}); a.y = raw; a.y2 = xact; HIPC(launch_conv1d(a, st)); Q3C(TAP(Q3_DEC_INIT, raw, (size_t)Cc * L)); }
         else { a.y = xact; HIPC(launch_conv1d(a, st)); }
@@ -230,7 +232,7 @@
         const DecBlockW& Bk = m->blk[b];
         float* Y = other({xact});
         float* YA = other({xact, Y});
-        HIPC(launch_transconv1d_taps(xact, Bk.tw, Bk.tb, Y, Bk.cin, Bk.cout, L, Bk.rate, 2, nullptr, nullptr, st, Bk.res[0].a1, Bk.res[0].ib1, YA, m->pk(Bk.tw), NPL));
+        HIPC(launch_transconv1d_taps(xact, Bk.tw, Bk.tb, Y, Bk.cin, Bk.cout, L, Bk.rate, 2, nullptr, nullptr, st, Bk.res[0].a1, Bk.res[0].ib1, YA, m->pk(Bk.tw), NPL, nullptr, RES));
         L *= Bk.rate; Cc = Bk.cout;
         float* T2 = other({Y, YA});
         for (int uu = 0; uu < 3; ++uu) {
@@ -240,18 +242,18 @@
             {
                 ResUnitArgs r{};
                 r.xa = YA; r.y = Y; r.ya = T2; r.w1pk = m->pk(R.c1w); r.w2pk = m->pk(R.c2w); r.b1 = R.c1b; r.b2 = R.c2b;
-                r.mid_a = R.a2; r.mid_ib = R.ib2; r.post_a = nxt_a; r.post_ib = nxt_ib; r.C = Cc; r.L = L; r.dil = dils[uu]; r.planes = NPL;
+                r.mid_a = R.a2; r.mid_ib = R.ib2; r.post_a = nxt_a; r.post_ib = nxt_ib; r.C = Cc; r.L = L; r.dil = dils[uu]; r.planes = NPL; r.resident = RES;
                 const hipError_t e = launch_resunit(r, st);
                 if (e == hipSuccess) { float* t = YA; YA = T2; T2 = t; continue; }
                 if (e != hipErrorNotSupported) HIPC(e);
             }
             {
-                ConvArgs a; a.x = YA; a.w = R.c1w; a.wpk = m->pk(R.c1w); a.b = R.c1b; a.y = T2; a.cin = Cc; a.cout = Cc; a.L = L; a.k = 7; a.dil = dils[uu]; a.planes = NPL;
+                ConvArgs a; a.x = YA; a.w = R.c1w; a.wpk = m->pk(R.c1w); a.b = R.c1b; a.y = T2; a.cin = Cc; a.cout = Cc; a.L = L; a.k = 7; a.dil = dils[uu]; a.planes = NPL; a.resident = RES;
                 a.post_a = R.a2; a.post_ib = R.ib2;
                 HIPC(launch_conv1d(a, st));
             }
             {
-                ConvArgs a; a.x = T2; a.w = R.c2w; a.wpk = m->pk(R.c2w); a.b = R.c2b; a.y = Y; a.y2 = YA; a.cin = Cc; a.cout = Cc; a.L = L; a.k = 1; a.dil = 1; a.resid = Y; a.planes = NPL;
+                ConvArgs a; a.x = T2; a.w = R.c2w; a.wpk = m->pk(R.c2w); a.b = R.c2b; a.y = Y; a.y2 = YA; a.cin = Cc; a.cout = Cc; a.L = L; a.k = 1; a.dil = 1; a.resid = Y; a.planes = NPL; a.resident = RES;
                 if (uu < 2) { a.post_a = Bk.res[uu + 1].a1; a.post_ib = Bk.res[uu + 1].ib1; }
                 else if (b < 3) { a.post_a = m->blk[b + 1].a; a.post_ib = m->blk[b + 1].ib; }
                 else { a.post_a = m->fin_a; a.post_ib = m->fin_ib; }
@@ -265,9 +267,9 @@
     return Q3_OK;
 }
 
-q3_status codec_decode_dev(const q3_model* m, CodecWS& ws, int T, hipStream_t st, float** taps, int c0) {
-    const q3_config& c = m->cfg;
-    const CodecScope scope(m);
+q3_status codec_decode_dev(const q3_model* m, CodecWS& ws, int T, hipStream_t st, float** taps, int c0, int resident) {
+    const q3_config& c = m->cfg;
+    const CodecScope scope(m, resident);
     const int Q = c.dec_q_dim, LAT = c.dec_latent;
     float *B = ws.bufB, *C = ws.bufC;
     Q3C(codec_front_quant(m, ws, T, st));
diff --git a/qwen3_tts_rs_amd/csrc/q3_engine.h b/qwen3_tts_rs_amd/csrc/q3_engine.h
--- a/qwen3_tts_rs_amd/csrc/q3_engine.h
+++ b/qwen3_tts_rs_amd/csrc/q3_engine.h
@@ -391,8 +391,8 @@
 Q3_HIDDEN void retile_bf16(const uint16_t* src, int N, int K, uint16_t* dst, int mode);
 Q3_HIDDEN q3_status codec_reserve(const q3_model* m, CodecWS& ws, int T, int Tf = 0);
 Q3_HIDDEN int samples_per_frame(const q3_config& c);
-Q3_HIDDEN q3_status codec_decode_dev(const q3_model* m, CodecWS& ws, int T, hipStream_t st, float** taps, int c0 = 0);
-struct Q3_HIDDEN CodecScope { int planes; explicit CodecScope(const q3_model* m); ~CodecScope(); CodecScope(const CodecScope&) = delete; };
+Q3_HIDDEN q3_status codec_decode_dev(const q3_model* m, CodecWS& ws, int T, hipStream_t st, float** taps, int c0 = 0, int resident = 0);
+struct Q3_HIDDEN CodecScope { int planes, resident; explicit CodecScope(const q3_model* m, int resident = 0); ~CodecScope(); CodecScope(const CodecScope&) = delete; };
 using CodecAttnFn = std::function<q3_status(int layer, float* q, float* k, float* v, float* ao)>;
 Q3_HIDDEN q3_status codec_rope_table(const q3_config& c, int n, float* cs_dev, float* sn_dev);
 Q3_HIDDEN q3_status codec_front_quant(const q3_model* m, CodecWS& ws, int T, hipStream_t st);
diff --git a/qwen3_tts_rs_amd/csrc/q3_kernels.h b/qwen3_tts_rs_amd/csrc/q3_kernels.h
--- a/qwen3_tts_rs_amd/csrc/q3_kernels.h
+++ b/qwen3_tts_rs_amd/csrc/q3_kernels.h
@@ -240,7 +240,10 @@
     float* y2 = nullptr;
     const void* wpk = nullptr;
     int planes = 3;
-};
+    int resident = 0;
+};
+size_t conv_resident_lds(size_t lds, int resident);
+size_t conv_last_dyn_lds();
 hipError_t launch_pack_conv_w(const float* w, void* out, int cout, int cin, int K, hipStream_t st);
 size_t packed_conv_w_bytes(int cout, int cin, int K);
 enum ConvKernel {
@@ -279,13 +282,14 @@
     const float* mid_a; const float* mid_ib; const float* post_a; const float* post_ib;
     int C, L, dil;
     int planes = 3;
+    int resident = 0;
 };
 hipError_t launch_resunit(const ResUnitArgs& r, hipStream_t st, int* path = nullptr);
 hipError_t launch_transconv1d_taps(const float* x, const float* wp, const float* b, float* y, int cin, int cout, int L,
                                    int stride, int taps, const float* snake_a, const float* snake_ib, hipStream_t st,
                                    const float* post_a = nullptr, const float* post_ib = nullptr, float* y2 = nullptr,
                                    const void* wpk = nullptr,
-                                   int planes = 3, int* path = nullptr);
+                                   int planes = 3, int* path = nullptr, int resident = 0);
 void transconv_phase_weights(const float* w, int cin, int cout, int k, int stride, float* out);
 hipError_t launch_snake_tables(const float* alpha, const float* beta, float* a, float* ib, int C, hipStream_t st);
 hipError_t launch_dwconv7(const float* x, const float* w, const float* b, float* y, int C, int L, hipStream_t st);
diff --git a/qwen3_tts_rs_amd/csrc/q3_kernels_codec.hip b/qwen3_tts_rs_amd/csrc/q3_kernels_codec.hip
--- a/qwen3_tts_rs_amd/csrc/q3_kernels_codec.hip
+++ b/qwen3_tts_rs_amd/csrc/q3_kernels_codec.hip
@@ -1,5 +1,6 @@
 #include "q3_kernels.h"
 
+#include <atomic>
 #include <math.h>
 #include <stdio.h>
 #include <stdlib.h>
@@ -698,6 +699,39 @@
 
 static int conv_planes(int asked) { return asked == 2 ? 2 : 3; }
 
+constexpr size_t CU_LDS_BYTES = 160 * 1024, LDS_GRANULE = 1280;
+size_t conv_resident_lds(size_t lds, int resident) {
+    if (resident < 1) return lds;
+    const size_t cap = (CU_LDS_BYTES / ((size_t)resident + 1) + 1 + LDS_GRANULE - 1) / LDS_GRANULE * LDS_GRANULE;
+    return lds > cap ? lds : cap;
+}
+static thread_local size_t tl_last_dyn_lds = 0;
+size_t conv_last_dyn_lds() { return tl_last_dyn_lds; }
+static size_t capped_lds(const void* fn, std::atomic<int>* raised, size_t lds, int resident) {
+    size_t want = conv_resident_lds(lds, resident);
+    if (want > 64 * 1024) {
+        int dev = 0;
+        if (hipGetDevice(&dev) != hipSuccess || dev < 0 || dev >= 16) want = lds;
+        else {
+            int r = raised[dev].load(std::memory_order_acquire);
+            if (r == 0) {
+                r = hipFuncSetAttribute(fn, hipFuncAttributeMaxDynamicSharedMemorySize, (int)conv_resident_lds(0, 1)) == hipSuccess ? 1 : -1;
+                if (r < 0) (void)hipGetLastError();
+                raised[dev].store(r, std::memory_order_release);
+            }
+            if (r < 0) want = lds;
+        }
+    }
+    tl_last_dyn_lds = want;
+    return want;
+}
+#define Q3_LAUNCH_CAPPED(KERNEL, grid, blk, lds, resident, st, ...)                                                              \
+    do {                                                                                                                       \
+        static std::atomic<int> raised_[16];                                                                                   \
+        const size_t lds_ = capped_lds(reinterpret_cast<const void*>(&KERNEL), raised_, (lds), (resident));                    \
+        hipLaunchKernelGGL(KERNEL, grid, blk, lds_, st, __VA_ARGS__);                                                          \
+    } while (0)
+
 ConvPath resunit_pick(int C, int L, int dil, bool complete, bool ya_is_xa, int planes) {
     static const bool off = getenv("Q3_CONV_F32") != nullptr || getenv("Q3_CODEC_NO_UNIT_FUSE") != nullptr;
     static const bool fuse192 = getenv("Q3_CODEC_UNIT_FUSE_192") != nullptr;
@@ -723,11 +757,11 @@
     const size_t lds = lds_x > lds_mid ? lds_x : lds_mid;
     const dim3 grid((r.L + 127) / 128);
     if (np == 2) {
-        if (r.C == 96) hipLaunchKernelGGL((k_resunit_bf16x3<3, 2>), grid, dim3(192), lds, st, a);
-        else hipLaunchKernelGGL((k_resunit_bf16x3<6, 2>), grid, dim3(384), lds, st, a);
+        if (r.C == 96) Q3_LAUNCH_CAPPED((k_resunit_bf16x3<3, 2>), grid, dim3(192), lds, r.resident, st, a);
+        else Q3_LAUNCH_CAPPED((k_resunit_bf16x3<6, 2>), grid, dim3(384), lds, r.resident, st, a);
     } else {
-        if (r.C == 96) hipLaunchKernelGGL((k_resunit_bf16x3<3, 3>), grid, dim3(192), lds, st, a);
-        else hipLaunchKernelGGL((k_resunit_bf16x3<6, 3>), grid, dim3(384), lds, st, a);
+        if (r.C == 96) Q3_LAUNCH_CAPPED((k_resunit_bf16x3<3, 3>), grid, dim3(192), lds, r.resident, st, a);
+        else Q3_LAUNCH_CAPPED((k_resunit_bf16x3<6, 3>), grid, dim3(384), lds, r.resident, st, a);
     }
     return hipGetLastError();
 }
@@ -815,7 +849,7 @@
 }
 
 template <int K, int CO_M, int T_M, int WCO, int WT, int NP>
-static hipError_t launch_bf16x3_vp(const ConvPath& p, const ConvDev& a, int phases, hipStream_t st) {
+static hipError_t launch_bf16x3_vp(const ConvPath& p, const ConvDev& a, int phases, int resident, hipStream_t st) {
     constexpr int CO_WG = 32 * CO_M * WCO, T_WG = 32 * T_M * WT;
     constexpr bool K1 = K == 1;
     constexpr int CIS1 = T_WG <= 64 ? 128 : 32;
@@ -828,7 +862,7 @@
     const dim3 blk(64 * WCO * WT);
     if constexpr (K1) {
         const bool pre = p.pre;
-#define Q3_CV(P, S, C) hipLaunchKernelGGL((k_conv_bf16x3<K, CO_M, T_M, WCO, WT, P, S, C, NP>), grid, blk, lds, st, ap)
+#define Q3_CV(P, S, C) Q3_LAUNCH_CAPPED((k_conv_bf16x3<K, CO_M, T_M, WCO, WT, P, S, C, NP>), grid, blk, lds, resident, st, ap)
         if (wide) {
             if (segm) { if (pre) Q3_CV(CO_M == 1, true, CIS1); else Q3_CV(false, true, CIS1); }
             else { if (pre) Q3_CV(CO_M == 1, false, CIS1); else Q3_CV(false, false, CIS1); }
@@ -838,28 +872,28 @@
         }
 #undef Q3_CV
     } else {
-        hipLaunchKernelGGL((k_conv_bf16x3<K, CO_M, T_M, WCO, WT, false, false, 32, NP>), grid, blk, lds, st, ap);
+        Q3_LAUNCH_CAPPED((k_conv_bf16x3<K, CO_M, T_M, WCO, WT, false, false, 32, NP>), grid, blk, lds, resident, st, ap);
     }
     return hipGetLastError();
 }
 static bool conv_two_plane_taps(int k) { return k == 1 || k == 2 || k == 7; }
 template <int K, int CO_M, int T_M, int WCO, int WT>
-static hipError_t launch_bf16x3_v(const ConvPath& p, const ConvDev& a, int phases, hipStream_t st) {
+static hipError_t launch_bf16x3_v(const ConvPath& p, const ConvDev& a, int phases, int resident, hipStream_t st) {
     if constexpr (K == 1 || K == 2 || K == 7)
-        if (p.np == 2) return launch_bf16x3_vp<K, CO_M, T_M, WCO, WT, 2>(p, a, phases, st);
+        if (p.np == 2) return launch_bf16x3_vp<K, CO_M, T_M, WCO, WT, 2>(p, a, phases, resident, st);
     if (p.np != 3) return hipErrorInvalidValue;
-    return launch_bf16x3_vp<K, CO_M, T_M, WCO, WT, 3>(p, a, phases, st);
+    return launch_bf16x3_vp<K, CO_M, T_M, WCO, WT, 3>(p, a, phases, resident, st);
 }
 template <int K>
-static hipError_t launch_bf16x3_k(const ConvPath& p, const ConvDev& a, int phases, hipStream_t st) {
+static hipError_t launch_bf16x3_k(const ConvPath& p, const ConvDev& a, int phases, int resident, hipStream_t st) {
     switch (p.kernel) {
-        case CK_BF16X3_96x128_TM4: return launch_bf16x3_v<K, 1, 4, 3, 1>(p, a, phases, st);
-        case CK_BF16X3_4Wx32x128: return launch_bf16x3_v<K, 1, 4, 4, 1>(p, a, phases, st);
-        case CK_BF16X3_4Wx32x256: return launch_bf16x3_v<K, 1, 8, 4, 1>(p, a, phases, st);
-        case CK_BF16X3_64x128: return launch_bf16x3_v<K, 1, 2, 2, 2>(p, a, phases, st);
-        case CK_BF16X3_64x64: return launch_bf16x3_v<K, 1, 1, 2, 2>(p, a, phases, st);
-        case CK_BF16X3_128x128: return launch_bf16x3_v<K, 2, 2, 2, 2>(p, a, phases, st);
-        case CK_BF16X3_96x128_6W: return launch_bf16x3_v<K, 1, 2, 3, 2>(p, a, phases, st);
+        case CK_BF16X3_96x128_TM4: return launch_bf16x3_v<K, 1, 4, 3, 1>(p, a, phases, resident, st);
+        case CK_BF16X3_4Wx32x128: return launch_bf16x3_v<K, 1, 4, 4, 1>(p, a, phases, resident, st);
+        case CK_BF16X3_4Wx32x256: return launch_bf16x3_v<K, 1, 8, 4, 1>(p, a, phases, resident, st);
+        case CK_BF16X3_64x128: return launch_bf16x3_v<K, 1, 2, 2, 2>(p, a, phases, resident, st);
+        case CK_BF16X3_64x64: return launch_bf16x3_v<K, 1, 1, 2, 2>(p, a, phases, resident, st);
+        case CK_BF16X3_128x128: return launch_bf16x3_v<K, 2, 2, 2, 2>(p, a, phases, resident, st);
+        case CK_BF16X3_96x128_6W: return launch_bf16x3_v<K, 1, 2, 3, 2>(p, a, phases, resident, st);
         default: return hipErrorInvalidValue;
     }
 }
@@ -998,7 +1032,7 @@
     *reinterpret_cast<float4*>(a.y + t) = make_float4(o[0], o[1], o[2], o[3]);
 }
 
-static hipError_t launch_conv_path(const ConvPath& p, const ConvDev& a, int phases, hipStream_t st) {
+static hipError_t launch_conv_path(const ConvPath& p, const ConvDev& a, int phases, int resident, hipStream_t st) {
     switch (p.kernel) {
         case CK_NONE: return p.refusal != hipSuccess ? p.refusal : hipErrorInvalidValue;
         case CK_OUT1_V4: hipLaunchKernelGGL(k_conv_out1_v4, dim3((a.L / 4 + 255) / 256), dim3(256), 0, st, a); break;
@@ -1024,11 +1058,11 @@
         }
         default:
             switch (a.k) {
-                case 1: return launch_bf16x3_k<1>(p, a, phases, st);
-                case 2: return launch_bf16x3_k<2>(p, a, phases, st);
-                case 3: return launch_bf16x3_k<3>(p, a, phases, st);
-                case 5: return launch_bf16x3_k<5>(p, a, phases, st);
-                case 7: return launch_bf16x3_k<7>(p, a, phases, st);
+                case 1: return launch_bf16x3_k<1>(p, a, phases, resident, st);
+                case 2: return launch_bf16x3_k<2>(p, a, phases, resident, st);
+                case 3: return launch_bf16x3_k<3>(p, a, phases, resident, st);
+                case 5: return launch_bf16x3_k<5>(p, a, phases, resident, st);
+                case 7: return launch_bf16x3_k<7>(p, a, phases, resident, st);
                 default: return hipErrorInvalidValue;
             }
     }
@@ -1046,12 +1080,12 @@
     a.ostride = 1; a.ooff = 0; a.oL = c.L; a.w_phase_stride = 0; a.ooff_phase = 0;
     a.post_a = c.post_a; a.post_ib = c.post_ib; a.y2 = c.y2;
     a.wpk = c.wpk; a.wpk_phase_stride = 0; a.planes = conv_planes(c.planes);
-    return launch_conv_path(p, a, 1, st);
+    return launch_conv_path(p, a, 1, c.resident, st);
 }
 
 hipError_t launch_transconv1d_taps(const float* x, const float* wp, const float* b, float* y, int cin, int cout, int L,
                                    int stride, int taps, const float* snake_a, const float* snake_ib, hipStream_t st,
-                                   const float* post_a, const float* post_ib, float* y2, const void* wpk, int planes, int* path) {
+                                   const float* post_a, const float* post_ib, float* y2, const void* wpk, int planes, int* path, int resident) {
     const ConvPath p = conv_pick(cout, cin, L, taps, 1, stride, wpk != nullptr, false, planes, false, true);
     if (path) *path = conv_path_code(p);
     if (p.kernel == CK_NONE) return p.refusal;
@@ -1063,7 +1097,7 @@
     a.snake_a = snake_a; a.snake_ib = snake_ib; a.resid = nullptr; a.scale = nullptr; a.act = 0;
     a.ostride = stride; a.ooff = 0; a.oL = L * stride;
     a.w_phase_stride = (size_t)cout * cin * taps; a.ooff_phase = 1;
-    return launch_conv_path(p, a, stride, st);
+    return launch_conv_path(p, a, stride, resident, st);
 }
 
 void transconv_phase_weights(const float* w, int cin, int cout, int k, int stride, float* out) {
diff --git a/qwen3_tts_rs_amd/csrc/q3_session.hip b/qwen3_tts_rs_amd/csrc/q3_session.hip
--- a/qwen3_tts_rs_amd/csrc/q3_session.hip
+++ b/qwen3_tts_rs_amd/csrc/q3_session.hip
@@ -1730,6 +1730,7 @@
     return decode_range_on(s, b, f0, f1, s->stream, pcm_host, cap, n_samples);
 }
 
+static constexpr bool DECODE_OVERLAP_DEFAULT = true;
 extern "C" q3_status q3_session_run(q3_session* s, int use_graph, float** pcm_host, const size_t* cap, size_t* n_samples, q3_timing* timing) {
     if (!s) return set_err(Q3_INVALID_ARG, "null session");
     if (any_open_text(s)) return set_err(Q3_UNSUPPORTED, "q3_session_run: a row's text is still open (q3_session_append_text with last != 0 closes it; or drive the session with q3_session_generate)");
@@ -1739,9 +1740,11 @@
     s->precapture = use_graph != 0;
     Q3C(q3_session_prefill(s));
     const auto t1 = clk::now();
-    const int overlap_env = [] { const char* e = getenv("Q3_DECODE_OVERLAP"); return e ? atoi(e) : 0; }();
-    static const int seg_env = [] { const char* e = getenv("Q3_DECODE_SEG"); const int v = e ? atoi(e) : 128; return v < 16 ? 16 : v; }();
-    bool overlap = overlap_env != 0 && !s->debug && !s->profile && s->max_frames > seg_env;
+    const int overlap_env = [] { const char* e = getenv("Q3_DECODE_OVERLAP"); return e ? (atoi(e) != 0 ? 1 : 0) : -1; }();
+    const int resident_env = [] { const char* e = getenv("Q3_DECODE_RESIDENT"); const int v = e ? atoi(e) : 1; return v < 0 ? 0 : (v > 2 ? 2 : v); }();
+    const int seg_env = [] { const char* e = getenv("Q3_DECODE_SEG"); const int v = e ? atoi(e) : 256; return v < 16 ? 16 : v; }();
+    const bool overlap_wanted = overlap_env >= 0 ? overlap_env != 0 : (DECODE_OVERLAP_DEFAULT && s->B >= 2 && s->B <= 16);
+    bool overlap = overlap_wanted && !s->debug && !s->profile && s->max_frames > seg_env;
     for (auto& q : s->seq) if (!q.ref_codes.empty()) overlap = false;
     const int spf = samples_per_frame(s->m->cfg);
     if (!overlap) {
@@ -1812,17 +1815,18 @@
     if (cus && s->aql && !s->aql_failed) { std::string why; if (q3::aql_restrict_cus(s->aql, 256 - cus, &why)) split.p = s->aql; }
     std::vector<int> dec_pos((size_t)s->B, 0);
     std::thread worker; q3_status wst = Q3_OK; std::string werr;
+    double join_wait_ms = 0.0; int n_dispatch = 0;
     auto join = [&]() -> q3_status {
         if (worker.joinable()) worker.join();
         if (wst != Q3_OK) return set_err(wst, "%s", werr.c_str());
         return Q3_OK;
     };
     struct Job { int b, a, e; };
-    auto seg_enqueue = [s, spf, pcm_host, cap](const Job& j, CodecWS& ws, hipStream_t st) -> q3_status {
+    auto seg_enqueue = [s, spf, pcm_host, cap](const Job& j, CodecWS& ws, hipStream_t st, int resident) -> q3_status {
         const int c0 = j.a > CODEC_CTX_FRAMES ? j.a - CODEC_CTX_FRAMES : 0;
         if (pcm_host && pcm_host[j.b] && (!cap || cap[j.b] < (size_t)j.e * spf)) return set_err(Q3_INVALID_ARG, "pcm buffer too small");
         HIPC(hipMemcpyAsync(ws.frames, s->codes + (size_t)j.b * s->max_frames * 16, (size_t)j.e * 16 * 4, hipMemcpyDeviceToDevice, st));
-        Q3C(codec_decode_dev(s->m, ws, j.e, st, nullptr, c0));
+        Q3C(codec_decode_dev(s->m, ws, j.e, st, nullptr, c0, resident));
         if (pcm_host && pcm_host[j.b])
             HIPC(hipMemcpyAsync(pcm_host[j.b] + (size_t)j.a * spf, ws.pcm + (size_t)(j.a - c0) * spf, (size_t)(j.e - j.a) * spf * 4, hipMemcpyDeviceToHost, st));
         return Q3_OK;
@@ -1842,17 +1846,21 @@
     auto dispatch = [&]() -> q3_status {
         std::vector<Job> jobs = collect(false);
         if (jobs.empty()) return Q3_OK;
-        Q3C(join());
-        worker = std::thread([s, jobs, seg_enqueue, &wst, &werr]() {
+        {
+            const auto j0 = clk::now();
+            Q3C(join());
+            join_wait_ms += ms(j0, clk::now()); ++n_dispatch;
+        }
+        worker = std::thread([s, jobs, seg_enqueue, resident_env, &wst, &werr]() {
             if (hipSetDevice(s->m->device) != hipSuccess) { wst = Q3_HIP_ERROR; werr = "hipSetDevice failed in the decode thread"; return; }
             for (const Job& j : jobs) {
-                const q3_status st = seg_enqueue(j, s->seg_ws, s->dec_stream);
+                const q3_status st = seg_enqueue(j, s->seg_ws, s->dec_stream, resident_env);
                 if (st != Q3_OK) { wst = st; werr = q3_last_error(); return; }
             }
         });
         return Q3_OK;
     };
-    static const int tail_env = [] { const char* e = getenv("Q3_DECODE_TAIL"); const int v = e ? atoi(e) : 32; return v < 16 ? 16 : v; }();
+    const int tail_env = [] { const char* e = getenv("Q3_DECODE_TAIL"); const int v = e ? atoi(e) : 32; return v < 16 ? 16 : v; }();
     q3_status st = Q3_OK;
     while (st == Q3_OK && session_remaining(s) > 0 && !all_done(s)) {
         int n = seg_env;
@@ -1878,7 +1886,7 @@
                 s->par_ws.emplace_back(); s->par_streams.push_back(pst);
             }
             for (int k = 0; k < conc; ++k) Q3C(codec_reserve(s->m, ws_of(k), seg_env + CODEC_CTX_FRAMES, s->max_frames));
-            for (size_t i = 0; i < jobs.size(); ++i) Q3C(seg_enqueue(jobs[i], ws_of((int)(i % conc)), st_of((int)(i % conc))));
+            for (size_t i = 0; i < jobs.size(); ++i) Q3C(seg_enqueue(jobs[i], ws_of((int)(i % conc)), st_of((int)(i % conc)), 0));
             return Q3_OK;
         };
         st = tail();
@@ -1894,6 +1902,10 @@
     }
     const auto t3 = clk::now();
     if (timing) { timing->prefill_ms = ms(t0, t1); timing->generation_ms = ms(t1, t2); timing->decode_ms = ms(t2, t3); timing->generation_frames = total; }
+    const bool log_env = getenv("Q3_DECODE_LOG") != nullptr;
+    if (log_env)
+        fprintf(stderr, "q3_session_run overlap: resident %d seg %d tail %d, %d dispatches, frame loop waited %.3f ms for the enqueue thread, frames %.1f ms, exposed decode %.1f ms\n",
+                resident_env, seg_env, tail_env, n_dispatch, join_wait_ms, ms(t1, t2), ms(t2, t3));
     return Q3_OK;
 }
 
diff --git a/qwen3_tts_rs_amd/csrc/q3_testapi.hip b/qwen3_tts_rs_amd/csrc/q3_testapi.hip
--- a/qwen3_tts_rs_amd/csrc/q3_testapi.hip
+++ b/qwen3_tts_rs_amd/csrc/q3_testapi.hip
@@ -589,7 +589,7 @@
 }
 extern "C" const char* q3_conv_path_name(int code) { return conv_path_name(code); }
 
-extern "C" q3_status q3_conv_ex(int device, const q3_conv_ex_args* p) {
+static q3_status conv_ex_run(int device, const q3_conv_ex_args* p, int resident, int* lds_bytes) {
     if (!p || !p->x || !p->w || !p->y) return set_err(Q3_INVALID_ARG, "q3_conv_ex: null argument");
     if (p->path) *p->path = 0;
     const int kind = p->kind, cin = p->cin, cout = p->cout, L = p->L, k = p->k, dil = p->dil;
@@ -660,14 +660,14 @@
         ConvArgs a;
         a.x = x; a.w = w; a.b = b; a.y = yr; a.cin = cin; a.cout = cout; a.L = L; a.k = k; a.dil = dil;
         a.snake_a = sa; a.snake_b = sb; a.resid = p->resid_in_place ? yr : res; a.scale = scale; a.act = p->act;
-        a.post_a = pa; a.post_ib = pb; a.y2 = y2r; a.wpk = wpk; a.planes = p->planes;
+        a.post_a = pa; a.post_ib = pb; a.y2 = y2r; a.wpk = wpk; a.planes = p->planes; a.resident = resident;
         e = launch_conv1d(a, 0, &path);
     } else if (kind == 1) {
-        e = launch_transconv1d_taps(x, w, b, yr, cin, cout, L, stride, taps, sa, sb, 0, pa, pb, y2r, wpk, p->planes, &path);
+        e = launch_transconv1d_taps(x, w, b, yr, cin, cout, L, stride, taps, sa, sb, 0, pa, pb, y2r, wpk, p->planes, &path, resident);
     } else {
         ResUnitArgs r{};
         r.xa = x; r.y = yr; r.ya = p->y2_is_x ? x : y2r; r.w1pk = wpk; r.w2pk = w2pk; r.b1 = b; r.b2 = b2;
-        r.mid_a = ma; r.mid_ib = mb; r.post_a = pa; r.post_ib = pb; r.C = cout; r.L = L; r.dil = dil; r.planes = p->planes;
+        r.mid_a = ma; r.mid_ib = mb; r.post_a = pa; r.post_ib = pb; r.C = cout; r.L = L; r.dil = dil; r.planes = p->planes; r.resident = resident;
         e = launch_resunit(r, 0, &path);
     }
     if (p->path) *p->path = path;
@@ -680,7 +680,24 @@
     HIPC(q3_hipDeviceSynchronize());
     HIPC(q3_hipMemcpy(p->y, y, yn * 4, hipMemcpyDeviceToHost));
     if (y2) HIPC(q3_hipMemcpy(p->y2, y2, yn * 4, hipMemcpyDeviceToHost));
-    return Q3_OK;
+    if (lds_bytes) *lds_bytes = (int)conv_last_dyn_lds();
+    return Q3_OK;
+}
+extern "C" q3_status q3_conv_ex(int device, const q3_conv_ex_args* p) { return conv_ex_run(device, p, 0, nullptr); }
+extern "C" q3_status q3_test_conv_resident(int device, const q3_conv_ex_args* p, int resident, int* lds_bytes) {
+    if (lds_bytes) *lds_bytes = 0;
+    if (resident < 0 || resident > 8) return set_err(Q3_INVALID_ARG, "q3_test_conv_resident: resident 0..8");
+    if (p && p->kind >= 0 && p->kind <= 2 && p->cin >= 1 && p->cout >= 1 && p->L >= 1 && p->k >= 1 && p->dil >= 1 && (p->kind != 1 || (p->stride >= 1 && p->k % p->stride == 0))) {
+        const int code = p->kind == 2 ? conv_path_code(resunit_pick(p->cout, p->L, p->dil, p->packed != 0 && p->w2 && p->mid_a, p->y2_is_x != 0, p->planes))
+                       : p->kind == 1 ? conv_path_code(conv_pick(p->cout, p->cin, p->L, p->k / p->stride, 1, p->stride, p->packed != 0, false, p->planes, false, true))
+                                      : conv_path_code(conv_pick(p->cout, p->cin, p->L, p->k, p->dil, 1, p->packed != 0, p->resid || p->resid_in_place, p->planes, false, false));
+        const int kern = code & CP_KERNEL_MASK;
+        if (!((kern >= CK_BF16X3_96x128_TM4 && kern <= CK_BF16X3_96x128_6W) || kern == CK_RESUNIT_3W || kern == CK_RESUNIT_6W)) {
+            if (p->path) *p->path = code;
+            return set_err(Q3_UNSUPPORTED, "q3_test_conv_resident: %s has no dynamic LDS to cap", conv_path_name(code));
+        }
+    }
+    return conv_ex_run(device, p, resident, lds_bytes);
 }
 
 static q3_status check_cl_out(const char* who, const void* x, const void* w, const void* y, int C, int L, int y_front, int y_elems) {
```

Measured after the change: 2882 (median of 6 runs). +1.4%, better.
